# bacpop/Pansim

Hardware: AMD Instinct MI355X
Metric: generations/sec (higher is better)
Workload: dtype u8

## Files before the change

### pansim_amd/csrc/core_kernels.h

```cpp
#pragma once

#include "ps_common.h"

#include <type_traits>

#define PS_SWEEP_MAX_GENS 2
struct core_sweep_args {
    uint8_t *state;
    uint8_t *out;
    const uint32_t *idx;
    const uint32_t *idx_next[PS_SWEEP_MAX_GENS - 1];
    const uint32_t *idxT;
    uint32_t N, pitch, cpr, rows;
    uint32_t site_offset;
    uint32_t gen, k0, k1;
    ps_core_plan plan;
    uint32_t *overflow_flag;
    unsigned long long *stamps;
    uint32_t *work_ctr;
    uint32_t launch_parity;
    uint32_t nt;
    uint32_t qcap;
    uint32_t qcap_limit;
    uint32_t *wide_flags;
    const uint32_t *site_T;
};

typedef uint32_t ps_u32x4 __attribute__((ext_vector_type(4)));
__device__ __forceinline__ uint4 ps_load_row16(const uint8_t *p, bool nt)
{
    if (nt) {
        const ps_u32x4 v = __builtin_nontemporal_load((const ps_u32x4 *)p);
        return make_uint4(v.x, v.y, v.z, v.w);
    }
    return *(const uint4 *)p;
}
__device__ __forceinline__ void ps_store_row16(uint8_t *p, const uint4 &v, bool nt)
{
    if (nt) {
        ps_u32x4 w = { v.x, v.y, v.z, v.w };
        __builtin_nontemporal_store(w, (ps_u32x4 *)p);
    } else {
        *(uint4 *)p = v;
    }
}

__device__ __forceinline__ void ps_set_byte(uint32_t (&w)[4], uint32_t k, uint32_t v)
{
    const uint32_t j = k >> 2, sh = (k & 3u) * 8u;
    const uint32_t m = ~(0xFFu << sh), val = v << sh;
#pragma unroll
    for (uint32_t jj = 0; jj < 4; jj++) w[jj] = (jj == j) ? ((w[jj] & m) | val) : w[jj];
}

#ifndef PS_WAVE_DMA
#define PS_WAVE_DMA 0
#endif
__device__ __forceinline__ void ps_dma16(const uint8_t *gsrc, uint8_t *lds_base, bool nt)
{
    if (nt) __builtin_amdgcn_global_load_lds((const __attribute__((address_space(1))) void *)gsrc,
                                             (__attribute__((address_space(3))) void *)lds_base, 16, 0, 2);
    else __builtin_amdgcn_global_load_lds((const __attribute__((address_space(1))) void *)gsrc,
                                          (__attribute__((address_space(3))) void *)lds_base, 16, 0, 0);
}

__device__ __forceinline__ uint32_t ps_noncand_word(const ps_u4 &A, uint32_t cshift)
{
    return (cshift <= 0u ? A.x : 0u) | (cshift <= 1u ? A.y : 0u) | (cshift <= 2u ? A.z : 0u) | (cshift <= 3u ? A.w : 0u);
}

__device__ __forceinline__ uint32_t ps_site_bits(uint32_t site) { return 0x0F0F0F0Fu << (4u * (site & 1u)); }
__device__ __forceinline__ uint32_t ps_bit_cell(uint32_t p) { return ((p & 3u) << 2) | (p >> 3); }
__device__ __forceinline__ uint32_t ps_valid_word(uint32_t nvalid)
{
    if (nvalid >= 16u) return 0xFFFFFFFFu;
    uint32_t m = 0;
#pragma unroll
    for (uint32_t k = 0; k < 16u; k++)
        if (k < nvalid) m |= 0x11u << (8u * (k & 3u) + (k >> 2));
    return m;
}

__device__ __forceinline__ uint32_t ps_cand_word(const ps_u4 &A, uint32_t site, uint32_t cshift)
{
    return ~ps_noncand_word(A, cshift) & ps_site_bits(site);
}

template <bool WT>
__device__ __forceinline__ ps_cell ps_classify_site(uint32_t u, const ps_core_plan &pl, const core_sweep_args &a, uint32_t site)
{
    if (!WT) return ps_classify(u, pl);
    const uint4 *rec = (const uint4 *)(a.site_T + 8u * (size_t)min(site - a.site_offset, a.rows - 1u));
    const uint4 lo = rec[0], hi = rec[1];
    ps_core_plan sp;
    sp.T[0] = lo.x; sp.T[1] = lo.y; sp.T[2] = lo.z; sp.T[3] = lo.w; sp.T[4] = hi.x; sp.T[5] = hi.y; sp.T[6] = hi.z;
    return ps_classify(u, sp);
}

template <bool WT>
__device__ __forceinline__ ps_cell ps_cell_events(const core_sweep_args &a, const ps_u4 &A, const ps_u4 &B, uint32_t site, uint32_t ind, uint32_t gen,
                                                  uint32_t k0, uint32_t k1, const ps_core_plan &pl, uint32_t &l2y)
{
    ps_cell o = { 0u, 0u };
    const uint32_t n = ps_cell_nibble(A, site, ind);
    if (n >> pl.cshift) return o;
    const uint32_t code = ps_sym_code(4u * n + ps_cell_pair(B, site, ind), pl);
    if (code > 1u) {
        o.mut = code;
    } else if (code == 1u) {
        const ps_u4 l2 = ps_philox(site, ind, gen, PS_STREAM_CORE_L2, k0, k1);
        o = ps_classify_site<WT>(l2.x, pl, a, site);
        l2y = l2.y;
    }
    return o;
}

template <bool DO_GATHER, bool DO_MUT, bool DO_HR, bool WT = false>
__global__ void __launch_bounds__(1024) core_sweep_inline_kernel(core_sweep_args a)
{
    extern __shared__ __attribute__((aligned(16))) uint8_t lds[];
    const uint32_t lane = threadIdx.x, lpr = blockDim.x;
    uint8_t *rowA = lds;
    uint8_t *rowS = rowA + a.pitch;
    uint16_t *hrm = (uint16_t *)(rowS + a.pitch);
    const ps_core_plan pl = a.plan;
    const bool events = pl.has_events && (DO_MUT || DO_HR);

    for (uint32_t row = blockIdx.x; row < a.rows; row += gridDim.x) {
        const uint32_t site = a.site_offset + row;
        uint8_t *grow = a.state + (size_t)row * a.pitch;
        if (DO_GATHER) {
            for (uint32_t c = lane; c < a.cpr; c += lpr)
                *(uint4 *)(rowA + 16u * c) = *(const uint4 *)(grow + 16u * c);
            __syncthreads();
        }
        for (uint32_t c = lane; c < a.cpr; c += lpr) {
            uint32_t d[4];
            if (DO_GATHER) {
#pragma unroll
                for (int j = 0; j < 4; j++) {
                    uint32_t w = 0;
#pragma unroll
                    for (int b = 0; b < 4; b++) {
                        const uint32_t i = c * 16u + 4 * j + b;
                        const uint32_t v = (i < a.N) ? (uint32_t)rowA[a.idx[i]] : 0u;
                        w |= v << (8 * b);
                    }
                    d[j] = w;
                }
            } else {
                const uint4 v = *(const uint4 *)(grow + 16u * c);
                d[0] = v.x; d[1] = v.y; d[2] = v.z; d[3] = v.w;
            }
            uint32_t hm = 0;
            if (events) {
                const ps_u4 A = ps_philox_l1a(site >> 1, c, a.gen, a.k0, a.k1), B = ps_philox_l1b(site >> 2, c, a.gen, a.k0, a.k1);
                uint32_t cm = ps_cand_word(A, site, pl.cshift);
                while (cm) {
                    const uint32_t k = ps_bit_cell(__builtin_ctz(cm));
                    cm &= cm - 1u;
                    const uint32_t i = c * 16u + k;
                    if (i >= a.N) continue;
                    uint32_t l2y;
                    const ps_cell cell = ps_cell_events<WT>(a, A, B, site, i, a.gen, a.k0, a.k1, pl, l2y);
                    if (DO_MUT && cell.mut) ps_set_byte(d, k, cell.mut);
                    if (DO_HR && cell.hr) hm |= 1u << k;
                }
            }
            if (DO_HR) {
                *(uint4 *)(rowS + 16u * c) = make_uint4(d[0], d[1], d[2], d[3]);
                hrm[c] = (uint16_t)hm;
            } else {
                *(uint4 *)(grow + 16u * c) = make_uint4(d[0], d[1], d[2], d[3]);
            }
        }
        if (DO_HR) {
            __syncthreads();
            for (uint32_t c = lane; c < a.cpr; c += lpr) {
                const uint4 v = *(const uint4 *)(rowS + 16u * c);
                uint32_t d[4] = { v.x, v.y, v.z, v.w };
                uint32_t hm = hrm[c];
                while (hm) {
                    const uint32_t k = __builtin_ctz(hm);
                    hm &= hm - 1u;
                    const uint32_t i = c * 16u + k;
                    const ps_u4 l2 = ps_philox(site, i, a.gen, PS_STREAM_CORE_L2, a.k0, a.k1);
                    uint32_t donor = ps_mulhi(l2.y, a.N - 1u);
                    donor += (donor >= i) ? 1u : 0u;
                    ps_set_byte(d, k, (uint32_t)rowS[donor]);
                }
                *(uint4 *)(grow + 16u * c) = make_uint4(d[0], d[1], d[2], d[3]);
            }
            if (!DO_GATHER) __syncthreads();
        }
    }
}

#define PS_BATCH_ROWS 4u

__device__ __forceinline__ void ps_wave_sync()
{
    __builtin_amdgcn_fence(__ATOMIC_RELEASE, "wavefront");
    __builtin_amdgcn_wave_barrier();
    __builtin_amdgcn_fence(__ATOMIC_ACQUIRE, "wavefront");
}

__device__ __forceinline__ uint32_t ps_lane_prefix(uint64_t bal)
{
    return __builtin_amdgcn_mbcnt_hi((uint32_t)(bal >> 32), __builtin_amdgcn_mbcnt_lo((uint32_t)bal, 0u));
}

__device__ __forceinline__ uint32_t ps_wave_scan_incl(uint32_t x)
{
    x += (uint32_t)__builtin_amdgcn_update_dpp(0, (int)x, 0x111, 0xF, 0xF, false);
    x += (uint32_t)__builtin_amdgcn_update_dpp(0, (int)x, 0x112, 0xF, 0xF, false);
    x += (uint32_t)__builtin_amdgcn_update_dpp(0, (int)x, 0x114, 0xF, 0xF, false);
    x += (uint32_t)__builtin_amdgcn_update_dpp(0, (int)x, 0x118, 0xF, 0xF, false);
    x += (uint32_t)__builtin_amdgcn_update_dpp(0, (int)x, 0x142, 0xA, 0xF, false);
    x += (uint32_t)__builtin_amdgcn_update_dpp(0, (int)x, 0x143, 0xC, 0xF, false);
    return x;
}

struct ps_class_words { uint32_t dec, res; };
__device__ __forceinline__ ps_class_words ps_classes(uint32_t p0, uint32_t p1, uint32_t p2, uint32_t p3, uint32_t p4, uint32_t p5,
                                                     uint32_t k, uint32_t nE, uint32_t vm)
{
    const uint32_t c1 = __builtin_amdgcn_bitop3_b32(p1, p2, p3, 0x01) & vm;
    uint32_t lt;
    switch (nE) {
    case 1: lt = __builtin_amdgcn_bitop3_b32(p0, p5, p4, 0x01); break;
    case 2: lt = __builtin_amdgcn_bitop3_b32(p0, p5, p4, 0x03); break;
    case 3: lt = __builtin_amdgcn_bitop3_b32(p0, p5, p4, 0x07); break;
    case 4: lt = __builtin_amdgcn_bitop3_b32(p0, p5, p4, 0x0F); break;
    case 5: lt = __builtin_amdgcn_bitop3_b32(p0, p5, p4, 0x1F); break;
    case 6: lt = __builtin_amdgcn_bitop3_b32(p0, p5, p4, 0x3F); break;
    case 7: lt = __builtin_amdgcn_bitop3_b32(p0, p5, p4, 0x7F); break;
    default: lt = 0xFFFFFFFFu; break;
    }
    ps_class_words o;
    o.dec = k ? c1 & __builtin_amdgcn_bitop3_b32(p0, p5, p4, 0x07) : 0u;
    o.res = c1 & lt & ~o.dec;
    return o;
}

struct ps_apply_words { uint32_t y0, y1, ya, yb, yc; };
PS_HD uint32_t ps_bfi(uint32_t m, uint32_t a, uint32_t b)
{
#if defined(__HIP_DEVICE_COMPILE__) && __has_builtin(__builtin_amdgcn_bitop3_b32)
    return __builtin_amdgcn_bitop3_b32(m, a, b, 0xCA);
#else
    return (a & m) | (b & ~m);
#endif
}
__device__ __forceinline__ ps_apply_words ps_apply_prepare(uint32_t dec, uint32_t p4, uint32_t p5)
{
    const uint32_t r1 = p5 >> 1, r2 = p4 >> 2, l1 = p5 << 1, l2 = dec << 2;
    ps_apply_words o;
    o.y0 = ps_bfi(0x01010101u, p4, ps_bfi(0x02020202u, l1, l2));
    o.y1 = ps_bfi(0x02020202u, p4, ps_bfi(0x04040404u, l1, l2));
    o.ya = ps_bfi(0x09090909u, r2, ps_bfi(0x12121212u, r1, dec));
    o.yb = ps_bfi(0x12121212u, r2, ps_bfi(0x24242424u, r1, dec));
    o.yc = ps_bfi(0x24242424u, r2, ps_bfi(0x48484848u, r1, dec));
    return o;
}
template <uint32_t SLOT>
__device__ __forceinline__ uint32_t ps_apply_dword(const ps_apply_words &y, uint32_t d)
{
    constexpr uint32_t sh = SLOT == 0u ? 0u : SLOT == 1u ? 1u : SLOT == 2u ? 0u : SLOT == 3u ? 1u : SLOT == 4u ? 2u : SLOT == 5u ? 3u : SLOT == 6u ? 4u : 5u;
    const uint32_t src = SLOT == 0u ? y.y0 : SLOT == 1u ? y.y1 : (SLOT == 2u || SLOT == 5u) ? y.ya : (SLOT == 3u || SLOT == 6u) ? y.yb : y.yc;
    const uint32_t f = (src >> sh) & 0x07070707u;
    const uint32_t allele = __builtin_amdgcn_perm(0x00080402u, 0u, f);
    const uint32_t mask = __builtin_amdgcn_perm(0x00FFFFFFu, 0u, f);
    return ps_bfi(mask, allele, d);
}
template <uint32_t H>
__device__ __forceinline__ void ps_apply_row(const ps_apply_words &y, uint4 &d)
{
    d.x = ps_apply_dword<4u * H + 0u>(y, d.x);
    d.y = ps_apply_dword<4u * H + 1u>(y, d.y);
    d.z = ps_apply_dword<4u * H + 2u>(y, d.z);
    d.w = ps_apply_dword<4u * H + 3u>(y, d.w);
}

__device__ __forceinline__ uint32_t ps_push_scan(uint32_t w0, uint32_t w1, uint16_t *q, uint32_t lane, uint32_t qcap)
{
    const uint32_t c0 = (uint32_t)__popc(w0), c = c0 + (uint32_t)__popc(w1);
    const uint32_t incl = ps_wave_scan_incl(c);
    const uint32_t qn = __builtin_amdgcn_readlane(incl, 63);
    if (qn <= qcap) {
        uint16_t *qp = q + (incl - c) - 1, *qp1 = qp + c0;
        const uint32_t tag = lane << 6;
        for (uint32_t m = w0; m; m &= m - 1u) *++qp = (uint16_t)(tag | (uint32_t)__builtin_ctz(m));
        for (uint32_t m = w1; m; m &= m - 1u) *++qp1 = (uint16_t)(tag | 32u | (uint32_t)__builtin_ctz(m));
    }
    return qn;
}
__device__ __forceinline__ uint32_t ps_entry_cell(uint32_t ent)
{
    const uint32_t cell = ((ent & 3u) << 2) | ((ent >> 3) & 3u), row = ((ent >> 2) & 1u) | ((ent >> 4) & 2u);
    return (row << 10) | ((ent >> 2) & 0x3F0u) | cell;
}

PS_HD uint32_t ps_gather_dword(uint32_t lane, uint32_t m) { return lane + 64u * m; }
PS_HD uint32_t ps_gather_child(uint32_t lane, uint32_t m, uint32_t b) { return 4u * ps_gather_dword(lane, m) + b; }
PS_HD uint32_t ps_gather_source(uint32_t child, uint32_t parent, uint32_t N, uint32_t pitch)
{
    return child < N ? parent : (N < pitch - 1u ? N : pitch - 1u);
}

__device__ __forceinline__ uint32_t ps_pack4(uint32_t b0, uint32_t b1, uint32_t b2, uint32_t b3)
{
    return __builtin_amdgcn_perm(b1, b0, 0x0c0c0400u) | __builtin_amdgcn_perm(b3, b2, 0x04000c0cu);
}

#ifdef PS_STAMP
#define PS_T(k) do { unsigned long long t_; asm volatile("s_waitcnt lgkmcnt(0)\n\ts_memtime %0\n\ts_waitcnt lgkmcnt(0)" : "=s"(t_) :: "memory"); st_acc[k] += t_ - st_last; st_last = t_; } while (0)
#else
#define PS_T(k) do { } while (0)
#endif
#ifndef PS_WAVE_LB
#define PS_WAVE_LB 6
#endif
#ifndef PS_WAVE_PREFETCH
#define PS_WAVE_PREFETCH 0
#endif
__host__ __device__ constexpr uint32_t ps_queue_bytes(uint32_t qcap) { return (qcap * 2u + 15u) & ~15u; }
__host__ __device__ constexpr uint32_t ps_wave_lds(uint32_t qcap) { return PS_BATCH_ROWS * 1024u + ps_queue_bytes(qcap); }

template <bool DO_GATHER, bool DO_MUT, bool DO_HR, bool NT = false, bool WT = false, uint32_t T = 1>
__global__ void __launch_bounds__(256, T > 1 ? 4 : PS_WAVE_LB) core_sweep_wave_kernel(core_sweep_args a)
{
    static_assert(T >= 1 && T <= PS_SWEEP_MAX_GENS, "generations per pass");
    static_assert(T == 1 || (DO_GATHER && (DO_MUT || DO_HR)), "several generations per pass: the gather + events form only");
#ifdef PS_STAMP
    unsigned long long st_acc[8] = { 0, 0, 0, 0, 0, 0, 0, 0 };
    unsigned long long st_last;
    asm volatile("s_memtime %0\n\ts_waitcnt lgkmcnt(0)" : "=s"(st_last) :: "memory");
#endif
#ifdef PS_GROUP_TIMES
    const unsigned long long gt_start = __builtin_amdgcn_s_memrealtime();
#endif
    constexpr uint32_t PS_ROWS = PS_BATCH_ROWS;
    extern __shared__ __attribute__((aligned(16))) uint8_t lds[];
    const uint32_t wave = threadIdx.x >> 6, lane = threadIdx.x & 63u;
    uint8_t *rowbuf = lds + wave * ps_wave_lds(a.qcap);
    uint16_t *q = (uint16_t *)(rowbuf + PS_ROWS * 1024u);
    const ps_core_plan pl = a.plan;
    const uint32_t nE = 3u * pl.k + pl.R;
    constexpr bool events = DO_MUT || DO_HR;
    const bool has_chunk = lane < a.cpr;
    const uint32_t i0 = lane * 16u;
    const uint32_t ld_off = has_chunk ? i0 : 0u;
    const uint32_t nvalid = (i0 >= a.N) ? 0u : min(16u, a.N - i0);
    const uint32_t vm = ps_valid_word(nvalid);

    uint32_t pidx[T][16];
    if (DO_GATHER) {
#pragma unroll
        for (uint32_t t = 0; t < T; t++) {
            const uint32_t *ix = t ? a.idx_next[t ? t - 1u : 0u] : a.idx;
            const bool wide = ((uintptr_t)ix & 15u) == 0u;
#pragma unroll
            for (uint32_t m = 0; m < 4; m++) {
                const uint32_t c0 = ps_gather_child(lane, m, 0u);
                if (wide && c0 + 4u <= a.N) {
                    const uint4 p4 = *(const uint4 *)(ix + c0);
                    pidx[t][4u * m] = p4.x, pidx[t][4u * m + 1u] = p4.y, pidx[t][4u * m + 2u] = p4.z, pidx[t][4u * m + 3u] = p4.w;
                } else {
#pragma unroll
                    for (uint32_t b = 0; b < 4; b++) pidx[t][4u * m + b] = ps_gather_source(c0 + b, c0 + b < a.N ? ix[c0 + b] : 0u, a.N, a.pitch);
                }
            }
        }
    }

    constexpr uint32_t PS_CHUNK = 3u;
    const uint32_t grp = blockIdx.x & 7u;
    const uint32_t off = a.site_offset & 3u, g0 = a.site_offset >> 2;
    const uint32_t batches = (a.rows + off + PS_ROWS - 1u) / PS_ROWS;
    const uint32_t b_lo = (uint32_t)((uint64_t)batches * grp / 8u), b_hi = (uint32_t)((uint64_t)batches * (grp + 1u) / 8u);
    uint32_t *ctr = a.work_ctr + (a.launch_parity * 8u + grp) * 32u;
    if (blockIdx.x < 8u && threadIdx.x == 0) a.work_ctr[((a.launch_parity ^ 1u) * 8u + blockIdx.x) * 32u] = 0u;
    uint32_t next_chunk = 0;
    if (lane == 0) next_chunk = __hip_atomic_fetch_add(ctr, 1u, __ATOMIC_RELAXED, __HIP_MEMORY_SCOPE_AGENT);
#if PS_WAVE_PREFETCH
    uint4 vn[PS_ROWS];
    uint32_t pf_batch = 0xFFFFFFFFu;
#pragma unroll
    for (uint32_t rr = 0; rr < PS_ROWS; rr++) vn[rr] = make_uint4(0, 0, 0, 0);
#endif
    for (;;) {
        const uint32_t chunk = __builtin_amdgcn_readfirstlane(next_chunk);
        if (b_lo + chunk * PS_CHUNK >= b_hi) break;
        if (lane == 0) next_chunk = __hip_atomic_fetch_add(ctr, 1u, __ATOMIC_RELAXED, __HIP_MEMORY_SCOPE_AGENT);
    for (uint32_t cb = 0; cb < PS_CHUNK; cb++) {
        const uint32_t batch = b_lo + chunk * PS_CHUNK + cb;
        if (batch >= b_hi) break;
        const int lr0 = (int)(batch * PS_ROWS) - (int)off;
        const uint32_t sg = g0 + batch;
        auto lrow = [&](uint32_t rr) -> uint32_t { return (uint32_t)min(max(lr0 + (int)rr, 0), (int)a.rows - 1); };
        uint4 v[PS_ROWS];
#if PS_WAVE_PREFETCH
        if (pf_batch == batch) {
#pragma unroll
            for (uint32_t rr = 0; rr < PS_ROWS; rr++) v[rr] = vn[rr];
        } else
#endif
#pragma unroll
        for (uint32_t rr = 0; rr < PS_ROWS; rr++)
            v[rr] = ps_load_row16(a.state + (size_t)lrow(rr) * a.pitch + ld_off, NT);
        if (DO_GATHER) {
#pragma unroll
            for (uint32_t rr = 0; rr < PS_ROWS; rr++) *(uint4 *)(rowbuf + rr * 1024u + i0) = v[rr];
            ps_wave_sync();
        }
        PS_T(0);

#pragma unroll
        for (uint32_t t = 0; t < T; t++) {
        const uint32_t gen = a.gen + t;
        uint32_t wl[2] = { 0u, 0u };
        ps_apply_words y[2] = {};
        if (events) {
            const ps_u4 A0 = ps_philox_l1a(2u * sg, lane, gen, a.k0, a.k1);
            const ps_u4 A1 = ps_philox_l1a(2u * sg + 1u, lane, gen, a.k0, a.k1);
            const ps_u4 B = ps_philox_l1b(sg, lane, gen, a.k0, a.k1);
            const ps_class_words c0 = ps_classes(A0.x, A0.y, A0.z, A0.w, B.x, B.z, pl.k, nE, vm);
            const ps_class_words c1 = ps_classes(A1.x, A1.y, A1.z, A1.w, B.y, B.w, pl.k, nE, vm);
            wl[0] = c0.res;
            wl[1] = c1.res;
            if (DO_MUT) {
                y[0] = ps_apply_prepare(c0.dec, B.x & c0.dec, B.z & c0.dec);
                y[1] = ps_apply_prepare(c1.dec, B.y & c1.dec, B.w & c1.dec);
            }
        }
        PS_T(2);
        constexpr bool ahead = T > 1 && DO_GATHER;
        uint32_t g[16] = {};
        auto gather = [&](uint32_t rr) {
#pragma unroll
            for (int k = 0; k < 16; k++) g[k] = rowbuf[rr * 1024u + pidx[t][k]];
        };
        if (ahead) gather(0u);
#pragma unroll
        for (uint32_t rr = 0; rr < PS_ROWS; rr++) {
            uint8_t *row = rowbuf + rr * 1024u;
            uint4 d = v[rr];
            if (DO_GATHER) {
                if (!ahead) gather(rr);
                uint32_t w[4];
#pragma unroll
                for (int m = 0; m < 4; m++) w[m] = ps_pack4(g[4 * m], g[4 * m + 1], g[4 * m + 2], g[4 * m + 3]);
                ps_wave_sync();
#pragma unroll
                for (uint32_t m = 0; m < 4; m++) *(uint32_t *)(row + 4u * ps_gather_dword(lane, m)) = w[m];
                if (events && DO_MUT) {
                    ps_wave_sync();
                    d = *(const uint4 *)(row + i0);
                }
                if (ahead && rr + 1u < PS_ROWS) {
                    __builtin_amdgcn_sched_barrier(0);
                    gather(rr + 1u);
                    __builtin_amdgcn_sched_barrier(0);
                }
            }
            if (events && DO_MUT) {
                if (rr & 1u) ps_apply_row<1u>(y[rr >> 1], d);
                else ps_apply_row<0u>(y[rr >> 1], d);
            }
            if (events && (DO_MUT || !DO_GATHER)) *(uint4 *)(row + i0) = d;
            __builtin_amdgcn_sched_barrier(0);
        }
        PS_T(1);
        const uint32_t qcap = a.qcap_limit ? min(a.qcap, a.qcap_limit) : a.qcap;
        uint32_t qn = 0;
        if (events) qn = ps_push_scan(wl[0], wl[1], q, lane, qcap);
        PS_T(3);
        ps_wave_sync();
#if PS_WAVE_PREFETCH
        if (t + 1u == T) {
            uint32_t nb = batch + 1u;
            if (cb + 1u >= PS_CHUNK || nb >= b_hi) nb = b_lo + (uint32_t)__builtin_amdgcn_readfirstlane(next_chunk) * PS_CHUNK;
            pf_batch = nb < b_hi ? nb : 0xFFFFFFFFu;
            if (nb < b_hi) {
                const int nlr0 = (int)(nb * PS_ROWS) - (int)off;
#pragma unroll
                for (uint32_t rr = 0; rr < PS_ROWS; rr++)
                    vn[rr] = ps_load_row16(a.state + (size_t)(uint32_t)min(max(nlr0 + (int)rr, 0), (int)a.rows - 1) * a.pitch + ld_off, NT);
            }
        }
#endif
        const bool redo = events && (qn > qcap || (DO_HR && 2u * qn > qcap));
        if (redo) {
#pragma unroll 1
            for (uint32_t rr = 0; rr < PS_ROWS; rr++) {
                uint8_t *row = rowbuf + rr * 1024u;
                const uint32_t site = 4u * sg + rr;
                const ps_u4 Ar = ps_philox_l1a(site >> 1, lane, gen, a.k0, a.k1);
                const ps_u4 Br = ps_philox_l1b(sg, lane, gen, a.k0, a.k1);
                uint32_t cmr = ps_cand_word(Ar, site, pl.cshift) & vm;
                uint32_t hm = 0;
                while (cmr) {
                    const uint32_t k = ps_bit_cell(__builtin_ctz(cmr)), cellidx = i0 + k;
                    cmr &= cmr - 1u;
                    uint32_t l2y = 0;
                    const ps_cell cell = ps_cell_events<WT>(a, Ar, Br, site, cellidx, gen, a.k0, a.k1, pl, l2y);
                    if (DO_MUT && cell.mut) row[cellidx] = (uint8_t)cell.mut;
                    if (DO_HR && cell.hr) hm |= 1u << k;
                }
                if (DO_HR) {
                    ps_wave_sync();
                    uint32_t dv[4] = { 0u, 0u, 0u, 0u };
                    for (uint32_t tmp = hm; tmp;) {
                        const uint32_t k = __builtin_ctz(tmp), cellidx = i0 + k;
                        tmp &= tmp - 1u;
                        const ps_u4 l2 = ps_philox(site, cellidx, gen, PS_STREAM_CORE_L2, a.k0, a.k1);
                        uint32_t donor = ps_mulhi(l2.y, a.N - 1u);
                        donor += (donor >= cellidx) ? 1u : 0u;
                        ps_set_byte(dv, k, (uint32_t)row[donor]);
                    }
                    ps_wave_sync();
                    for (uint32_t tmp = hm; tmp;) {
                        const uint32_t k = __builtin_ctz(tmp);
                        tmp &= tmp - 1u;
                        row[i0 + k] = (uint8_t)((dv[k >> 2] >> (8u * (k & 3u))) & 0xFFu);
                    }
                }
            }
            ps_wave_sync();
        } else if (events) {
            uint16_t *qh = q + qcap - 1u;
            for (uint32_t base = 0; base < qn; base += 64u) {
                const uint32_t e = base + lane;
                if (e < qn) {
                    const uint32_t ent = ps_entry_cell(q[e]);
                    const uint32_t cellidx = ent & 1023u, rr = ent >> 10;
                    const ps_u4 l2 = ps_philox(4u * sg + rr, cellidx, gen, PS_STREAM_CORE_L2, a.k0, a.k1);
                    const ps_cell cell = ps_classify_site<WT>(l2.x, pl, a, 4u * sg + rr);
                    if (DO_MUT && cell.mut) rowbuf[ent] = (uint8_t)cell.mut;
                    if (DO_HR) {
                        uint32_t out = 0;
                        if (cell.hr) {
                            uint32_t donor = ps_mulhi(l2.y, a.N - 1u);
                            donor += (donor >= cellidx) ? 1u : 0u;
                            out = donor | 0x8000u;
                        }
                        *(qh - e) = (uint16_t)out;
                    }
                }
            }
            if (DO_HR) {
                ps_wave_sync();
                for (uint32_t base = 0; base < qn; base += 64u) {
                    const uint32_t e = base + lane;
                    if (e < qn) {
                        const uint32_t h = *(qh - e);
                        if (h >> 15) *(qh - e) = (uint16_t)((uint32_t)rowbuf[(ps_entry_cell(q[e]) & 3072u) | (h & 1023u)] | 0x8000u);
                    }
                }
                ps_wave_sync();
                for (uint32_t base = 0; base < qn; base += 64u) {
                    const uint32_t e = base + lane;
                    if (e < qn) {
                        const uint32_t h = *(qh - e);
                        if (h >> 15) rowbuf[ps_entry_cell(q[e])] = (uint8_t)(h & 0xFFu);
                    }
                }
            }
            ps_wave_sync();
        }
        }
        PS_T(5);

        if (has_chunk) {
#pragma unroll
            for (uint32_t rr = 0; rr < PS_ROWS; rr++) {
                const int lr = lr0 + (int)rr;
                if (lr >= 0 && lr < (int)a.rows) {
                    const uint4 o = (DO_GATHER || events) ? *(const uint4 *)(rowbuf + rr * 1024u + i0) : v[rr];
                    ps_store_row16(a.out + (size_t)lr * a.pitch + i0, o, NT);
                }
            }
        }
        ps_wave_sync();
        PS_T(6);
    }
    }
#ifdef PS_STAMP
    if (lane == 0)
        for (int k = 0; k < 8; k++) atomicAdd((unsigned long long *)a.stamps + k, st_acc[k]);
#endif
#ifdef PS_GROUP_TIMES
    if (lane == 0) {
        atomicMax((unsigned long long *)a.stamps + 8 + grp, (unsigned long long)__builtin_amdgcn_s_memrealtime());
        atomicMax((unsigned long long *)a.stamps + 16 + grp, gt_start);
        if (blockIdx.x < 8 && wave == 0) ((unsigned long long *)a.stamps)[24 + grp] = gt_start;
    }
#endif
}

#ifndef PS_WCAP
#define PS_WCAP 1216u
#endif
#ifndef PS_WBPC
#define PS_WBPC 6
#endif
#ifndef PS_WLB
#define PS_WLB 6
#endif
#ifndef PS_WINDOW_NT_LOADS
#define PS_WINDOW_NT_LOADS 0
#endif
#define PS_WSTRIDE (PS_WCAP + 16u)
#define PS_WHR 64u
__host__ __device__ constexpr uint32_t ps_window_lds(uint32_t qcap) { return PS_BATCH_ROWS * PS_WSTRIDE + ps_queue_bytes(qcap) + PS_WHR * 6u; }

template <bool WT>
__device__ __forceinline__ uint32_t ps_donor_value(const core_sweep_args &a, const ps_core_plan &pl, const uint8_t *old_row,
                                                   uint32_t site, uint32_t donor, bool do_mut)
{
    uint32_t val = old_row[a.idx[donor]];
    if (do_mut) {
        const ps_u4 A = ps_philox_l1a(site >> 1, donor >> 4, a.gen, a.k0, a.k1);
        const uint32_t n = ps_cell_nibble(A, site, donor);
        if ((n >> pl.cshift) == 0u) {
            const ps_u4 B = ps_philox_l1b(site >> 2, donor >> 4, a.gen, a.k0, a.k1);
            const uint32_t code = ps_sym_code(4u * n + ps_cell_pair(B, site, donor), pl);
            if (code > 1u) {
                val = code;
            } else if (code == 1u) {
                const ps_u4 l2 = ps_philox(site, donor, a.gen, PS_STREAM_CORE_L2, a.k0, a.k1);
                const ps_cell cell = ps_classify_site<WT>(l2.x, pl, a, site);
                if (cell.mut) val = cell.mut;
            }
        }
    }
    return val;
}


template <bool DO_MUT, bool DO_HR, bool NT, bool WIDE, bool WT = false>
__global__ void __launch_bounds__(256, PS_WLB) core_sweep_window_kernel(core_sweep_args a)
{
    constexpr uint32_t PS_ROWS = PS_BATCH_ROWS;
    extern __shared__ __attribute__((aligned(16))) uint8_t lds[];
    const uint32_t wave = threadIdx.x >> 6, lane = threadIdx.x & 63u;
    uint8_t *rowbuf = lds + wave * ps_window_lds(a.qcap);
    uint16_t *q = (uint16_t *)(rowbuf + PS_ROWS * PS_WSTRIDE);
    uint32_t *hr_d = (uint32_t *)(rowbuf + PS_ROWS * PS_WSTRIDE + ps_queue_bytes(a.qcap));
    uint16_t *hr_e = (uint16_t *)(hr_d + PS_WHR);
    if (lane < PS_ROWS) *(uint4 *)(rowbuf + lane * PS_WSTRIDE + PS_WCAP) = make_uint4(0, 0, 0, 0);
    const ps_core_plan pl = a.plan;
    const uint32_t segs = (a.N + 1023u) >> 10;
    const uint32_t grp = blockIdx.x & 7u;
    const uint32_t wg = __builtin_amdgcn_readfirstlane((blockIdx.x >> 3) * 4u + wave);
    const uint32_t sgm = wg % segs;
    if (wg < segs && lane == 0) a.work_ctr[(((a.launch_parity ^ 1u) * 8u + grp) * segs + wg) * 32u] = 0u;
    if (WIDE) {
        if (__builtin_amdgcn_readfirstlane(a.wide_flags[(a.gen & 1u) * 32u]) == 0u) return;
    } else if (blockIdx.x == 0 && threadIdx.x == 0) {
        a.wide_flags[((a.gen + 1u) & 1u) * 32u] = 0u;
    }
    const uint32_t c_first = sgm * 1024u, c_last = min(c_first + 1023u, a.N - 1u);
    const uint32_t chunk = sgm * 64u + lane;
    const bool has_chunk = chunk < a.cpr;
    const uint32_t i0 = lane * 16u, c0 = c_first + i0;
    const uint32_t nvalid = (c0 >= a.N) ? 0u : min(16u, a.N - c0);
    const uint32_t vm = ps_valid_word(nvalid);
    const uint32_t nE = 3u * pl.k + pl.R;
    const uint32_t w_lo = __builtin_amdgcn_readfirstlane(a.idx[c_first]) & ~15u;
    const uint32_t w_hi = __builtin_amdgcn_readfirstlane(a.idx[c_last]);
    const uint32_t wbytes = w_hi - w_lo + 1u;
    const bool wide = wbytes > PS_WCAP;
    uint32_t pidx[16];
#pragma unroll
    for (uint32_t k = 0; k < 16; k++) pidx[k] = (k < nvalid) ? a.idx[c0 + k] - w_lo : PS_WCAP;
    const bool ld0 = !WIDE && i0 < wbytes, ld1 = !WIDE && 1024u + i0 < wbytes;
    auto cell_addr = [](uint32_t ent) -> uint32_t { return (ent & 1023u) + ((ent >> 10) & 3u) * PS_WSTRIDE; };

    constexpr uint32_t PS_CHUNK = 3u;
    const uint32_t off = a.site_offset & 3u, g0 = a.site_offset >> 2;
    const uint32_t batches = (a.rows + off + PS_ROWS - 1u) / PS_ROWS;
    const uint32_t b_lo = (uint32_t)((uint64_t)batches * grp / 8u), b_hi = (uint32_t)((uint64_t)batches * (grp + 1u) / 8u);
    uint32_t *ctr = a.work_ctr + ((a.launch_parity * 8u + grp) * segs + sgm) * 32u;
    if (wide != WIDE) {
        if (!WIDE && lane == 0) a.wide_flags[(a.gen & 1u) * 32u] = 1u;
        return;
    }
    uint32_t next_chunk = 0;
    if (lane == 0) next_chunk = __hip_atomic_fetch_add(ctr, 1u, __ATOMIC_RELAXED, __HIP_MEMORY_SCOPE_AGENT);
    for (;;) {
        const uint32_t chk = __builtin_amdgcn_readfirstlane(next_chunk);
        if (b_lo + chk * PS_CHUNK >= b_hi) break;
        if (lane == 0) next_chunk = __hip_atomic_fetch_add(ctr, 1u, __ATOMIC_RELAXED, __HIP_MEMORY_SCOPE_AGENT);
    for (uint32_t cb = 0; cb < PS_CHUNK; cb++) {
        const uint32_t batch = b_lo + chk * PS_CHUNK + cb;
        if (batch >= b_hi) break;
        const int lr0 = (int)(batch * PS_ROWS) - (int)off;
        const uint32_t sg = g0 + batch;
        auto lrow = [&](uint32_t rr) -> uint32_t { return (uint32_t)min(max(lr0 + (int)rr, 0), (int)a.rows - 1); };
#pragma unroll
        for (uint32_t rr = 0; rr < PS_ROWS; rr++) {
            const uint8_t *src = a.state + (size_t)lrow(rr) * a.pitch + w_lo;
            if (ld0) ps_dma16(src + i0, rowbuf + rr * PS_WSTRIDE, NT && PS_WINDOW_NT_LOADS);
            if (ld1) ps_dma16(src + 1024u + i0, rowbuf + rr * PS_WSTRIDE + 1024u, NT && PS_WINDOW_NT_LOADS);
        }
        uint32_t wl0, wl1;
        ps_apply_words y[2] = {};
        {
            const ps_u4 A0 = ps_philox_l1a(2u * sg, chunk, a.gen, a.k0, a.k1);
            const ps_u4 A1 = ps_philox_l1a(2u * sg + 1u, chunk, a.gen, a.k0, a.k1);
            const ps_u4 B = ps_philox_l1b(sg, chunk, a.gen, a.k0, a.k1);
            const ps_class_words c0 = ps_classes(A0.x, A0.y, A0.z, A0.w, B.x, B.z, pl.k, nE, vm);
            const ps_class_words c1 = ps_classes(A1.x, A1.y, A1.z, A1.w, B.y, B.w, pl.k, nE, vm);
            wl0 = c0.res;
            wl1 = c1.res;
            if (DO_MUT) {
                y[0] = ps_apply_prepare(c0.dec, B.x & c0.dec, B.z & c0.dec);
                y[1] = ps_apply_prepare(c1.dec, B.y & c1.dec, B.w & c1.dec);
            }
        }
        asm volatile("s_waitcnt vmcnt(0)" ::: "memory");
        ps_wave_sync();
#pragma unroll
        for (uint32_t rr = 0; rr < PS_ROWS; rr++) {
            uint8_t *win = rowbuf + rr * PS_WSTRIDE;
            uint32_t w[4] = { 0u, 0u, 0u, 0u };
            if (!WIDE) {
#pragma unroll
                for (int j = 0; j < 4; j++)
                    w[j] = ps_pack4(win[pidx[4 * j]], win[pidx[4 * j + 1]], win[pidx[4 * j + 2]], win[pidx[4 * j + 3]]);
// ... 1523 lines not shown
```

### pansim_amd/csrc/pansim_capi.hip

```cpp
#include "../../include/pansim_hip.h"

#include <hip/hip_runtime.h>

#include <algorithm>
#include <charconv>
#include <chrono>
#include <condition_variable>
#include <mutex>
#include <cmath>
#include <cstdarg>
#include <cstdio>
#include <cstdlib>
#include <cstring>
#include <string>
#include <thread>
#include <type_traits>
#include <vector>

#include "acc_kernels.h"
#include "core_kernels.h"
#include "ps_common.h"

static thread_local std::string g_err;

// ... 80 lines not shown
    hs_poisson_table(lambda, &kmin, &t);
    if (t.empty() || t.size() > cap || !kmin_out || !thr) return 0;
    *kmin_out = kmin;
    memcpy(thr, t.data(), t.size() * sizeof(uint32_t));
    return (uint32_t)t.size();
}


static uint32_t prob_to_u32(double p)
{
    const double x = std::floor(p * 4294967296.0);
    if (!(x > 0.0)) return 0u;
    if (x >= 4294967295.0) return 0xFFFFFFFFu;
    return (uint32_t)x;
}

static void make_core_plan(double lam_mut, double lam_hr, uint64_t L, ps_core_plan *plan)
{
    const double p = (lam_mut > 0.0) ? -std::expm1(-lam_mut / (double)L) : 0.0;
    const double q = (lam_hr > 0.0) ? -std::expm1(-lam_hr / (double)L) : 0.0;
    const double a = p * (1.0 - q) / 3.0;
    const double b = p * q / 3.0;
    const double c = (1.0 - p) * q;
    const uint32_t k = (uint32_t)std::floor(a * 64.0);
    const double a_left = a - (double)k / 64.0;
    const double m_res = a_left + a_left + a_left + b + b + b + c;
    uint32_t R = (uint32_t)std::ceil(m_res * 64.0);
    if (3u * k + R > 64u) R = 64u - 3u * k;
    const double scale = R ? 64.0 / (double)R : 0.0;
    double cum[7];
    cum[0] = a_left * scale;
    cum[1] = (a_left + a_left) * scale;
    cum[2] = (a_left + a_left + a_left) * scale;
    cum[3] = (a_left + a_left + a_left + b) * scale;
    cum[4] = (a_left + a_left + a_left + b + b) * scale;
    cum[5] = (a_left + a_left + a_left + b + b + b) * scale;
    cum[6] = m_res * scale;
    uint32_t prev = 0;
    for (int j = 0; j < 7; j++) {
        uint32_t t = prob_to_u32(cum[j]);
        if (t < prev) t = prev;
        plan->T[j] = t;
        prev = t;
    }
    if (plan->T[6] == 0u) R = 0u;
    plan->k = k;
    plan->R = R;
    plan->has_events = (k > 0u || R > 0u) ? 1u : 0u;
    uint32_t cs = 0;
    while (cs < 4u && 3u * k + R > (4u << cs)) cs++;
    plan->cshift = cs;
}

static uint32_t acc_flip_threshold(double lam, uint64_t n_genes)
{
    if (!(lam > 0.0) || n_genes == 0) return 0u;
    const double pf = -std::expm1(-2.0 * lam / (double)n_genes) / 2.0;
    return prob_to_u32(pf);
}

enum { PS_RO_HIST, PS_RO_CLUSTERS, PS_RO_TREE, PS_RO_KNN, PS_RO_GEN, PS_RO_LD_SEL, PS_RO_LD, PS_RO_UPGMA, PS_RO_DIFF, PS_RO_PARS, PS_RO_TCMP, PS_RO_GS, PS_RO_MLST, PS_RO_NJ, PS_RO_BOOT, PS_RO_NNI, PS_RO_LIK, PS_RO_MODEL, PS_RO_MODEL_NNI, PS_RO_ANC, PS_RO_GENE, PS_RO_COUNT };
struct readout_slot {
    void *d = nullptr;
    uint64_t cap = 0;
    double ms[5] = {};
    bool timed = false;
};

struct ps_population {
    ps_config cfg{};
    int device = 0;
    hipStream_t stream = nullptr;
    bool rates_set = false;
    uint8_t *state = nullptr;
    uint8_t *state2 = nullptr;
    int sweep_oop = -1;
    uint32_t pitch = 0, cpr = 0;
    ps_core_plan cplan{};
    bool site_weighted = false;
    uint32_t *d_site_T = nullptr;
    uint8_t *d_gene_tab = nullptr;
    bool nibble_safe = true;
    bool onehot_safe = true;
    uint32_t *d_pack2 = nullptr;
    uint32_t *d_pair_part = nullptr;
    uint64_t pair_part_cap = 0;
    uint64_t pack2_cap = 0;
    acc_dims d{};
    uint64_t *G[2] = { nullptr, nullptr };
    bool g_valid = false;
    int32_t *fuse_counts_out = nullptr;
    double *fuse_logw_out = nullptr;
    bool counts_fresh = false;
    hipStream_t stream_of_call = nullptr;
    uint64_t edit_epoch = 0;
    uint64_t *I[2] = { nullptr, nullptr };
    uint32_t *d_ptab[PS_MAX_COMP] = {};
    uint32_t ptab_kmin[PS_MAX_COMP] = {}, ptab_len[PS_MAX_COMP] = {};
    void *hgt_ovf_img = nullptr;
    uint32_t hgt_bin_cap = 0;
    void *hgt_scratch = nullptr;
    uint64_t hgt_scratch_cap = 0;
    uint64_t *I_snap = nullptr;
    bool snap_valid = false;
    uint32_t hgt_slices = 0;
    uint32_t hgt_events_per_thread = 0;
    bool hgt_list_in_global = false;
    bool hgt_bin_list_in_global = false;
    uint32_t hgt_bin_prio = 0;
    uint32_t *cnt = nullptr;
    int cur = 0;
    ps_acc_plan aplan{};
    uint32_t donor_lo = 0, donor_cnt = 0;
    uint64_t *d_delta = nullptr;
    uint64_t delta_words = 0;
    ps_exchange_fn exchange = nullptr;
    void *exchange_ctx = nullptr;
    uint32_t *d_idx = nullptr;
    uint32_t *d_idxT = nullptr;
    uint32_t *d_work = nullptr;
    uint32_t work_flags_ofs = 0;
    uint64_t sweep_launches = 0;
    uint64_t window_launches = 0;
    double *d_log1p = nullptr;
    int32_t *d_num_genes = nullptr;
    double *d_logw = nullptr;
    uint32_t *d_H = nullptr;
    double *d_Dt = nullptr;
    void *d_davg = nullptr;
    uint64_t davg_cap = 0;
    int davg_form = 0;
    void *d_davg_in = nullptr;
    uint64_t davg_in_cap = 0;
    uint32_t davg_nb = 0;
    uint32_t davg_ib = 0;
    bool davg_plain_division = false;
    uint64_t H_cap = 0;
    int core_davg_form = 0;
    uint32_t core_davg_band = 0;
    uint32_t *d_cdavg = nullptr;
    uint64_t cdavg_cap = 0;
    int pair_mode = 0;
    int last_pair_form = 0;
    uint32_t pair_ranges = 0;
    int hgt_mode = 0;
    void *d_pairs = nullptr;
    uint32_t pair_threads = 0;
    uint64_t pairs_cap = 0, pairs_cached = 0;
    const uint32_t *pairs_src1 = nullptr, *pairs_src2 = nullptr;
    bool pairs_tiled = false;
    std::vector<uint32_t> h_r1, h_r2;
    uint32_t lds_limit = 160 * 1024;
    uint32_t sweep_blocks_per_cu = 8;
    uint32_t sweep_rows = 4;
    bool force_block_sweep = false;
    bool force_inline_sweep = false;
    uint32_t block_waves = 0;
    bool no_block_preload = false;
    uint32_t block_batch = 0;
    uint32_t sweep_generations = 0;
    uint32_t sweep_queue_cap = 0;
    uint32_t hgt_apply_threads = 1024;
    uint32_t window_blocks_per_cu = 0;
    uint32_t free_cus_per_xcd = 0;
    bool exchange_beside_sweep = false;
    int last_sweep_form = 0;
    int window_sweep = -1;
    int (*rows_refresh)(void *ctx) = nullptr;
    void *rows_ctx = nullptr;
    std::vector<uint32_t> row_slot;
    uint32_t *d_row_slot = nullptr;
    bool rows_overridden = false;
    uint32_t *d_site_counts = nullptr;
    unsigned long long *d_div = nullptr;
    hipEvent_t div_ev[2] = {};
    bool div_timed = false;
    readout_slot ro[PS_RO_COUNT];
    uint32_t gene_team = 0;
    uint32_t ld_band = 0;
    uint32_t mlst_band = 0;
    int gather_form = 0;
    double sample_ms = 0.0;
    bool sample_timed = false;
    uint32_t *h_flag = nullptr, *d_flag = nullptr;
    unsigned long long *h_stamps = nullptr, *d_stamps = nullptr;
};

static int use_device(const ps_population *p)
{
    HIPCHK(hipSetDevice(p->device));
    return PS_OK;
}

template <class T>
static hipError_t dev_grow_err(T *&ptr, uint64_t &cap, uint64_t need)
{
    if (cap >= need) return hipSuccess;
    if (ptr) {
        const hipError_t e = hipFree(ptr);
        if (e != hipSuccess) return e;
    }
    ptr = nullptr;
    cap = 0;
    const hipError_t e = hipMalloc(&ptr, need * sizeof(std::conditional_t<std::is_void<T>::value, char, T>));
    if (e == hipSuccess) cap = need;
    return e;
}

template <class T>
static int dev_grow(T *&ptr, uint64_t &cap, uint64_t need)
{
    HIPCHK(dev_grow_err(ptr, cap, need));
    return PS_OK;
}

#include "readout_common.h"

template <class T>
struct dev_tmp {
    T *p = nullptr;
    int device = 0;
    dev_tmp() = default;
    dev_tmp(const dev_tmp &) = delete;
    dev_tmp &operator=(const dev_tmp &) = delete;
    ~dev_tmp()
    {
        if (!p) return;
        (void)hipSetDevice(device);
        (void)hipFree(p);
    }
    int alloc(uint64_t n)
    {
        HIPCHK(hipGetDevice(&device));
        HIPCHK(hipMalloc(&p, n * sizeof(T)));
        return PS_OK;
    }
};

static int rows_current(ps_population *p, const uint32_t **slot_out)
{
    if (p->rows_overridden) p->row_slot.clear();
    else if (p->rows_refresh) PSCHK(p->rows_refresh(p->rows_ctx));
    *slot_out = p->row_slot.empty() ? nullptr : p->row_slot.data();
    return PS_OK;
}

template <typename T>
static void rows_permute(T *v, const uint32_t *slot, uint64_t n)
{
    if (!slot) return;
    std::vector<T> tmp(v, v + n);
    for (uint64_t k = 0; k < n; k++) v[k] = tmp[slot[k]];
}

extern "C" void ps_population_destroy(ps_population *p)
{
    if (!p) return;
    (void)hipSetDevice(p->device);
    if (p->stream) (void)hipStreamSynchronize(p->stream);
    void *ptrs[] = { p->d_row_slot, p->state, p->state2, p->d_delta, p->hgt_ovf_img, p->G[0], p->G[1], p->I[0], p->I[1], p->I_snap, p->d_ptab[0], p->d_ptab[1], p->hgt_scratch, p->cnt, p->d_idx, p->d_idxT, p->d_work,
                     p->d_log1p, p->d_num_genes, p->d_logw, p->d_pairs, p->d_H, p->d_Dt, p->d_davg, p->d_davg_in, p->d_pack2, p->d_pair_part, p->d_cdavg };
    for (void *q : ptrs)
        if (q) (void)hipFree(q);
    for (int c = 2; c < PS_MAX_COMP; c++)
        if (p->d_ptab[c]) (void)hipFree(p->d_ptab[c]);
    if (p->d_site_T) (void)hipFree(p->d_site_T);
    if (p->d_gene_tab) (void)hipFree(p->d_gene_tab);
    if (p->d_site_counts) (void)hipFree(p->d_site_counts);
    if (p->d_div) (void)hipFree(p->d_div);
    for (readout_slot &r : p->ro)
        if (r.d) (void)hipFree(r.d);
    for (hipEvent_t e : p->div_ev)
        if (e) (void)hipEventDestroy(e);
    if (p->h_flag) (void)hipHostFree(p->h_flag);
    if (p->h_stamps) {
        if (p->d_stamps) {
            (void)hipMemcpy(p->h_stamps, p->d_stamps, 32 * sizeof(unsigned long long), hipMemcpyDeviceToHost);
            (void)hipFree(p->d_stamps);
        }
        if (getenv("PANSIM_PRINT_STAMPS"))
            for (int k = 0; k < 32; k++) fprintf(stderr, "stamp[%d] = %llu\n", k, p->h_stamps[k]);
        (void)hipHostFree(p->h_stamps);
    }
    if (p->stream) (void)hipStreamDestroy(p->stream);
    delete p;
}

static int pop_create_impl(const ps_config *cfg, const uint8_t *init_vec, ps_population *p)
{
    int ndev = 0;
    PSCHK(ps_needs_device(&ndev));
    if (cfg->device >= 0) {
        if (cfg->device >= ndev) return ps_fail(PS_ERR_INVALID, "device %d out of range", cfg->device);
        p->device = cfg->device;
    } else {
        HIPCHK(hipGetDevice(&p->device));
    }
    PSCHK(use_device(p));
    if (cfg->core)
        if (const char *e = getenv("PANSIM_SWEEP_FREE_CUS")) p->free_cus_per_xcd = (uint32_t)std::max(0, std::min(8, atoi(e)));
    if (p->free_cus_per_xcd) {
        hipDeviceProp_t prop;
        HIPCHK(hipGetDeviceProperties(&prop, p->device));
        std::vector<uint32_t> mask((size_t)(prop.multiProcessorCount + 31) / 32, 0xFFFFFFFFu);
        for (uint32_t b = 0; b < 8u * p->free_cus_per_xcd && b < (uint32_t)prop.multiProcessorCount; b++) mask[b / 32u] &= ~(1u << (b % 32u));
        if (hipExtStreamCreateWithCUMask(&p->stream, (uint32_t)mask.size(), mask.data()) != hipSuccess) {
            (void)hipGetLastError();
            p->free_cus_per_xcd = 0;
            HIPCHK(hipStreamCreateWithFlags(&p->stream, hipStreamNonBlocking));
        }
    } else
    HIPCHK(hipStreamCreateWithFlags(&p->stream, hipStreamNonBlocking));
    if (const char *e = getenv("PANSIM_SWEEP_BLOCKS_PER_CU")) {
        const int v = atoi(e);
        if (v >= 1 && v <= 8) p->sweep_blocks_per_cu = (uint32_t)v;
    }
    if (const char *e = getenv("PANSIM_SWEEP_GENERATIONS")) {
        const int v = atoi(e);
        if (v >= 0 && v <= (int)PS_SWEEP_MAX_GENS) p->sweep_generations = (uint32_t)v;
    }
    if (const char *e = getenv("PANSIM_HGT_MODE")) p->hgt_mode = atoi(e);
    if (const char *e = getenv("PANSIM_SWEEP_OOP")) p->sweep_oop = std::max(-1, std::min(2, atoi(e)));
    if (const char *e = getenv("PANSIM_WINDOW_SWEEP")) p->window_sweep = std::max(-1, std::min(1, atoi(e)));
    if (const char *e = getenv("PANSIM_ACC_LDS_LIMIT")) { const int v = atoi(e); if (v >= 1024 && v <= 160 * 1024 && !cfg->core) p->lds_limit = (uint32_t)v; }
    if (const char *e = getenv("PANSIM_HGT_APPLY_THREADS")) { const int v = atoi(e); if (v == 256 || v == 512 || v == 1024) p->hgt_apply_threads = (uint32_t)v; }
    if (const char *e = getenv("PANSIM_WINDOW_BPC")) p->window_blocks_per_cu = (uint32_t)std::max(0, std::min(8, atoi(e)));
    if (const char *e = getenv("PANSIM_BLOCK_BATCH")) p->block_batch = (uint32_t)atoi(e);
    if (const char *e = getenv("PANSIM_BLOCK_WAVES")) p->block_waves = (uint32_t)atoi(e);
    if (const char *e = getenv("PANSIM_HGT_SLICES")) p->hgt_slices = (uint32_t)atoi(e);
    if (const char *e = getenv("PANSIM_HGT_BIN_LIST_GLOBAL")) p->hgt_bin_list_in_global = atoi(e) != 0;
    if (const char *e = getenv("PANSIM_HGT_BIN_PRIO")) p->hgt_bin_prio = (uint32_t)std::max(0, std::min(3, atoi(e)));
    if (const char *e = getenv("PANSIM_SWEEP_ROWS")) {
        const int v = atoi(e);
        if (v >= 2 && v <= 4) p->sweep_rows = (uint32_t)v;
    }
    const uint64_t N = cfg->pop_size, C = cfg->ncols;
    HIPCHK(hipMalloc(&p->d_idx, std::max<uint64_t>(N, 1) * sizeof(uint32_t)));
    HIPCHK(hipHostMalloc(&p->h_flag, sizeof(uint32_t), hipHostMallocMapped));
    *p->h_flag = 0;
    HIPCHK(hipHostMalloc(&p->h_stamps, 32 * sizeof(unsigned long long), hipHostMallocMapped));
    memset(p->h_stamps, 0, 32 * sizeof(unsigned long long));
    HIPCHK(hipMalloc(&p->d_stamps, 32 * sizeof(unsigned long long)));
    HIPCHK(hipMemset(p->d_stamps, 0, 32 * sizeof(unsigned long long)));
    HIPCHK(hipHostGetDevicePointer((void **)&p->d_flag, p->h_flag, 0));
    uint8_t *d_vec = nullptr;
    HIPCHK(hipMalloc(&d_vec, std::max<uint64_t>(C, 1)));
    if (C && init_vec) HIPCHK(hipMemcpyAsync(d_vec, init_vec, C, hipMemcpyHostToDevice, p->stream));
    if (cfg->core) {
        p->pitch = (uint32_t)((N + 127) / 128 * 128);
        p->cpr = p->pitch / 16;
        HIPCHK(hipMalloc(&p->state, std::max<uint64_t>(C, 1) * p->pitch));
        HIPCHK(hipMalloc(&p->d_idxT, 16ull * p->cpr * sizeof(uint32_t)));
        {
            const uint64_t nctr = 8 * std::max<uint64_t>(1, std::min<uint64_t>((N + 1023) / 1024, 4096));
            HIPCHK(hipMalloc(&p->d_work, 2 * nctr * 128 + 256));
            HIPCHK(hipMemsetAsync(p->d_work, 0, 2 * nctr * 128 + 256, p->stream));
            p->work_flags_ofs = (uint32_t)(2 * nctr * 32);
        }
        if (C && init_vec) {
            const uint64_t total = C * p->cpr;
            const uint32_t blocks = (uint32_t)std::min<uint64_t>((total + 255) / 256, 65536);
            core_init_kernel<<<blocks, 256, 0, p->stream>>>(p->state, d_vec, (uint32_t)N, p->pitch,
                                                            (uint32_t)C);
        }
    } else {
        p->d.N = (uint32_t)N;
        p->d.G = (uint32_t)C;
        p->d.W = (uint32_t)((N + 63) / 64);
        p->d.GW = (uint32_t)((C + 63) / 64);
        const uint64_t nG = std::max<uint64_t>((uint64_t)p->d.G * p->d.W, 1) * 8;
        const uint64_t nI = std::max<uint64_t>((uint64_t)p->d.N * p->d.GW, 1) * 8;
        HIPCHK(hipMalloc(&p->G[0], nG));
        for (int k = 0; k < 2; k++) HIPCHK(hipMalloc(&p->I[k], nI));
        if (C > 65536) return ps_fail(PS_ERR_INVALID, "at most 65536 accessory genes are supported");
        HIPCHK(hipMalloc(&p->cnt, (std::max<uint64_t>(N, 1) * PS_MAX_COMP + 64) * sizeof(uint32_t)));
        HIPCHK(hipMalloc(&p->d_log1p, std::max<uint64_t>(C, 1) * sizeof(double)));
        HIPCHK(hipMalloc(&p->d_num_genes, std::max<uint64_t>(N, 1) * sizeof(int32_t)));
        HIPCHK(hipMalloc(&p->d_logw, std::max<uint64_t>(N, 1) * sizeof(double)));
        const uint64_t total = (uint64_t)p->d.G * p->d.W + (uint64_t)p->d.N * p->d.GW;
        if (total && init_vec)
            acc_init_kernel<<<(uint32_t)((total + 255) / 256), 256, 0, p->stream>>>(p->G[0], p->I[0],
                                                                                d_vec, p->d);
        p->g_valid = true;
    }
    HIPCHK(hipGetLastError());
    HIPCHK(hipStreamSynchronize(p->stream));
    HIPCHK(hipFree(d_vec));
    return PS_OK;
}

extern "C" int ps_population_create(const ps_config *cfg, const uint8_t *init_vec, ps_population **out)
{
    if (!cfg || !out) return ps_fail(PS_ERR_INVALID, "null argument");
    *out = nullptr;
    if (cfg->pop_size < 1) return ps_fail(PS_ERR_INVALID, "pop_size must be >= 1");
    if (cfg->pop_size > 0xFFFFFFFFull - 128 || cfg->global_cols > 0xFFFFFFFFull
        || cfg->ncols > 0xFFFFFFFFull)
        return ps_fail(PS_ERR_INVALID, "pop_size and column counts must fit 32 bits");
    if (cfg->col_offset + cfg->ncols > cfg->global_cols)
        return ps_fail(PS_ERR_INVALID, "column shard [%llu,%llu) exceeds global_cols %llu",
                       (unsigned long long)cfg->col_offset,
                       (unsigned long long)(cfg->col_offset + cfg->ncols),
                       (unsigned long long)cfg->global_cols);
    if (!cfg->core && (cfg->col_offset != 0 || cfg->ncols != cfg->global_cols))
        return ps_fail(PS_ERR_INVALID, "the accessory matrix is replicated, not sharded");
    if (cfg->ncols && !init_vec) return ps_fail(PS_ERR_INVALID, "init_vec is null");
    ps_population *p = new ps_population();
    p->cfg = *cfg;
    const int rc = pop_create_impl(cfg, init_vec, p);
    if (rc != PS_OK) {
        const std::string keep = g_err;
        ps_population_destroy(p);
        g_err = keep;
        return rc;
    }
    *out = p;
    return PS_OK;
}

extern "C" int ps_init_vector(uint64_t seed, int core, uint64_t col_offset, uint64_t ncols,
                              double avg_gene_freq, uint8_t *out)
{
    if (!out && ncols) return ps_fail(PS_ERR_INVALID, "null output");
    for (uint64_t c = 0; c < ncols; c++) {
        const uint64_t g = col_offset + c;
        if (core)
            out[c] = (uint8_t)(1u << (hs_u32(seed, PS_STREAM_INIT_CORE, 0, g) >> 30));
        else
            out[c] = hs_f64(seed, PS_STREAM_INIT_ACC, 0, g) < avg_gene_freq ? 1 : 0;
    }
    return PS_OK;
}

static int check_device_flag(ps_population *p)
{
    if (p->h_flag && *p->h_flag != 0)
        return ps_fail(PS_ERR_STATE, "a device error flag is set (%u)", *p->h_flag);
    return PS_OK;
}

static int sync_checked(ps_population *p)
{
    HIPCHK(hipStreamSynchronize(p->stream));
    return check_device_flag(p);
}

extern "C" int ps_sync(ps_population *p)
{
    if (!p) return ps_fail(PS_ERR_INVALID, "null handle");
    PSCHK(use_device(p));
    return sync_checked(p);
}

extern "C" int ps_set_tuning(ps_population *p, const char *key, int64_t value)
{
    if (!p || !key) return ps_fail(PS_ERR_INVALID, "null argument");
    const std::string k(key);
    if (k == "sweep_blocks_per_cu") {
        if (value < 1 || value > 8) return ps_fail(PS_ERR_INVALID, "sweep_blocks_per_cu must be 1..8");
        p->sweep_blocks_per_cu = (uint32_t)value;
    } else if (k == "sweep_rows") {
        if (value < 2 || value > 4) return ps_fail(PS_ERR_INVALID, "sweep_rows must be 2..4");
        p->sweep_rows = (uint32_t)value;
    } else if (k == "sweep_out_of_place") {
        if (value < -1 || value > 2) return ps_fail(PS_ERR_INVALID, "sweep_out_of_place must be -1 (choose), 0 (in place), 1 (out of place) or 2 (out of place, nontemporal loads and stores)");
        p->sweep_oop = (int)value;
    } else if (k == "hgt_apply_threads") {
        if (value != 256 && value != 512 && value != 1024) return ps_fail(PS_ERR_INVALID, "hgt_apply_threads must be 256, 512 or 1024");
        p->hgt_apply_threads = (uint32_t)value;
    } else if (k == "window_blocks_per_cu") {
        if (value < 0 || value > 8) return ps_fail(PS_ERR_INVALID, "window_blocks_per_cu must be 0 (choose) or 1..8");
        p->window_blocks_per_cu = (uint32_t)value;
    } else if (k == "davg_form") {
        if (value < 0 || value > 3)
            return ps_fail(PS_ERR_INVALID, "davg_form must be 0 (choose), 1 (LDS-tile popcount kernels), 2 (matrix cores, one kernel) or 3 (matrix cores, two phases)");
        p->davg_form = (int)value;
    } else if (k == "core_davg_form") {
        if (value < 0 || value > 3)
            return ps_fail(PS_ERR_INVALID, "core_davg_form must be 0 (choose), 1 (whole matrix), 2 (banded) or 3 (generic)");
        p->core_davg_form = (int)value;
    } else if (k == "ld_band") {
        if (value < 0 || value > 65536) return ps_fail(PS_ERR_INVALID, "ld_band must be 0 (choose)..65536 rows of loci");
        p->ld_band = (uint32_t)value;
    } else if (k == "mlst_band") {
        if (value < 0 || value > 65535) return ps_fail(PS_ERR_INVALID, "mlst_band must be 0 (choose)..65535 loci");
        p->mlst_band = (uint32_t)value;
    } else if (k == "gene_team") {
        if (value != 0 && value != 64 && value != 256) return ps_fail(PS_ERR_INVALID, "gene_team must be 0 (choose), 64 or 256 threads");
        p->gene_team = (uint32_t)value;
    } else if (k == "gather_form") {
        if (value < 0 || value > 2) return ps_fail(PS_ERR_INVALID, "gather_form must be 0 (choose), 1 (source rows staged in LDS) or 2 (bytes loaded from global memory)");
        p->gather_form = (int)value;
    } else if (k == "core_davg_band") {
        if (value < 0 || value > (1ll << 31)) return ps_fail(PS_ERR_INVALID, "core_davg_band must be 0 (choose)..2^31 rows");
        p->core_davg_band = (uint32_t)value;
    } else if (k == "davg_plain_division") {
        p->davg_plain_division = value != 0;
    } else if (k == "davg_ib") {
        if (value != 0 && value != 16 && value != 32) return ps_fail(PS_ERR_INVALID, "davg_ib must be 0 (choose), 16 or 32");
        p->davg_ib = (uint32_t)value;
    } else if (k == "davg_nb") {
        if (value < 0 || value > 4 || value == 3) return ps_fail(PS_ERR_INVALID, "davg_nb must be 0 (choose), 1, 2 or (two-phase form only) 4");
        p->davg_nb = (uint32_t)value;
    } else if (k == "hgt_mode") {
        if (value < 0 || value > 2) return ps_fail(PS_ERR_INVALID, "hgt_mode must be 0 (auto), 1 (one atomic per event) or 2 (binned by recipient partition, two passes)");
        p->hgt_mode = (int)value;
    } else if (k == "pair_mode") {
        if (value < 0 || value > 7) return ps_fail(PS_ERR_INVALID, "pair_mode must be 0 (auto), 1 (sampled), 2 (all pairs), 3 (sampled, nibble form even for one-hot matrices), 4 (transposed bit strings, streamed per pair), 5 (all pairs, xor + popcount tiles even for one-hot matrices), 6 (all pairs, i8 matrix cores when the matrix is one-hot; mode 2 takes the FP4 form) or 7 (the FP4 form on three +-1 features per site)");
        p->pair_mode = (int)value;
    } else if (k == "pair_ranges") {
        if (value < 0 || value > 65535) return ps_fail(PS_ERR_INVALID, "pair_ranges must be 0 (choose)..65535");
        p->pair_ranges = (uint32_t)value;
    } else if (k == "force_block_sweep") {
        p->force_block_sweep = value != 0;
    } else if (k == "force_inline_sweep") {
        p->force_inline_sweep = value != 0;
    } else if (k == "hgt_slices") {
        if (value < 0 || value > 4096) return ps_fail(PS_ERR_INVALID, "hgt_slices must be 0..4096");
        p->hgt_slices = (uint32_t)value;
    } else if (k == "block_batch") {
        if (value != 0 && value != 2 && value != 4) return ps_fail(PS_ERR_INVALID, "block_batch must be 0 (choose), 2 or 4");
        p->block_batch = (uint32_t)value;
    } else if (k == "hgt_bin_cap") {
        if (value < 0 || value > (1 << 30)) return ps_fail(PS_ERR_INVALID, "hgt_bin_cap must be 0 (sized by the rates)..2^30");
        p->hgt_bin_cap = (uint32_t)value;
    } else if (k == "hgt_events_per_thread") {
        if (value < 0 || value > 100000) return ps_fail(PS_ERR_INVALID, "hgt_events_per_thread must be 0 (whole chip)..100000");
        p->hgt_events_per_thread = (uint32_t)value;
    } else if (k == "window_sweep") {
        if (value < -1 || value > 1) return ps_fail(PS_ERR_INVALID, "window_sweep must be -1 (choose), 0 (block sweep) or 1 (window sweep where the parents are sorted)");
        p->window_sweep = (int)value;
    } else if (k == "sweep_generations") {
        if (value < 0 || value > (int64_t)PS_SWEEP_MAX_GENS) return ps_fail(PS_ERR_INVALID, "sweep_generations must be 0 (choose), 1 or 2");
        p->sweep_generations = (uint32_t)value;
    } else if (k == "sweep_queue_cap") {
        if (value < 0 || value > 65536) return ps_fail(PS_ERR_INVALID, "sweep_queue_cap must be 0 (real size)..65536");
        p->sweep_queue_cap = (uint32_t)value;
    } else if (k == "hgt_list_in_global") {
        p->hgt_list_in_global = value != 0;
    } else if (k == "hgt_bin_list_in_global") {
        p->hgt_bin_list_in_global = value != 0;
    } else if (k == "no_block_preload") {
        p->no_block_preload = value != 0;
    } else if (k == "block_waves") {
        if (value != 0 && value != 4 && value != 8 && value != 16) return ps_fail(PS_ERR_INVALID, "block_waves must be 0 (auto), 4, 8 or 16");
        p->block_waves = (uint32_t)value;
    } else if (k == "lds_limit") {
        if (value < 1024 || value > 160 * 1024) return ps_fail(PS_ERR_INVALID, "lds_limit must be 1 KiB..160 KiB");
        p->lds_limit = (uint32_t)value;
        p->pairs_cached = 0;
    } else {
        return ps_fail(PS_ERR_INVALID, "unknown tuning key %s", key);
    }
    return PS_OK;
}

extern "C" int ps_load_matrix(ps_population *p, const uint8_t *rows)
{
    if (!p || !rows) return ps_fail(PS_ERR_INVALID, "null argument");
    PSCHK(use_device(p));
    const uint64_t N = p->cfg.pop_size, C = p->cfg.ncols;
    if (N * C == 0) return PS_OK;
    uint8_t *d_rows = nullptr;
    HIPCHK(hipMalloc(&d_rows, N * C));
    HIPCHK(hipMemcpyAsync(d_rows, rows, N * C, hipMemcpyHostToDevice, p->stream));
    if (p->cfg.core) {
        bool safe = true;
        bool onehot = true;
        for (uint64_t k = 0; k < N * C; k++) {
            const uint8_t b = rows[k];
            if (b > 15) { safe = false; onehot = false; break; }
            if (b != 1 && b != 2 && b != 4 && b != 8) onehot = false;
        }
        p->nibble_safe = safe;
        p->onehot_safe = onehot;
        dim3 grid((uint32_t)((C + 63) / 64), (uint32_t)((p->pitch + 63) / 64));
        core_transpose_kernel<true><<<grid, 256, 0, p->stream>>>(p->state, d_rows, (uint32_t)N,
                                                                 p->pitch, C);
    } else {
        const uint64_t nI = (uint64_t)p->d.N * p->d.GW;
        p->snap_valid = false;
        acc_pack_rows_kernel<<<(uint32_t)((nI + 255) / 256), 256, 0, p->stream>>>(d_rows, p->I[p->cur],
                                                                              p->d);
        p->g_valid = false;
        p->counts_fresh = false;
        p->edit_epoch++;
    }
    HIPCHK(hipGetLastError());
    HIPCHK(hipStreamSynchronize(p->stream));
    HIPCHK(hipFree(d_rows));
    p->rows_overridden = true;
    return PS_OK;
}

extern "C" int ps_read_matrix(ps_population *p, uint8_t *rows)
{
    if (!p || !rows) return ps_fail(PS_ERR_INVALID, "null argument");
    PSCHK(use_device(p));
    const uint64_t N = p->cfg.pop_size, C = p->cfg.ncols;
    if (N * C == 0) return PS_OK;
    uint8_t *d_rows = nullptr;
    HIPCHK(hipMalloc(&d_rows, N * C));
    if (p->cfg.core) {
        dim3 grid((uint32_t)((C + 63) / 64), (uint32_t)((N + 63) / 64));
        core_transpose_kernel<false><<<grid, 256, 0, p->stream>>>(p->state, d_rows, (uint32_t)N,
                                                                  p->pitch, C);
    } else {
        acc_unpack_rows_kernel<<<(uint32_t)((N * C + 255) / 256), 256, 0, p->stream>>>(
            p->I[p->cur], d_rows, p->d);
    }
    HIPCHK(hipGetLastError());
    const uint32_t *slot = nullptr;
    PSCHK(rows_current(p, &slot));
    HIPCHK(hipMemcpyAsync(rows, d_rows, N * C, hipMemcpyDeviceToHost, p->stream));
    HIPCHK(hipStreamSynchronize(p->stream));
    HIPCHK(hipFree(d_rows));
    if (slot) {
        std::vector<uint8_t> tmp(rows, rows + N * C);
        for (uint64_t k = 0; k < N; k++) memcpy(rows + k * C, tmp.data() + (uint64_t)slot[k] * C, C);
    }
    return PS_OK;
}

static int set_hgt_count_tables(ps_population *p, int n_comp, const double *lam_rec)
{
    PSCHK(use_device(p));
    for (int c = 0; c < PS_MAX_COMP; c++) {
        if (p->d_ptab[c]) { HIPCHK(hipStreamSynchronize(p->stream)); HIPCHK(hipFree(p->d_ptab[c])); }
        p->d_ptab[c] = nullptr;
        p->ptab_len[c] = 0;
        if (c >= n_comp || !(lam_rec[c] > 0.0)) continue;
        std::vector<uint32_t> thr;
        hs_poisson_table(lam_rec[c], &p->ptab_kmin[c], &thr);
        HIPCHK(hipMalloc(&p->d_ptab[c], thr.size() * sizeof(uint32_t)));
        HIPCHK(hipMemcpy(p->d_ptab[c], thr.data(), thr.size() * sizeof(uint32_t), hipMemcpyHostToDevice));
        p->ptab_len[c] = (uint32_t)thr.size();
    }
    return PS_OK;
}

extern "C" int ps_set_rates(ps_population *p, int n_comp, const double *lam_mut, const double *lam_rec,
                            const uint64_t *comp_begin, const uint64_t *comp_end)
{
    if (!p) return ps_fail(PS_ERR_INVALID, "null handle");
    if (n_comp < 0 || n_comp > 2) return ps_fail(PS_ERR_INVALID, "n_comp must be 0..2");
    for (int c = 0; c < n_comp; c++) {
        if (!(lam_mut[c] >= 0.0) || !(lam_rec[c] >= 0.0) || std::isinf(lam_mut[c]) || std::isinf(lam_rec[c]))
            return ps_fail(PS_ERR_INVALID, "rates must be finite and >= 0");
        if (comp_begin[c] > comp_end[c] || comp_end[c] > p->cfg.global_cols)
            return ps_fail(PS_ERR_INVALID, "compartment range out of bounds");
    }
    if (p->cfg.core) {
        if (n_comp != 1) return ps_fail(PS_ERR_INVALID, "the core matrix has one compartment (main.rs:276, :279)");
        if (p->cfg.pop_size < 2 && lam_rec[0] > 0.0)
            return ps_fail(PS_ERR_INVALID, "recombination needs pop_size >= 2 (population.rs:584 panics)");
        make_core_plan(lam_mut[0], lam_rec[0], p->cfg.global_cols, &p->cplan);
    } else {
        p->aplan = ps_acc_plan{};
        p->aplan.n_comp = n_comp;
        for (int c = 0; c < n_comp; c++) {
            if (p->cfg.pop_size < 2 && lam_rec[c] > 0.0)
                return ps_fail(PS_ERR_INVALID, "recombination needs pop_size >= 2 (population.rs:584 panics)");
            p->aplan.comp_begin[c] = (uint32_t)comp_begin[c];
            p->aplan.comp_end[c] = (uint32_t)comp_end[c];
            p->aplan.flip_thr[c] = acc_flip_threshold(lam_mut[c], comp_end[c] - comp_begin[c]);
            p->aplan.lam_rec[c] = lam_rec[c];
        }
        PSCHK(set_hgt_count_tables(p, n_comp, lam_rec));
    }
    p->site_weighted = false;
    p->rates_set = true;
    return PS_OK;
}

static_assert(PS_MAX_COMP == PS_MAX_SITE_COMP, "the header documents the compartment cap");
struct site_tables {
    bool ranges = false;
    uint64_t rb[PS_MAX_COMP] = {}, re[PS_MAX_COMP] = {};
    ps_core_plan cplan{};
    std::vector<uint32_t> T;
    std::vector<uint32_t> flip;
    std::vector<uint16_t> wq;
};

static bool mask_range(const float *w, uint64_t n, uint64_t *b, uint64_t *e)
{
    uint64_t i = 0;
// ... 57 lines not shown
        }
    }
    t->ranges = core ? n_comp == 1 : n_comp <= 2;
    for (int c = 0; c < n_comp && t->ranges; c++) {
        uint64_t b2 = 0, e2 = 0;
        t->ranges = mask_range(w_mut + (uint64_t)c * cols, cols, &t->rb[c], &t->re[c]);
        if (t->ranges && core) t->ranges = t->rb[c] == 0 && t->re[c] == cols;
        if (t->ranges && !core)
            t->ranges = mask_range(w_rec + (uint64_t)c * cols, cols, &b2, &e2) && b2 == t->rb[c] && e2 == t->re[c];
        if (t->ranges && c == 1) t->ranges = t->re[0] <= t->rb[1] || t->re[1] <= t->rb[0];
    }
    if (core) {
        t->T.assign(7 * cols, 0u);
        if (t->ranges) {
            make_core_plan(lam_mut[0], lam_rec[0], cols, &t->cplan);
            for (uint64_t s = 0; s < cols; s++) memcpy(&t->T[7 * s], t->cplan.T, 7 * sizeof(uint32_t));
            return PS_OK;
        }
        double lam_hr = 0.0;
        for (int c = 0; c < n_comp; c++) lam_hr += lam_rec[c];
        const double q = (lam_hr > 0.0) ? -std::expm1(-lam_hr / (double)cols) : 0.0;
        std::vector<double> ps(cols);
        double m_max = 0.0;
        for (uint64_t s = 0; s < cols; s++) {
            double r = 0.0;
            for (int c = 0; c < n_comp; c++)
                if (lam_mut[c] > 0.0) r += lam_mut[c] * (double)w_mut[(uint64_t)c * cols + s] / Wm[c];
            ps[s] = (r > 0.0) ? -std::expm1(-r) : 0.0;
            m_max = std::max(m_max, site_event_mass(ps[s], q));
        }
        uint32_t R = (uint32_t)std::ceil(m_max * 64.0);
        if (R > 64u) R = 64u;
        const double scale = R ? 64.0 / (double)R : 0.0;
        uint32_t t6 = 0;
        for (uint64_t s = 0; s < cols; s++) {
            site_thresholds(ps[s], q, scale, &t->T[7 * s]);
            t6 = std::max(t6, t->T[7 * s + 6]);
        }
        if (t6 == 0u) R = 0u;
        ps_core_plan &pl = t->cplan;
        pl = ps_core_plan{};
        pl.T[6] = t6;
        pl.k = 0u;
        pl.R = R;
        pl.has_events = R > 0u ? 1u : 0u;
        uint32_t cs = 0;
        while (cs < 4u && R > (4u << cs)) cs++;
        pl.cshift = cs;
        return PS_OK;
    }
    t->flip.assign(cols, 0u);
    t->wq.assign((uint64_t)n_comp * cols, 0);
    if (t->ranges) {
        for (int c = 0; c < n_comp; c++)
            for (uint64_t g = t->rb[c]; g < t->re[c]; g++) {
                t->flip[g] = acc_flip_threshold(lam_mut[c], t->re[c] - t->rb[c]);
                t->wq[(uint64_t)c * cols + g] = 1;
            }
        return PS_OK;
    }
    for (uint64_t g = 0; g < cols; g++) {
        double r = 0.0;
        for (int c = 0; c < n_comp; c++)
            if (lam_mut[c] > 0.0) r += lam_mut[c] * (double)w_mut[(uint64_t)c * cols + g] / Wm[c];
        t->flip[g] = (r > 0.0) ? prob_to_u32(-std::expm1(-2.0 * r) / 2.0) : 0u;
    }
    for (int c = 0; c < n_comp; c++) {
        const float *w = w_rec + (uint64_t)c * cols;
        double wmax = 0.0;
        for (uint64_t g = 0; g < cols; g++) wmax = std::max(wmax, (double)w[g]);
        if (!(wmax > 0.0)) continue;
        for (uint64_t g = 0; g < cols; g++) {
            if (!(w[g] > 0.0f)) continue;
            const double x = std::floor((double)w[g] / wmax * 65535.0 + 0.5);
            t->wq[(uint64_t)c * cols + g] = (uint16_t)(x < 1.0 ? 1.0 : x);
        }
    }
    return PS_OK;
}

extern "C" int ps_site_tables(int core, uint64_t global_cols, int n_comp, const double *lam_mut, const double *lam_rec, const float *w_mut,
                              const float *w_rec, uint32_t *plan_out, uint32_t *thr_out, uint16_t *wq_out)
{
    site_tables t;
    PSCHK(make_site_tables(core, global_cols, n_comp, lam_mut, lam_rec, w_mut, w_rec, &t));
    if (plan_out) {
        plan_out[0] = core ? t.cplan.k : 0u;
        plan_out[1] = core ? t.cplan.R : 0u;
        plan_out[2] = core ? t.cplan.cshift : 0u;
        plan_out[3] = core ? t.cplan.has_events : 0u;
        plan_out[4] = t.ranges ? 1u : 0u;
    }
    if (thr_out) {
        const std::vector<uint32_t> &v = core ? t.T : t.flip;
        memcpy(thr_out, v.data(), v.size() * sizeof(uint32_t));
    }
    if (wq_out && !core) memcpy(wq_out, t.wq.data(), t.wq.size() * sizeof(uint16_t));
    return PS_OK;
}

extern "C" int ps_set_site_rates(ps_population *p, int n_comp, const double *lam_mut, const double *lam_rec, const float *w_mut,
                                 const float *w_rec)
{
    if (!p) return ps_fail(PS_ERR_INVALID, "null handle");
    const int core = p->cfg.core ? 1 : 0;
    const uint64_t cols = p->cfg.global_cols;
    site_tables t;
    PSCHK(make_site_tables(core, cols, n_comp, lam_mut, lam_rec, w_mut, w_rec, &t));
    if (t.ranges) return ps_set_rates(p, n_comp, lam_mut, lam_rec, t.rb, t.re);
    for (int c = 0; c < n_comp; c++)
        if (p->cfg.pop_size < 2 && lam_rec[c] > 0.0)
            return ps_fail(PS_ERR_INVALID, "recombination needs pop_size >= 2 (population.rs:584 panics)");
    PSCHK(use_device(p));
    HIPCHK(hipStreamSynchronize(p->stream));
    if (core) {
        const uint64_t rows = p->cfg.ncols, off = p->cfg.col_offset;
        std::vector<uint32_t> rec(8 * std::max<uint64_t>(rows, 1), 0u);
        for (uint64_t r = 0; r < rows; r++) memcpy(&rec[8 * r], &t.T[7 * (off + r)], 7 * sizeof(uint32_t));
        if (!p->d_site_T) HIPCHK(hipMalloc(&p->d_site_T, rec.size() * sizeof(uint32_t)));
        HIPCHK(hipMemcpy(p->d_site_T, rec.data(), rec.size() * sizeof(uint32_t), hipMemcpyHostToDevice));
        p->cplan = t.cplan;
    } else {
        const uint64_t GW = p->d.GW, G64 = GW * 64;
        const uint64_t thr_bytes = G64 * 4, nz_bytes = (uint64_t)PS_MAX_COMP * GW * 8, wq_bytes = (uint64_t)PS_MAX_COMP * G64 * 2;
        std::vector<uint8_t> tab(thr_bytes + nz_bytes + wq_bytes, 0);
        uint32_t *thr = (uint32_t *)tab.data();
        uint64_t *nz = (uint64_t *)(tab.data() + thr_bytes);
        uint16_t *wq = (uint16_t *)(tab.data() + thr_bytes + nz_bytes);
        memcpy(thr, t.flip.data(), cols * 4);
        for (int c = 0; c < n_comp; c++)
            for (uint64_t g = 0; g < cols; g++) {
                const uint16_t v = t.wq[(uint64_t)c * cols + g];
                wq[(uint64_t)c * G64 + g] = v;
                if (v) nz[(uint64_t)c * GW + (g >> 6)] |= 1ull << (g & 63u);
            }
        if (!p->d_gene_tab) HIPCHK(hipMalloc(&p->d_gene_tab, tab.size()));
        HIPCHK(hipMemcpy(p->d_gene_tab, tab.data(), tab.size(), hipMemcpyHostToDevice));
        p->aplan = ps_acc_plan{};
        p->aplan.n_comp = n_comp;
        for (int c = 0; c < n_comp; c++) {
            p->aplan.comp_begin[c] = 0;
            p->aplan.comp_end[c] = (uint32_t)cols;
            p->aplan.lam_rec[c] = lam_rec[c];
        }
        PSCHK(set_hgt_count_tables(p, n_comp, lam_rec));
    }
    p->site_weighted = true;
    p->rates_set = true;
    return PS_OK;
}

static uint32_t sweep_queue_entries(const ps_core_plan &pl, uint32_t cells, bool twice)
{
    if (!pl.has_events) return 16u;
    if (pl.cshift > 1u || pl.k > 1u) return 0u;
    const double m = (double)PS_BATCH_ROWS * (double)cells * (double)pl.R / 64.0;
    const uint32_t n = ((uint32_t)std::ceil(m + 10.0 * std::sqrt(m) + 16.0) + 15u) & ~15u;
    return twice ? 2u * n : n;
}

template <bool GA, bool MU, bool HR>
static int launch_core_sweep_wave(ps_population *p, core_sweep_args a, hipStream_t st, uint32_t gens = 1)
{
    const uint32_t block = 256u, wpb = block / 64u;
    a.qcap = sweep_queue_entries(a.plan, std::min(1024u, (uint32_t)p->cfg.pop_size), HR);
    a.launch_parity = (uint32_t)(p->sweep_launches++ & 1u);
    const uint32_t lds = wpb * ps_wave_lds(a.qcap);
    const uint32_t batches = (a.rows + (a.site_offset & 3u) + PS_BATCH_ROWS - 1u) / PS_BATCH_ROWS;
    const uint32_t want = (batches + wpb - 1u) / wpb;
    const uint32_t fit = std::max(1u, std::min(8u, p->lds_limit / lds));
    const uint32_t bpc = std::min(p->sweep_blocks_per_cu, fit);
    const uint32_t grid = std::max(8u, std::min((want + 7u) & ~7u, 256u * bpc));
    constexpr bool EV = MU || HR;
    if (gens > 1) {
        if constexpr (GA && MU) {
            if (gens != 2u) return ps_fail(PS_ERR_INVALID, "the wave sweep applies 1 or 2 generations per launch, not %u", gens);
            if (a.site_T) {
                if (a.nt) hipLaunchKernelGGL((core_sweep_wave_kernel<true, true, HR, true, true, 2u>), dim3(grid), dim3(block), lds, st, a);
                else hipLaunchKernelGGL((core_sweep_wave_kernel<true, true, HR, false, true, 2u>), dim3(grid), dim3(block), lds, st, a);
            } else if (a.nt) hipLaunchKernelGGL((core_sweep_wave_kernel<true, true, HR, true, false, 2u>), dim3(grid), dim3(block), lds, st, a);
            else hipLaunchKernelGGL((core_sweep_wave_kernel<true, true, HR, false, false, 2u>), dim3(grid), dim3(block), lds, st, a);
        } else
            return ps_fail(PS_ERR_INVALID, "the wave sweep has no several-generation form of this step");
    } else
    if (EV && a.site_T) {
        if (a.nt) hipLaunchKernelGGL((core_sweep_wave_kernel<GA, MU, HR, true, EV>), dim3(grid), dim3(block), lds, st, a);
        else hipLaunchKernelGGL((core_sweep_wave_kernel<GA, MU, HR, false, EV>), dim3(grid), dim3(block), lds, st, a);
    } else if (a.nt) hipLaunchKernelGGL((core_sweep_wave_kernel<GA, MU, HR, true>), dim3(grid), dim3(block), lds, st, a);
    else hipLaunchKernelGGL((core_sweep_wave_kernel<GA, MU, HR, false>), dim3(grid), dim3(block), lds, st, a);
    HIPCHK(hipGetLastError());
    return PS_OK;
}

static bool wave_sweep_eligible(ps_population *p, bool mu, bool hr)
{
    if (p->pitch > 1024 || p->force_block_sweep) return false;
    const ps_core_plan &pl = p->cplan;
    if (!pl.has_events || (!mu && !hr)) return true;
    const uint32_t qe = sweep_queue_entries(pl, std::min(1024u, (uint32_t)p->cfg.pop_size), hr);
    return qe != 0u && 4u * ps_wave_lds(qe) <= p->lds_limit;
}

static bool block_sweep_geometry(const ps_population *p, bool ga, bool mu, bool hr, core_block_geom *g,
                                 uint32_t *lds, uint32_t *waves)
{
    const ps_core_plan &pl = p->cplan;
    const bool events = pl.has_events && (mu || hr);
    if (events && (pl.cshift > 1u || pl.k > 1u)) return false;
    g->segs = (p->cpr + 63u) / 64u;
    auto up16 = [](double x) { return (uint32_t)(((uint64_t)std::ceil(x) + 15u) & ~15ull); };
    const double hr_frac = (events && hr) ? (double)(pl.T[6] - pl.T[2]) / 4294967296.0 * (double)pl.R / 64.0 : 0.0;
    for (uint32_t SB = (p->block_batch == 2 ? 2u : 4u); SB >= 2; SB >>= 1) {
        uint32_t nw = 4;
        while (nw < 16u && nw * SB < g->segs) nw *= 2u;
        if (p->block_waves) nw = p->block_waves;
        *waves = nw;
        g->SB = SB;
        const double mq = events ? SB * 1024.0 * (double)pl.R / 64.0 : 0.0;
        g->QW = std::max(64u, up16(mq + 10.0 * std::sqrt(mq)));
        for (uint32_t R = std::max(1u, nw * SB / std::max(1u, g->segs)); R >= 1; R >>= 1) {
            const uint32_t batches_per_wave = (R * g->segs + nw * SB - 1u) / (nw * SB);
            const double mh = (double)batches_per_wave * SB * 1024.0 * hr_frac;
            g->R = R;
            g->HW = std::max(16u, up16(mh + 10.0 * std::sqrt(mh) + 16.0));
            const uint32_t rows_bytes = (ga ? 2u : 1u) * R * p->pitch;
            const uint32_t scratch = (std::max(nw * (g->QW + 2u * g->HW) * 4u, R * p->cpr * 2u + 16u) + 15u) & ~15u;
            g->ovf_off = rows_bytes + scratch - 4u;
            *lds = rows_bytes + scratch;
            if (*lds <= p->lds_limit) return true;
            if (R == 1) break;
        }
    }
    return false;
}

static bool block_sweep_preload(const ps_population *p, const core_block_geom &g, uint32_t nw)
{
    return p->pitch <= 65536u && g.R * g.segs <= nw * g.SB && !p->no_block_preload;
}

template <uint32_t SB, bool PRE, bool GA, bool MU, bool HR, bool WT = false>
static int launch_block_kernel(const core_sweep_args &a, const core_block_geom &g, uint32_t lds, uint32_t nw, hipStream_t st)
{
    if ((MU || HR) && !WT && a.site_T) return launch_block_kernel<SB, PRE, GA, MU, HR, MU || HR>(a, g, lds, nw, st);
    auto kern = core_sweep_block_kernel<SB, PRE, GA, MU, HR, WT>;
    if (lds > 64 * 1024)
        HIPCHK(hipFuncSetAttribute((const void *)kern, hipFuncAttributeMaxDynamicSharedMemorySize, (int)lds));
    const uint32_t groups = (a.rows + g.R - 1) / g.R;
    int bpc = 0;
    HIPCHK(hipOccupancyMaxActiveBlocksPerMultiprocessor(&bpc, (const void *)kern, (int)(64u * nw), lds));
    bpc = std::max(1, bpc);
    const uint32_t grid = std::max(1u, std::min(groups, 256u * (uint32_t)bpc));
    hipLaunchKernelGGL(kern, dim3(grid), dim3(64u * nw), lds, st, a, g);
    HIPCHK(hipGetLastError());
    return PS_OK;
}

template <bool GA, bool MU, bool HR>
static int launch_core_sweep_block(ps_population *p, const core_sweep_args &a, const uint32_t *d_idx, hipStream_t st)
{
    core_block_geom g{};
    uint32_t lds = 0, nw = 0;
    if (!p->force_inline_sweep && block_sweep_geometry(p, GA, MU, HR, &g, &lds, &nw)) {
        const bool pre = GA && block_sweep_preload(p, g, nw);
        if (GA) {
            const uint32_t n = (pre ? 8u : 16u) * p->cpr;
            if (pre) idx_pack16_kernel<<<(n + 255) / 256, 256, 0, st>>>(d_idx, p->d_idxT, a.N, p->cpr);
            else idx_transpose_kernel<<<(n + 255) / 256, 256, 0, st>>>(d_idx, p->d_idxT, a.N, p->cpr);
        }
        if (GA && pre)
            return g.SB == 4u ? launch_block_kernel<4, GA, GA, MU, HR>(a, g, lds, nw, st)
                              : launch_block_kernel<2, GA, GA, MU, HR>(a, g, lds, nw, st);
        return g.SB == 4u ? launch_block_kernel<4, false, GA, MU, HR>(a, g, lds, nw, st)
                          : launch_block_kernel<2, false, GA, MU, HR>(a, g, lds, nw, st);
    }
    const uint32_t block = 1024u;
    const uint32_t hrm_bytes = (a.cpr * 2u + 15u) & ~15u;
    lds = 2u * a.pitch + hrm_bytes;
    if (lds > p->lds_limit)
        return ps_fail(PS_ERR_INVALID, "pop_size %u needs %u bytes of LDS per row (limit %u)", a.N, lds,
                       p->lds_limit);
    constexpr bool EV = MU || HR;
    auto kern = (EV && a.site_T) ? core_sweep_inline_kernel<GA, MU, HR, EV> : core_sweep_inline_kernel<GA, MU, HR>;
    if (lds > 64 * 1024)
        HIPCHK(hipFuncSetAttribute((const void *)kern, hipFuncAttributeMaxDynamicSharedMemorySize, (int)lds));
    const uint32_t cap = 256u * (lds > 80 * 1024 ? 1u : 2u);
    const uint32_t grid = std::max(1u, std::min(a.rows, cap));
    hipLaunchKernelGGL(kern, dim3(grid), dim3(block), lds, st, a);
    HIPCHK(hipGetLastError());
    return PS_OK;
}

static uint32_t window_sweep_lds(const ps_core_plan &pl)
{
    const uint32_t qe = sweep_queue_entries(pl, 1024u, false);
    return qe ? 4u * ps_window_lds(qe) : 0u;
}

template <bool HR>
static int launch_core_sweep_window(ps_population *p, const core_sweep_args &a, hipStream_t st)
{
    const uint32_t lds = window_sweep_lds(a.plan);
    const uint32_t bpc = std::max(1u, std::min(p->window_blocks_per_cu ? p->window_blocks_per_cu : (uint32_t)PS_WBPC, p->lds_limit / lds));
    const uint32_t segs = (a.N + 1023u) / 1024u;
    const uint32_t grid = (std::max(8u * ((segs + 3u) / 4u), (256u - 8u * p->free_cus_per_xcd) * bpc) + 7u) & ~7u;
    core_sweep_args a0 = a, b = a;
    a0.qcap = b.qcap = sweep_queue_entries(a.plan, 1024u, false);
    a0.launch_parity = (uint32_t)(p->window_launches++ & 1u);
    b.launch_parity = (uint32_t)(p->window_launches++ & 1u);
#define PS_WLAUNCH(NT_)                                                                                                    \
    {                                                                                                                     \
        hipLaunchKernelGGL((core_sweep_window_kernel<true, HR, NT_, false>), dim3(grid), dim3(256), lds, st, a0);          \
        hipLaunchKernelGGL((core_sweep_window_kernel<true, HR, NT_, true>), dim3(grid), dim3(256), lds, st, b);            \
    }
#define PS_WLAUNCH_W(NT_)                                                                                                  \
    {                                                                                                                     \
        hipLaunchKernelGGL((core_sweep_window_kernel<true, HR, NT_, false, true>), dim3(grid), dim3(256), lds, st, a0);    \
        hipLaunchKernelGGL((core_sweep_window_kernel<true, HR, NT_, true, true>), dim3(grid), dim3(256), lds, st, b);      \
    }
    if (a.site_T) { if (a.nt) PS_WLAUNCH_W(true) else PS_WLAUNCH_W(false) }
    else if (a.nt) PS_WLAUNCH(true) else PS_WLAUNCH(false)
#undef PS_WLAUNCH_W
#undef PS_WLAUNCH
    HIPCHK(hipGetLastError());
    return PS_OK;
}

static int launch_core_sweep(ps_population *p, const uint32_t *d_idx, uint32_t gen, bool ga, bool mu,
                             bool hr, hipStream_t st, bool parents_sorted = false, uint32_t gens = 1,
                             const uint32_t *const *d_idx_next = nullptr)
{
    if (p->cfg.ncols == 0) return PS_OK;
    core_sweep_args a;
    a.state = p->state;
// ... 1017 lines not shown
                hipLaunchKernelGGL(core_allpairs_mfma_fp4_kernel<false>, dim3(tile_pairs, ranges), dim3(512), lds, st, p->d_pack2, WT, N, p->d_H, cpr, n_chunks, ntile);
                p->last_pair_form = PS_PAIR_FORM_ALLPAIRS_MFMA_FP4;
            } else {
            HIPCHK(hipFuncSetAttribute((const void *)core_allpairs_mfma_kernel, hipFuncAttributeMaxDynamicSharedMemorySize, (int)lds));
            hipLaunchKernelGGL(core_allpairs_mfma_kernel, dim3(tile_pairs, ranges), dim3(512), lds, st, p->d_pack2, WT, N, p->d_H, cpr, n_chunks, ntile);
            }
            if (ranges > 1u) core_allpairs_sum_slices_kernel<<<N, 256, 0, st>>>(p->d_H, N, ranges);
            core_pair_lookup256_kernel<<<(uint32_t)((P + 255) / 256), 256, 0, st>>>(p->d_H, N, d_r1, d_r2, d_perm, P, d_a);
        } else
        if (use_all) {
            p->last_pair_form = PS_PAIR_FORM_ALLPAIRS;
            const uint32_t WA = 32u, ntile = (N + 127u) / 128u;
            const uint32_t lds = 2u * 128u * ((WA >> 2) + 1u) * 16u;
            PSCHK(dev_grow(p->d_H, p->H_cap, (uint64_t)N * N));
            HIPCHK(hipMemsetAsync(p->d_H, 0, (uint64_t)N * N * sizeof(uint32_t), st));
            const uint32_t tile_pairs = ntile * (ntile + 1u) / 2u;
            const uint32_t n_chunks = (rows + WA * 8u - 1u) / (WA * 8u);
            uint32_t ranges = std::max(1u, std::min(n_chunks, (256u * 16u + tile_pairs - 1u) / tile_pairs));
            const uint32_t cpr = (n_chunks + ranges - 1u) / ranges;
            ranges = (n_chunks + cpr - 1u) / cpr;
            core_allpairs_kernel<<<dim3(tile_pairs, ranges), 256, lds, st>>>(p->state, N, p->pitch, rows, p->d_H, WA,
                                                                          cpr, ntile);
            core_pair_lookup_kernel<<<(uint32_t)((P + 255) / 256), 256, 0, st>>>(p->d_H, N, d_r1, d_r2, d_perm, P, d_a);
        } else if (p->onehot_safe && W && p->pair_mode != 3) {
            p->last_pair_form = PS_PAIR_FORM_TILED2;
            constexpr int A = 32;
            constexpr uint32_t PT = 1024;
            const uint32_t n_tiles = (rows + W * 16 - 1) / (W * 16);
            const uint64_t need = (uint64_t)n_tiles * N * W;
            PSCHK(dev_grow(p->d_pack2, p->pack2_cap, need));
            const uint32_t pack_lds = N * W * 4u;
            if (pack_lds > 64 * 1024)
                HIPCHK(hipFuncSetAttribute((const void *)core_pack2_kernel, hipFuncAttributeMaxDynamicSharedMemorySize, (int)pack_lds));
            hipLaunchKernelGGL(core_pack2_kernel, dim3(n_tiles), dim3(PT), pack_lds, st, p->state, N, p->pitch, rows, p->d_pack2, W);
            const uint32_t lds = N * ((W >> 2) + 1u) * 16u;
            auto kern = core_pair_counts_packed2<A>;
            if (lds > 64 * 1024)
                HIPCHK(hipFuncSetAttribute((const void *)kern, hipFuncAttributeMaxDynamicSharedMemorySize, (int)lds));
            const uint32_t pair_blocks = std::max(1u, (p->pair_threads + PT - 1) / PT);
            uint32_t ranges = std::max(1u, std::min(n_tiles, p->pair_ranges ? p->pair_ranges : (256u * 4u + pair_blocks - 1) / pair_blocks));
            const uint32_t max_tpr = std::max(1u, 65535u / (W * 16u));
            ranges = std::max(ranges, (n_tiles + max_tpr - 1) / max_tpr);
            const uint32_t tpr = (n_tiles + ranges - 1) / ranges;
            ranges = (n_tiles + tpr - 1) / tpr;
            uint32_t *part = nullptr;
            PSCHK(pair_partials(p, (uint64_t)ranges * P, &part));
            hipLaunchKernelGGL(kern, dim3(pair_blocks, ranges), dim3(PT), lds, st, p->d_pack2, N, n_tiles, d_r1, d_r2,
                               (uint32_t)P, d_r1 + 5 * P, d_r1 + 6 * P, p->pair_threads, part, W, tpr);
            core_pair_reduce_kernel<<<(uint32_t)((P + 255) / 256), 256, 0, st>>>(part, ranges, (uint32_t)P, d_perm, d_a);
        } else if (p->nibble_safe && W) {
            p->last_pair_form = PS_PAIR_FORM_TILED4;
            constexpr int A = 32;
            constexpr uint32_t PT = 1024;
            const uint32_t lds = N * ((W >> 2) + 1u) * 16u;
            auto kern = core_pair_counts_tiled<A>;
            if (lds > 64 * 1024)
                HIPCHK(hipFuncSetAttribute((const void *)kern, hipFuncAttributeMaxDynamicSharedMemorySize, (int)lds));
            const uint32_t n_tiles = (rows + W * 8 - 1) / (W * 8);
            const uint32_t pair_blocks = std::max(1u, (p->pair_threads + PT - 1) / PT);
            uint32_t ranges = std::max(1u, std::min(n_tiles, p->pair_ranges ? p->pair_ranges : (256u * 4u + pair_blocks - 1) / pair_blocks));
            const uint32_t max_tpr = std::max(1u, 16383u / (W * 8u));
            ranges = std::max(ranges, (n_tiles + max_tpr - 1) / max_tpr);
            const uint32_t tpr = (n_tiles + ranges - 1) / ranges;
            ranges = (n_tiles + tpr - 1) / tpr;
            uint32_t *part = nullptr;
            PSCHK(pair_partials(p, (uint64_t)ranges * P, &part));
            hipLaunchKernelGGL(kern, dim3(pair_blocks, ranges), dim3(PT), lds, st, p->state, N, p->pitch,
                               rows, d_r1, d_r2, (uint32_t)P, d_r1 + 5 * P, d_r1 + 6 * P, p->pair_threads, part, W, tpr);
            core_pair_reduce_kernel<<<(uint32_t)((P + 255) / 256), 256, 0, st>>>(part, ranges, (uint32_t)P, d_perm, d_a);
        } else {
            p->last_pair_form = PS_PAIR_FORM_SIMPLE;
            const uint32_t slices = std::max(1u, std::min(rows, 64u));
            const uint32_t rps = (rows + slices - 1) / slices;
            dim3 grid((uint32_t)((P + 255) / 256), (rows + rps - 1) / rps);
            core_pair_counts_simple<<<grid, 256, 0, st>>>(p->state, p->pitch, rows, d_r1, d_r2, d_perm, P, d_a, rps);
        }
    } else {
        const bool all = p->pair_mode != 1 && (uint64_t)N * N * 4 <= (2ull << 30)
                         && (p->pair_mode == 2 || (double)P * 4.0 > (double)N * (double)N);
        if (all) {
            PSCHK(dev_grow(p->d_H, p->H_cap, (uint64_t)N * N + N));
            uint32_t *rowcnt = p->d_H + (uint64_t)N * N;
            const uint32_t nt = (N + 63u) / 64u;
            acc_pair_inter_tiled_kernel<<<dim3(nt, nt), 256, 0, st>>>(p->I[p->cur], p->d_H, rowcnt, p->d);
            acc_pair_lookup_kernel<<<(uint32_t)((P + 255) / 256), 256, 0, st>>>(p->d_H, rowcnt, N, d_r1, d_r2, d_perm, P, d_a, d_b);
        } else {
            acc_pair_counts_kernel<<<(uint32_t)((P * 8 + 255) / 256), 256, 0, st>>>(p->I[p->cur], d_r1, d_r2, d_perm, P,
                                                                             d_a, d_b, p->d);
        }
    }
    HIPCHK(hipGetLastError());
    return PS_OK;
}

__global__ void __launch_bounds__(256) pairs_map_kernel(const uint32_t *r1, const uint32_t *r2, const uint32_t *slot, uint32_t *m1,
                                                        uint32_t *m2, uint64_t P)
{
    const uint64_t k = (uint64_t)blockIdx.x * blockDim.x + threadIdx.x;
    if (k >= P) return;
    m1[k] = slot[r1[k]];
    m2[k] = slot[r2[k]];
}

static int pairs_for_launch(ps_population *p, uint64_t P, const uint32_t *r1, const uint32_t *r2, bool trusted, const uint32_t *slot,
                            uint32_t **d_r1, uint32_t **d_r2, hipStream_t st)
{
    const bool dev_map = slot && !core_pairs_take_a_tiled_kernel(p, P);
    if (slot && !dev_map) {
        std::vector<uint32_t> m1(P), m2(P);
        for (uint64_t k = 0; k < P; k++) { m1[k] = slot[r1[k]]; m2[k] = slot[r2[k]]; }
        PSCHK(upload_pairs(p, P, m1.data(), m2.data()));
    } else {
        PSCHK(upload_pairs(p, P, r1, r2, trusted));
    }
    uint32_t *d = (uint32_t *)p->d_pairs;
    *d_r1 = d;
    *d_r2 = d + P;
    if (dev_map) {
        *d_r1 = d + 7 * P;
        *d_r2 = d + 8 * P;
        pairs_map_kernel<<<(uint32_t)((P + 255) / 256), 256, 0, st>>>(d, d + P, p->d_row_slot, *d_r1, *d_r2, P);
        HIPCHK(hipGetLastError());
    }
    return PS_OK;
}

extern "C" int ps_pairwise_counts(ps_population *p, uint64_t P, const uint32_t *range1, const uint32_t *range2,
                                  uint32_t *out_a, uint32_t *out_b, int out_is_device)
{
    if (!p || !range1 || !range2 || !out_a) return ps_fail(PS_ERR_INVALID, "null argument");
    if (!p->cfg.core && !out_b) return ps_fail(PS_ERR_INVALID, "out_b is required for the accessory matrix");
    if (P == 0) return PS_OK;
    const uint64_t N = p->cfg.pop_size;
    for (uint64_t k = 0; k < P; k++)
        if (range1[k] >= N || range2[k] >= N)
            return ps_fail(PS_ERR_INVALID, "pair %llu out of range", (unsigned long long)k);
    PSCHK(use_device(p));
    const uint32_t *slot = nullptr;
    PSCHK(rows_current(p, &slot));
    uint32_t *d_r1 = nullptr, *d_r2 = nullptr;
    PSCHK(pairs_for_launch(p, P, range1, range2, false, slot, &d_r1, &d_r2, p->stream));
    uint32_t *d_perm = (uint32_t *)p->d_pairs + 2 * P, *d_a = d_perm + P, *d_b = d_a + P;
    uint32_t *ka = out_is_device ? out_a : d_a;
    uint32_t *kb = out_is_device ? out_b : d_b;
    PSCHK(pair_counts_device(p, P, d_r1, d_r2, d_perm, ka, kb, p->stream));
    if (!out_is_device) {
        HIPCHK(hipMemcpyAsync(out_a, d_a, P * 4, hipMemcpyDeviceToHost, p->stream));
        if (!p->cfg.core) HIPCHK(hipMemcpyAsync(out_b, d_b, P * 4, hipMemcpyDeviceToHost, p->stream));
    }
    HIPCHK(hipStreamSynchronize(p->stream));
    return PS_OK;
}

extern "C" int ps_last_sweep_form(ps_population *p)
{
    if (!p) return ps_fail(PS_ERR_INVALID, "null handle");
    return p->last_sweep_form;
}

extern "C" int ps_last_pair_form(ps_population *p) { return p ? p->last_pair_form : 0; }

extern "C" int ps_pairwise_distances(ps_population *p, uint64_t P, const uint32_t *range1,
                                     const uint32_t *range2, double *out)
{
    if (!p || !out) return ps_fail(PS_ERR_INVALID, "null argument");
    std::vector<uint32_t> a(P), b(P);
    PSCHK(ps_pairwise_counts(p, P, range1, range2, a.data(), b.data(), 0));
    const double ncols = (double)p->cfg.ncols, cg = (double)p->cfg.core_genes;
    for (uint64_t k = 0; k < P; k++) {
        if (p->cfg.core) {
            const uint32_t distance = a[k] / 2;
            out[k] = (double)distance / ncols;
        } else {
            out[k] = 1.0 - (((double)a[k] + cg) / ((double)b[k] + cg));
        }
    }
    return PS_OK;
}

static const uint64_t PS_CDAVG_SCRATCH = 1ull << 30;

struct core_davg_bands { uint32_t c0, c_end, band; uint64_t ld; };

static core_davg_bands core_davg_plan_bands(const ps_population *p, uint64_t first, uint64_t count)
{
    const uint64_t N = p->cfg.pop_size;
    core_davg_bands b;
    b.c0 = (uint32_t)(first & ~255ull);
    b.c_end = (uint32_t)(first + count);
    b.ld = (N + 63) & ~63ull;
    const uint64_t span = ((uint64_t)(b.c_end - b.c0) + 255) & ~255ull;
    const uint64_t band = p->core_davg_band ? ((uint64_t)p->core_davg_band + 255) & ~255ull
                                            : std::max<uint64_t>(256, (PS_CDAVG_SCRATCH / b.ld) & ~255ull);
    b.band = (uint32_t)std::min<uint64_t>(std::min<uint64_t>(band, span), 65280);
    return b;
}

struct core_site_list { const uint32_t *d = nullptr; uint32_t n = 0; };

static int core_davg_pack(ps_population *p, const uint32_t *d_slot, hipStream_t st, uint32_t *WT_out, core_site_list list = {})
{
    const uint32_t N = (uint32_t)p->cfg.pop_size, rows = list.d ? list.n : (uint32_t)p->cfg.ncols;
    if (list.d && (d_slot || !rows)) return ps_fail(PS_ERR_STATE, "the strings of a site list are packed in internal order from at least one site");
    const uint32_t WT = ((rows + 15u) / 16u + PS_PT_WB - 1u) / PS_PT_WB * PS_PT_WB;
    const uint64_t need = (uint64_t)((N + 31u) / 32u * 32u) * WT;
    PSCHK(dev_grow(p->d_pack2, p->pack2_cap, need));
    const uint64_t ptiles = (uint64_t)((N + PS_PT_IB - 1u) / PS_PT_IB) * (WT / PS_PT_WB);
    if (ptiles > 0x7FFFFFFFull) return ps_fail(PS_ERR_INVALID, "matrix too large for the transposed distance form");
    if (list.d) core_packT_kernel<false, true, false, false, true><<<dim3((uint32_t)ptiles), 256, 0, st>>>(p->state, N, p->pitch, rows, p->d_pack2, WT, list.d);
    else if (d_slot) core_packT_kernel<false, true, false, true><<<dim3((uint32_t)ptiles), 256, 0, st>>>(p->state, N, p->pitch, rows, p->d_pack2, WT, d_slot);
    else core_packT_kernel<false, true><<<dim3((uint32_t)ptiles), 256, 0, st>>>(p->state, N, p->pitch, rows, p->d_pack2, WT);
    HIPCHK(hipGetLastError());
    *WT_out = WT;
    return PS_OK;
}

static int core_davg_whole(ps_population *p, bool onehot, const uint32_t *d_slot, uint64_t first, uint64_t count, double *d_out,
                           hipStream_t st)
{
    const uint32_t N = (uint32_t)p->cfg.pop_size, rows = (uint32_t)p->cfg.ncols;
    const double L = (double)p->cfg.global_cols;
    const uint32_t grid = (uint32_t)(((first & 15u) + count + 15u) / 16u);
    if (onehot) {
        uint32_t WT = 0;
        PSCHK(core_davg_pack(p, d_slot, st, &WT));
        const uint32_t ntile = (N + PS_MF_TILE - 1u) / PS_MF_TILE, tile_pairs = ntile * (ntile + 1u) / 2u, n_chunks = WT / PS_MF_CHUNK_DW;
        uint32_t ranges = mfma_allpairs_ranges(N, n_chunks, tile_pairs);
        const uint32_t cpr = (n_chunks + ranges - 1u) / ranges;
        ranges = (n_chunks + cpr - 1u) / cpr;
        PSCHK(dev_grow(p->d_H, p->H_cap, (uint64_t)N * N * ranges));
        const uint32_t lds = 256u * 16u * 16u;
        if ((uint64_t)cpr * PS_MF_CHUNK_DW * 16u < (1u << 24)) {
            HIPCHK(hipFuncSetAttribute((const void *)core_allpairs_mfma_fp4_kernel<false>, hipFuncAttributeMaxDynamicSharedMemorySize, (int)lds));
            hipLaunchKernelGGL(core_allpairs_mfma_fp4_kernel<false>, dim3(tile_pairs, ranges), dim3(512), lds, st, p->d_pack2, WT, N, p->d_H, cpr, n_chunks, ntile);
        } else {
            HIPCHK(hipFuncSetAttribute((const void *)core_allpairs_mfma_kernel, hipFuncAttributeMaxDynamicSharedMemorySize, (int)lds));
            hipLaunchKernelGGL(core_allpairs_mfma_kernel, dim3(tile_pairs, ranges), dim3(512), lds, st, p->d_pack2, WT, N, p->d_H, cpr, n_chunks, ntile);
        }
        if (ranges > 1u) core_allpairs_sum_slices_kernel<<<N, 256, 0, st>>>(p->d_H, N, ranges);
        core_average_from_h_kernel<8u><<<grid, 320, 0, st>>>(p->d_H, N, (uint32_t)first, (uint32_t)count, L, d_out);
    } else {
        const uint32_t WA = 32u, ntile = (N + 127u) / 128u;
        const uint32_t lds = 2u * 128u * ((WA >> 2) + 1u) * 16u;
        PSCHK(dev_grow(p->d_H, p->H_cap, (uint64_t)N * N));
        HIPCHK(hipMemsetAsync(p->d_H, 0, (uint64_t)N * N * sizeof(uint32_t), st));
        const uint32_t tile_pairs = ntile * (ntile + 1u) / 2u;
        const uint32_t n_chunks = (rows + WA * 8u - 1u) / (WA * 8u);
        uint32_t ranges = std::max(1u, std::min(n_chunks, (256u * 16u + tile_pairs - 1u) / tile_pairs));
        const uint32_t cpr = (n_chunks + ranges - 1u) / ranges;
        ranges = (n_chunks + cpr - 1u) / cpr;
        core_allpairs_kernel<<<dim3(tile_pairs, ranges), 256, lds, st>>>(p->state, N, p->pitch, rows, p->d_H, WA, cpr, ntile);
        core_average_from_h_kernel<7u><<<grid, 320, 0, st>>>(p->d_H, N, (uint32_t)first, (uint32_t)count, L, d_out);
    }
    HIPCHK(hipGetLastError());
    return PS_OK;
}

struct core_davg_src { bool fp4; uint32_t WT, n_chunks, ranges, cpr; const uint32_t *slot; uint32_t sites; };

static int core_davg_prepare(ps_population *p, const core_davg_bands &b, bool fp4, const uint32_t *d_slot, hipStream_t st,
                             core_davg_src *o, core_site_list list = {})
{
    const uint32_t N = (uint32_t)p->cfg.pop_size, rows = list.d ? list.n : (uint32_t)p->cfg.ncols;
    if (list.d && !fp4) return ps_fail(PS_ERR_INVALID, "the resampled form of the core strings exists for one-hot matrices only");
    *o = core_davg_src{ fp4 && rows > 0, 0, 0, 1, 0, d_slot, rows };
    const uint64_t slice = (uint64_t)b.band * b.ld;
    if (o->fp4) {
        PSCHK(core_davg_pack(p, d_slot, st, &o->WT, list));
        o->n_chunks = o->WT / PS_MF_CHUNK_DW;
        const uint32_t ntile = (N + PS_MF_TILE - 1u) / PS_MF_TILE, blocks = b.band / PS_MF_TILE * ntile;
        const uint32_t rmin = (o->n_chunks + 131070u) / 131071u;
        uint32_t r = std::min(o->n_chunks, std::max(rmin, (1024u + blocks - 1u) / blocks));
        r = std::max(rmin, std::min(r, (uint32_t)std::max<uint64_t>(1, PS_CDAVG_SCRATCH / slice)));
        o->cpr = (o->n_chunks + r - 1u) / r;
        o->ranges = (o->n_chunks + o->cpr - 1u) / o->cpr;
    }
    const uint64_t need = slice * o->ranges;
    PSCHK(dev_grow(p->d_cdavg, p->cdavg_cap, need));
    return PS_OK;
}

static int core_davg_band_counts(ps_population *p, const core_davg_src &src, const core_davg_bands &b, uint32_t lo, uint32_t nrows,
                                 hipStream_t st)
{
    const uint32_t N = (uint32_t)p->cfg.pop_size, rows = src.sites;
    uint32_t *C = p->d_cdavg;
    const uint64_t n = (uint64_t)nrows * b.ld, slice = (uint64_t)b.band * b.ld;
    if (rows == 0) {
        HIPCHK(hipMemsetAsync(C, 0, n * sizeof(uint32_t), st));
    } else if (src.fp4) {
        const uint32_t ntile = (N + PS_MF_TILE - 1u) / PS_MF_TILE, rtiles = (nrows + PS_MF_TILE - 1u) / PS_MF_TILE;
        const uint32_t lds = 256u * 16u * 16u;
        HIPCHK(hipFuncSetAttribute((const void *)core_allpairs_mfma_fp4_kernel<true>, hipFuncAttributeMaxDynamicSharedMemorySize, (int)lds));
        hipLaunchKernelGGL(core_allpairs_mfma_fp4_kernel<true>, dim3(rtiles * ntile, src.ranges), dim3(512), lds, st, p->d_pack2, src.WT, N,
                           C, src.cpr, src.n_chunks, ntile, lo / PS_MF_TILE, lo + nrows, b.ld, slice);
        for (uint32_t r = 1; r < src.ranges; r++)
            u32_add_kernel<<<(uint32_t)((n + 255) / 256), 256, 0, st>>>(C, C + r * slice, n);
    } else {
        core_band_counts_simple<<<dim3((N + 255u) / 256u, nrows), 256, 0, st>>>(p->state, p->pitch, rows, N, src.slot, lo, C, b.ld);
    }
    HIPCHK(hipGetLastError());
    return PS_OK;
}

static int core_davg_band_fold(const uint32_t *C, const core_davg_bands &b, uint32_t N, uint32_t lo, uint32_t nrows, uint64_t first,
                               double L, double *d_out, hipStream_t st)
// ... 502 lines not shown
static double zig_exp_1(ref_std_rng &rng, const double *xt, const double *ft)
{
    for (;;) {
        const uint64_t bits = rng.next_u64();
        const unsigned i = (unsigned)(bits & 0xff);
        const double u = (double)(bits >> 11) / 9007199254740992.0;
        const double x = u * xt[i];
        if (x < xt[i + 1]) return x;
        if (i == 0) return 7.69711747013104972 - std::log(rng.gen_f64());
        if (ft[i + 1] + (ft[i] - ft[i + 1]) * rng.gen_f64() < std::exp(-x)) return x;
    }
}

extern "C" int ps_reference_selection_coefficients(uint64_t seed, uint64_t G, double prop_positive, double pos_lambda,
                                                   double neg_lambda, double *out)
{
    if (!out && G) return ps_fail(PS_ERR_INVALID, "null output");
    for (uint64_t g = 0; g < G; g++) out[g] = 0.0;
    if (!(prop_positive >= 0.0)) return PS_OK;
    if (!(pos_lambda > 0.0) || !(neg_lambda > 0.0)) return ps_fail(PS_ERR_INVALID, "Exp::new(lambda).unwrap() panics for lambda <= 0");
    static double xt[257], ft[257];
    static std::once_flag once;
    std::call_once(once, [] { zig_exp_tables(xt, ft); });
    ref_std_rng rng(seed);
    for (uint64_t g = 0; g < G; g++) {
        const double weight = rng.uniform01();
        double s;
        if (weight <= prop_positive) {
            s = zig_exp_1(rng, xt, ft) / pos_lambda;
        } else {
            s = zig_exp_1(rng, xt, ft) / neg_lambda;
            while (s > 1.0) s = zig_exp_1(rng, xt, ft) / neg_lambda;
            s = -1.0 * s;
        }
        out[g] = s;
    }
    return PS_OK;
}

extern "C" int ps_sample_pairs(uint64_t seed, uint64_t N, uint64_t P, uint32_t *range1, uint32_t *range2)
{
    if (!range1 || !range2) return ps_fail(PS_ERR_INVALID, "null output");
    if (N < 2) return ps_fail(PS_ERR_INVALID, "pair sampling needs pop_size >= 2 (main.rs:421 panics)");
    for (uint64_t k = 0; k < P; k++)
        range1[k] = ps_mulhi(hs_u32(seed, PS_STREAM_PAIRS, 0, k), (uint32_t)N);
    for (uint64_t k = 0; k < P; k++) {
        uint32_t e = ps_mulhi(hs_u32(seed, PS_STREAM_PAIRS, 1, k), (uint32_t)(N - 1));
        if (e >= range1[k]) e += 1;
        range2[k] = e;
    }
    return PS_OK;
}

#define PS_RING 8
struct ps_sim {
    ps_sim_params prm{};
    ps_derived der{};
    ps_population *core = nullptr, *acc = nullptr;
    std::vector<double> sel;
    std::vector<uint32_t> r1, r2;
    uint32_t *d_idx[PS_RING] = {};
    uint32_t *h_idx[PS_RING] = {};
    uint32_t *m_idx[PS_RING] = {};
    hipEvent_t ev_idx[PS_RING] = {}, ev_core[PS_RING] = {};
    hipEvent_t ev_hgt = nullptr;
    hipEvent_t ev_gap[PS_RING][2] = {};
    std::vector<uint32_t> h_kids;
    uint32_t *h_draw[PS_RING] = {};
    uint32_t *m_draw[PS_RING] = {};
    int prev_slot = -1;
    std::vector<uint32_t> sigma, sigma_prev_inv;
    uint64_t sigma_step = ~0ull;
    bool heavy_hgt = false;
    bool slot_used[PS_RING] = {};
    int last_sweep_slot = -1;
    int32_t *h_num_genes = nullptr, *m_num_genes = nullptr;
    double *h_logw = nullptr, *m_logw = nullptr, *h_avg = nullptr;
    double *d_avg = nullptr;
    bool avg_prefetched = false;
    uint64_t avg_epoch = 0;
    hipEvent_t ev_avg = nullptr;
    std::vector<double> h_w;
    hipEvent_t ev_bin = nullptr;
    double *d_log1p = nullptr;
    uint64_t step_count = 0;
    uint64_t gens_done = 0;
    bool need_logw = false;
    bool device_draw = false;
    double *h_cum = nullptr, *d_cum = nullptr;
    uint32_t *d_idx_tsum = nullptr;
    uint32_t *d_idx_cnt = nullptr;
    int last_slot = 0;
    uint32_t *d_anc = nullptr;
    uint32_t anc_capacity = 0;
    uint64_t anc_written = 0;
    uint32_t *h_cnt = nullptr;
    uint64_t h_cnt_cap = 0;
    hipEvent_t ev_dist[4] = {};
    double dist_core_ms = 0.0, dist_acc_ms = 0.0;
    uint64_t host_calls = 0;
    double host_wait_ms = 0.0, host_weights_ms = 0.0, host_draw_ms = 0.0;
    int (*weights_hook)(void *ctx, ps_sim *s, uint32_t gen, double *w) = nullptr;
    void *weights_ctx = nullptr;
    int emu_shards = 0;
    void *emu_buf = nullptr;
    uint64_t emu_cap = 0;
    uint32_t emu_clock_khz = 0;
    double emu_link_gbps = 153.0, emu_latency_us = 20.0, emu_modelled_us = 0.0;
    uint64_t exchange_calls = 0, exchange_bytes = 0;
    bool timing = false;
    std::vector<std::pair<hipEvent_t, hipEvent_t>> tev;
    std::vector<hipEvent_t> ev_pool;
};

extern "C" void ps_sim_destroy(ps_sim *s)
{
    if (!s) return;
    if (s->core) (void)hipSetDevice(s->core->device);
    if (s->core) (void)hipStreamSynchronize(s->core->stream);
    if (s->acc) (void)hipStreamSynchronize(s->acc->stream);
    for (int k = 0; k < PS_RING; k++) {
        if (s->d_idx[k]) (void)hipFree(s->d_idx[k]);
        if (s->h_idx[k]) (void)hipHostFree(s->h_idx[k]);
        if (s->h_draw[k]) (void)hipHostFree(s->h_draw[k]);
        if (s->ev_idx[k]) (void)hipEventDestroy(s->ev_idx[k]);
        if (s->ev_core[k]) (void)hipEventDestroy(s->ev_core[k]);
        if (k == 0 && s->ev_hgt) (void)hipEventDestroy(s->ev_hgt);
        if (k == 0 && s->ev_avg) (void)hipEventDestroy(s->ev_avg);
        if (k == 0 && s->ev_bin) (void)hipEventDestroy(s->ev_bin);
        for (int j = 0; j < 2; j++) if (s->ev_gap[k][j]) (void)hipEventDestroy(s->ev_gap[k][j]);
    }
    if (s->h_num_genes) (void)hipHostFree(s->h_num_genes);
    if (s->h_logw) (void)hipHostFree(s->h_logw);
    if (s->h_avg) (void)hipHostFree(s->h_avg);
    if (s->h_cum) (void)hipHostFree(s->h_cum);
    if (s->d_cum) (void)hipFree(s->d_cum);
    if (s->d_idx_cnt) (void)hipFree(s->d_idx_cnt);
    if (s->d_idx_tsum) (void)hipFree(s->d_idx_tsum);
    if (s->d_anc) (void)hipFree(s->d_anc);
    if (s->h_cnt) (void)hipHostFree(s->h_cnt);
    for (auto e : s->ev_dist) if (e) (void)hipEventDestroy(e);
    if (s->d_avg) (void)hipFree(s->d_avg);
    if (s->emu_buf) (void)hipFree(s->emu_buf);
    if (s->d_log1p) (void)hipFree(s->d_log1p);
    for (auto &pr : s->tev) { (void)hipEventDestroy(pr.first); (void)hipEventDestroy(pr.second); }
    for (auto e : s->ev_pool) (void)hipEventDestroy(e);
    ps_population_destroy(s->core);
    ps_population_destroy(s->acc);
    delete s;
}

static int sim_refresh_rows(void *ctx);
static uint32_t sim_sweep_generations(ps_sim *s);

static int sim_create_impl(const ps_sim_params *p, ps_sim *s)
{
    char msg[1024];
    if (ps_sim_validate(p, msg, sizeof msg) != PS_OK) return ps_fail(PS_ERR_INVALID, "%s", msg);
    if (p->shard_count < 1 || p->shard_rank < 0 || p->shard_rank >= p->shard_count)
        return ps_fail(PS_ERR_INVALID, "bad shard %d of %d", p->shard_rank, p->shard_count);
    if (p->pop_size < 2) return ps_fail(PS_ERR_INVALID, "pop_size must be >= 2 (main.rs:421 / population.rs:584 panic)");
    s->prm = *p;
    PSCHK(ps_sim_derive(p, &s->der));
    const ps_derived &d = s->der;
    const uint64_t N = p->pop_size, L = p->core_size, G = d.pan_size;
    s->sel.assign(std::max<uint64_t>(G, 1), 0.0);
    if (p->reference_seed_stream)
        PSCHK(ps_reference_selection_coefficients(p->seed, G, p->prop_positive, p->pos_lambda, p->neg_lambda, s->sel.data()));
    else
        PSCHK(ps_selection_coefficients(p->seed, G, p->prop_positive, p->pos_lambda, p->neg_lambda, s->sel.data()));
    for (uint64_t g = 0; g < G; g++)
        if (std::log(1.0 + s->sel[g]) != 0.0) s->need_logw = true;
    const uint64_t sb = L * (uint64_t)p->shard_rank / (uint64_t)p->shard_count;
    const uint64_t se = L * ((uint64_t)p->shard_rank + 1) / (uint64_t)p->shard_count;
    ps_config cc{};
    cc.pop_size = N; cc.ncols = se - sb; cc.global_cols = L; cc.col_offset = sb;
    cc.core_genes = p->core_genes; cc.seed = p->seed; cc.core = 1; cc.device = p->device;
    {
        std::vector<uint8_t> v(std::max<uint64_t>(cc.ncols, 1));
        PSCHK(ps_init_vector(p->seed, 1, sb, cc.ncols, 0.0, v.data()));
        PSCHK(ps_population_create(&cc, v.data(), &s->core));
    }
    ps_config ca{};
    ca.pop_size = N; ca.ncols = G; ca.global_cols = G; ca.col_offset = 0;
    ca.core_genes = p->core_genes; ca.seed = p->seed; ca.core = 0; ca.device = s->core->device;
    {
        std::vector<uint8_t> v(std::max<uint64_t>(G, 1));
        PSCHK(ps_init_vector(p->seed, 0, 0, G, d.avg_gene_freq_adj, v.data()));
        PSCHK(ps_population_create(&ca, v.data(), &s->acc));
    }
    s->core->rows_refresh = s->acc->rows_refresh = sim_refresh_rows;
    s->core->rows_ctx = s->acc->rows_ctx = s;
    {
        const uint64_t b0 = 0, e0 = L;
        const double lm = d.n_core_mutations;
        const double lr = (p->HR_rate > 0.0) ? d.n_recombinations_core : 0.0;
        PSCHK(ps_set_rates(s->core, 1, &lm, &lr, &b0, &e0));
        double lrec[2] = { 0, 0 };
        for (int c = 0; c < d.n_comp; c++) lrec[c] = (p->HGT_rate > 0.0) ? d.n_recombinations_pan[c] : 0.0;
        PSCHK(ps_set_rates(s->acc, d.n_comp, d.n_pan_mutations, lrec, d.comp_begin, d.comp_end));
    }
    s->r1.resize(p->max_distances);
    s->r2.resize(p->max_distances);
    PSCHK(ps_sample_pairs(p->seed, N, p->max_distances, s->r1.data(), s->r2.data()));
    PSCHK(use_device(s->core));
    for (int k = 0; k < PS_RING; k++) {
        HIPCHK(hipMalloc(&s->d_idx[k], N * sizeof(uint32_t)));
        HIPCHK(hipHostMalloc(&s->h_idx[k], N * sizeof(uint32_t), hipHostMallocMapped));
        HIPCHK(hipHostGetDevicePointer((void **)&s->m_idx[k], s->h_idx[k], 0));
        HIPCHK(hipHostMalloc(&s->h_draw[k], N * sizeof(uint32_t), hipHostMallocMapped));
        HIPCHK(hipHostGetDevicePointer((void **)&s->m_draw[k], s->h_draw[k], 0));
        HIPCHK(hipEventCreateWithFlags(&s->ev_idx[k], hipEventDisableTiming));
        HIPCHK(hipEventCreateWithFlags(&s->ev_core[k], hipEventDisableTiming));
    }
    if (p->max_distances > 0) {
        PSCHK(upload_pairs(s->core, p->max_distances, s->r1.data(), s->r2.data(), true));
        PSCHK(upload_pairs(s->acc, p->max_distances, s->r1.data(), s->r2.data(), true));
    }
    if (!wave_sweep_eligible(s->core, true, p->HR_rate > 0.0)) {
        core_block_geom g{};
        uint32_t lds = 0, nw = 0;
        if (block_sweep_geometry(s->core, true, true, p->HR_rate > 0.0, &g, &lds, &nw))
            s->acc->hgt_list_in_global = lds + 16384u > s->core->lds_limit;
    }
    {
        const double bytes = 2.0 * (double)N * (double)s->core->cfg.ncols;
        double ept;
        if (sim_sweep_generations(s) >= 2u) {
            const double per_gen_ms = bytes / 4.0e12 * 1e3 / 2.0;
            ept = std::min((per_gen_ms - 0.222) / 0.445e-3, 192.0);
        } else {
            const double sweep_ms = bytes / 4.2e12 * 1e3;
            ept = std::min((sweep_ms - 0.3) / 1.0e-3 * 0.5, 112.0);
        }
        s->acc->hgt_events_per_thread = ept >= 16.0 ? (uint32_t)ept : 0u;
        if (const char *e = getenv("PANSIM_HGT_EVENTS_PER_THREAD")) s->acc->hgt_events_per_thread = (uint32_t)atoi(e);
    }
    HIPCHK(hipEventCreateWithFlags(&s->ev_hgt, hipEventDisableTiming));
    {
        const uint32_t parts = hgt_partitions(s->acc);
        s->heavy_hgt = (double)N * s->der.n_recombinations_pan_total >= 7.5e6 && parts >= 1 && parts <= 1024;
    }
    if (const char *e = getenv("PANSIM_HEAVY_HGT")) s->heavy_hgt = atoi(e) != 0;
    if (!getenv("PANSIM_SWEEP_BLOCKS_PER_CU")) {
        uint64_t max_comp = 0;
        for (int c = 0; c < d.n_comp; c++) max_comp = std::max<uint64_t>(max_comp, d.comp_end[c] - d.comp_begin[c]);
        const uint64_t list_lds = 2 * max_comp;
        if (list_lds > 36 * 1024) s->acc->hgt_list_in_global = true;
        const uint32_t light = 4u;
        s->core->sweep_blocks_per_cu = list_lds <= 16 * 1024 ? light : std::min(light, 6u);
    }
    HIPCHK(hipHostMalloc(&s->h_num_genes, N * sizeof(int32_t), hipHostMallocMapped));
    HIPCHK(hipHostMalloc(&s->h_logw, N * sizeof(double), hipHostMallocMapped));
    HIPCHK(hipHostGetDevicePointer((void **)&s->m_num_genes, s->h_num_genes, 0));
    HIPCHK(hipHostGetDevicePointer((void **)&s->m_logw, s->h_logw, 0));
    HIPCHK(hipHostMalloc(&s->h_avg, N * sizeof(double)));
    s->device_draw = N >= 4096;
    if (const char *e = getenv("PANSIM_DEVICE_DRAW")) s->device_draw = atoi(e) != 0;
    HIPCHK(hipHostMalloc(&s->h_cum, N * sizeof(double)));
    HIPCHK(hipMalloc(&s->d_cum, N * sizeof(double)));
    HIPCHK(hipMalloc(&s->d_idx_tsum, ((N + 1023) / 1024 + 1) * sizeof(uint32_t)));
    HIPCHK(hipMalloc(&s->d_idx_cnt, N * sizeof(uint32_t)));
    HIPCHK(hipMemset(s->d_idx_cnt, 0, N * sizeof(uint32_t)));
    HIPCHK(hipMalloc(&s->d_avg, N * sizeof(double)));
    if (G) {
        std::vector<double> l1p(G);
        for (uint64_t g = 0; g < G; g++) l1p[g] = std::log(1.0 + s->sel[g] * 1.0);
        HIPCHK(hipMalloc(&s->d_log1p, G * sizeof(double)));
        HIPCHK(hipMemcpy(s->d_log1p, l1p.data(), G * sizeof(double), hipMemcpyHostToDevice));
    }
    if (G && !s->need_logw && !(getenv("PANSIM_FUSE_COUNTS") && atoi(getenv("PANSIM_FUSE_COUNTS")) == 0)) {
        s->acc->fuse_counts_out = s->m_num_genes;
        s->acc->fuse_logw_out = s->m_logw;
    }
    return PS_OK;
}

extern "C" int ps_sim_create(const ps_sim_params *p, ps_sim **out)
{
    if (!p || !out) return ps_fail(PS_ERR_INVALID, "null argument");
    *out = nullptr;
    ps_sim *s = new ps_sim();
    const int rc = sim_create_impl(p, s);
    if (rc != PS_OK) {
        const std::string keep = g_err;
        ps_sim_destroy(s);
        g_err = keep;
        return rc;
    }
    *out = s;
    return PS_OK;
}

static int sim_average_distance(ps_sim *s)
{
    ps_population *acc = s->acc;
    const uint64_t N = s->prm.pop_size;
    hipStream_t sa = acc->stream;
    const bool sharded = acc->exchange && acc->donor_cnt != 0 && acc->d.G > 0 && N >= 2;
    if (!sharded) return average_distance_device(acc, s->d_avg, sa);
    HIPCHK(hipMemsetAsync(s->d_avg, 0, N * sizeof(double), sa));
    PSCHK(average_distance_device(acc, s->d_avg, sa, acc->donor_lo, acc->donor_cnt));
    const std::string prev = g_err;
    g_err.clear();
    const int rc = acc->exchange(acc->exchange_ctx, s->d_avg, N, (void *)sa);
    if (rc != 0) {
        const std::string inner = g_err;
        return ps_fail(PS_ERR_STATE, "the all-gather of the average distances failed (%d)%s%s", rc, inner.empty() ? "" : ": ", inner.c_str());
    }
    g_err = prev;
    return PS_OK;
}

static int sim_host_weights(ps_sim *s, uint32_t gen, double *w, bool avg_ready = false)
{
    (void)gen;
    ps_population *acc = s->acc;
    const ps_sim_params &p = s->prm;
    const uint64_t N = p.pop_size;
    hipStream_t sa = acc->stream;
    using clk = std::chrono::steady_clock;
    auto ms_since = [](clk::time_point t0) { return std::chrono::duration<double, std::milli>(clk::now() - t0).count(); };
    for (uint64_t i = 0; i < N; i++) s->h_avg[i] = 1.0;
    if (p.competition_strength > 0.0) {
        const bool ahead = s->avg_prefetched && s->avg_epoch == acc->edit_epoch;
        if (!avg_ready && !ahead) PSCHK(sim_average_distance(s));
        s->avg_prefetched = false;
        HIPCHK(hipMemcpyAsync(s->h_avg, s->d_avg, N * sizeof(double), hipMemcpyDeviceToHost, sa));
    }
    if (s->need_logw)
        acc_fitness_kernel<<<(uint32_t)((N + 255) / 256), 256, 0, sa>>>(acc->I[acc->cur], s->d_log1p, 1,
                                                                     s->m_num_genes, s->m_logw, acc->d);
    else if (!acc->counts_fresh)
        acc_gene_count_rows_kernel<<<(uint32_t)((N + 3) / 4), 256, 0, sa>>>(acc->I[acc->cur], s->m_num_genes,
                                                                         s->m_logw, acc->d);
    HIPCHK(hipGetLastError());
    auto th0 = clk::now();
    HIPCHK(hipStreamSynchronize(sa));
    s->host_wait_ms += ms_since(th0);
    th0 = clk::now();
    PSCHK(ps_sample_weights(s->h_num_genes, s->h_logw, N, acc->cfg.ncols, s->der.avg_gene_num, s->h_avg,
                            p.no_control_genome_size, p.genome_size_penalty, p.competition_strength, w));
    s->host_weights_ms += ms_since(th0);
    return PS_OK;
}

static int sim_light_hgt(ps_sim *s, uint32_t gen)
{
    const bool heavy_hgt = s->prm.HGT_rate > 0.0 && s->heavy_hgt;
    if (s->prm.HGT_rate > 0.0 && !heavy_hgt) PSCHK(launch_acc_hgt(s->acc, gen, s->acc->stream));
    return PS_OK;
}

static int sim_accessory_half(ps_sim *s, uint32_t gen, uint32_t gens, bool light_hgt)
{
    ps_population *core = s->core, *acc = s->acc;
    const ps_sim_params &p = s->prm;
    const uint64_t N = p.pop_size, G = acc->cfg.ncols;
    hipStream_t sa = acc->stream, sc = core->stream;
    const int slot = (int)(s->step_count % PS_RING);
    using clk = std::chrono::steady_clock;
    auto ms_since = [](clk::time_point t0) { return std::chrono::duration<double, std::milli>(clk::now() - t0).count(); };
    auto th0 = clk::now();
    {
        const int back = (int)std::min<uint32_t>(4u * gens, PS_RING);
        const int wslot = (slot + PS_RING - back) % PS_RING;
        if (s->slot_used[wslot]) HIPCHK(hipEventSynchronize(s->ev_core[wslot]));
    }
    s->host_wait_ms += ms_since(th0);
    std::vector<double> &w = s->h_w;
    w.resize(N);
    if (s->weights_hook) PSCHK(s->weights_hook(s->weights_ctx, s, gen, w.data()));
    else PSCHK(sim_host_weights(s, gen, w.data()));
    th0 = clk::now();
    s->prev_slot = s->step_count ? s->last_slot : -1;
    s->last_slot = slot;
    if (core->rows_overridden || acc->rows_overridden) s->anc_written = 0;
    core->rows_overridden = acc->rows_overridden = false;
    const bool want_snap = p.HGT_rate > 0.0 && !hgt_takes_binned_form(acc);
    if (s->device_draw) {
        double total = w[0];
        for (uint64_t i = 1; i < N; i++) { s->h_cum[i - 1] = total; total += w[i]; }
        HIPCHK(hipMemcpyAsync(s->d_cum, s->h_cum, (N - 1) * sizeof(double), hipMemcpyHostToDevice, sa));
        acc_draw_parents_kernel<<<(uint32_t)((N + 255) / 256), 256, 0, sa>>>(s->d_cum, total, (uint32_t)N, (uint32_t)p.seed,
                                                                         (uint32_t)(p.seed >> 32), gen, s->d_idx_cnt, s->m_draw[slot]);
        {
            const uint32_t tiles = (uint32_t)((N + 1023) / 1024);
            idx_tile_sums_kernel<<<tiles, 256, 0, sa>>>(s->d_idx_cnt, (uint32_t)N, s->d_idx_tsum);
            idx_tile_prefix_kernel<<<1, 256, 0, sa>>>(s->d_idx_tsum, tiles);
            idx_scan_kernel<<<tiles, 256, 0, sa>>>(s->d_idx_cnt, (uint32_t)N, s->d_idx_tsum);
        }
        idx_fill_kernel<<<(uint32_t)((N + 255) / 256), 256, 0, sa>>>(s->d_idx_cnt, (uint32_t)N, s->d_idx[slot], s->m_idx[slot]);
        idx_zero_kernel<<<(uint32_t)((N + 255) / 256), 256, 0, sa>>>(s->d_idx_cnt, (uint32_t)N);
        HIPCHK(hipGetLastError());
        s->host_draw_ms += ms_since(th0);
        s->host_calls++;
        PSCHK(launch_acc_step(acc, s->d_idx[slot], gen, true, true, sa, nullptr, want_snap));
    } else {
    PSCHK(ps_draw_parents(w.data(), N, p.seed, gen, s->h_idx[slot]));
    memcpy(s->h_draw[slot], s->h_idx[slot], N * sizeof(uint32_t));
    {
        s->h_kids.assign(N, 0u);
        uint32_t *ix = s->h_idx[slot];
        for (uint64_t k = 0; k < N; k++) s->h_kids[ix[k]]++;
        uint64_t j = 0;
        for (uint64_t par = 0; par < N; par++)
            for (uint32_t c = s->h_kids[par]; c; c--) ix[j++] = (uint32_t)par;
    }
    s->host_draw_ms += ms_since(th0);
    s->host_calls++;
    if (G == 0) HIPCHK(hipMemcpyAsync(s->d_idx[slot], s->h_idx[slot], N * sizeof(uint32_t), hipMemcpyHostToDevice, sa));
    PSCHK(launch_acc_step(acc, s->m_idx[slot], gen, true, true, sa, s->d_idx[slot], want_snap));
    }
    HIPCHK(hipEventRecord(s->ev_idx[slot], sa));
    if (s->anc_capacity) {
        HIPCHK(hipMemcpyAsync(s->d_anc + (s->anc_written % s->anc_capacity) * N, s->d_idx[slot], N * sizeof(uint32_t), hipMemcpyDeviceToDevice, sa));
        s->anc_written++;
    }
    const bool heavy_hgt = p.HGT_rate > 0.0 && s->heavy_hgt;
    if (heavy_hgt) {
        const int prev = s->last_sweep_slot;
        HIPCHK(hipEventRecord(s->ev_hgt, sa));
        static const bool gap_on_core = getenv("PANSIM_GAP_ON_CORE_STREAM") && atoi(getenv("PANSIM_GAP_ON_CORE_STREAM")) != 0;
        if (gap_on_core && !s->ev_bin) HIPCHK(hipEventCreateWithFlags(&s->ev_bin, hipEventDisableTiming));
        PSCHK(launch_acc_hgt(acc, gen, sa, prev >= 0 ? s->ev_core[prev] : nullptr, s->ev_hgt, gap_on_core ? sc : nullptr, s->ev_bin));
        HIPCHK(hipStreamWaitEvent(sc, s->ev_hgt, 0));
    }

    {
        const bool sharded_rows = acc->exchange && acc->donor_cnt != 0;
        const bool big_davg = acc->d.G > 0 && N >= 2 && (sharded_rows || N > 8192 || acc->davg_form >= 2) && acc->davg_form != 1;
        static const bool off = getenv("PANSIM_DAVG_AHEAD") && atoi(getenv("PANSIM_DAVG_AHEAD")) == 0;
        if (!off && p.competition_strength > 0.0 && big_davg && (heavy_hgt || p.HGT_rate <= 0.0) && (int64_t)gen + 1 != (int64_t)p.n_gen) {
            PSCHK(sim_average_distance(s));
            s->avg_prefetched = true;
            s->avg_epoch = acc->edit_epoch;
            if (!s->ev_avg) HIPCHK(hipEventCreateWithFlags(&s->ev_avg, hipEventDisableTiming));
            HIPCHK(hipEventRecord(s->ev_avg, sa));
            HIPCHK(hipStreamWaitEvent(sc, s->ev_avg, 0));
        }
    }

    if (light_hgt) PSCHK(sim_light_hgt(s, gen));
    s->step_count++;
    return PS_OK;
}

static int sim_core_half(ps_sim *s, uint32_t first, uint32_t gens)
{
    ps_population *core = s->core;
    const ps_sim_params &p = s->prm;
    hipStream_t sc = core->stream;
    int slots[PS_SWEEP_MAX_GENS];
    for (uint32_t t = 0; t < gens; t++) slots[t] = (int)((s->step_count + PS_RING - gens + t) % PS_RING);
    const int slot = slots[gens - 1u];
    HIPCHK(hipStreamWaitEvent(sc, s->ev_idx[slot], 0));
    hipEvent_t t0 = nullptr, t1 = nullptr;
    if (s->timing) {
        auto take = [&](hipEvent_t *e) -> int {
            if (!s->ev_pool.empty()) { *e = s->ev_pool.back(); s->ev_pool.pop_back(); return PS_OK; }
            HIPCHK(hipEventCreate(e));
            return PS_OK;
        };
        PSCHK(take(&t0));
        PSCHK(take(&t1));
        HIPCHK(hipEventRecord(t0, sc));
    } else {
        if (!s->ev_gap[slot][0]) {
            HIPCHK(hipEventCreate(&s->ev_gap[slot][0]));
            HIPCHK(hipEventCreate(&s->ev_gap[slot][1]));
        }
        HIPCHK(hipEventRecord(s->ev_gap[slot][0], sc));
    }
    const uint32_t *next[PS_SWEEP_MAX_GENS] = {};
    for (uint32_t t = 1; t < gens; t++) next[t - 1u] = s->d_idx[slots[t]];
    PSCHK(launch_core_sweep(core, s->d_idx[slots[0]], first, true, true, p.HR_rate > 0.0, sc, true, gens, next));
    if (s->timing) {
        HIPCHK(hipEventRecord(t1, sc));
        s->tev.emplace_back(t0, t1);
    } else {
        HIPCHK(hipEventRecord(s->ev_gap[slot][1], sc));
    }
    for (uint32_t t = 0; t < gens; t++) {
        HIPCHK(hipEventRecord(s->ev_core[slots[t]], sc));
        s->slot_used[slots[t]] = true;
    }
    s->last_sweep_slot = slot;
    return PS_OK;
}

static uint32_t sim_sweep_generations(ps_sim *s)
{
    ps_population *core = s->core;
    if (core->cfg.ncols == 0 || !core->cplan.has_events) return 1u;
    if (!wave_sweep_eligible(core, true, s->prm.HR_rate > 0.0)) return 1u;
    if (core->sweep_generations) return std::min<uint32_t>(core->sweep_generations, PS_SWEEP_MAX_GENS);
    return 2u;
}

static int sim_generations(ps_sim *s, uint32_t first, uint32_t gens, uint32_t depth)
{
    for (uint32_t t = 0; t < gens; t++) PSCHK(sim_accessory_half(s, first + t, depth, t + 1u < gens));
    PSCHK(sim_core_half(s, first, gens));
    return sim_light_hgt(s, first + gens - 1u);
}

static void sim_exchange_schedule(ps_sim *s)
{
    const char *e = getenv("PANSIM_EXCHANGE_BESIDE_SWEEP");
    const bool on = e && atoi(e) != 0 && s->acc->exchange != nullptr;
    s->acc->exchange_beside_sweep = on;
    if (s->acc->exchange != nullptr && s->core->window_blocks_per_cu == 0 && !getenv("PANSIM_WINDOW_BPC")) s->core->window_blocks_per_cu = 5;
}

extern "C" int ps_sim_set_exchange(ps_sim *s, ps_exchange_fn fn, void *ctx)
{
    if (!s) return ps_fail(PS_ERR_INVALID, "null handle");
    if (s->prm.shard_count < 2) return ps_fail(PS_ERR_INVALID, "the HGT donors are sharded over the site shards of a run: shard_count must be >= 2");
    PSCHK(ps_set_donor_shard(s->acc, (uint32_t)s->prm.shard_rank, (uint32_t)s->prm.shard_count, fn, ctx));
    sim_exchange_schedule(s);
    return PS_OK;
}

extern "C" int ps_sim_set_site_weights(ps_sim *s, const float *w_core, const float *w_acc_mut, const float *w_acc_rec)
{
    if (!s) return ps_fail(PS_ERR_INVALID, "null handle");
    if ((w_acc_mut == nullptr) != (w_acc_rec == nullptr))
        return ps_fail(PS_ERR_INVALID, "the accessory weights come as a pair (mutation and recombination)");
    PSCHK(ps_sim_sync(s));
    const ps_sim_params &p = s->prm;
    const ps_derived &d = s->der;
    if (w_core) {
        const double lm = d.n_core_mutations;
        const double lr = (p.HR_rate > 0.0) ? d.n_recombinations_core : 0.0;
        PSCHK(ps_set_site_rates(s->core, 1, &lm, &lr, w_core, nullptr));
    }
    if (w_acc_mut) {
        double lrec[2] = { 0, 0 };
        for (int c = 0; c < d.n_comp; c++) lrec[c] = (p.HGT_rate > 0.0) ? d.n_recombinations_pan[c] : 0.0;
        PSCHK(ps_set_site_rates(s->acc, d.n_comp, d.n_pan_mutations, lrec, w_acc_mut, w_acc_rec));
        if (s->acc->site_weighted && (uint64_t)hgt_list_u16(s->acc, (uint32_t)s->acc->d.G) * 2u > 36u * 1024u) s->acc->hgt_list_in_global = true;
    }
    return PS_OK;
}

extern "C" int ps_multi_set_site_weights(ps_multi *m, const float *w_core, const float *w_acc_mut, const float *w_acc_rec)
{
    (void)m; (void)w_core; (void)w_acc_mut; (void)w_acc_rec;
    return ps_fail(PS_ERR_INVALID, "ps_multi runs have no per-site weights yet: drive one ps_sim per shard and call ps_sim_set_site_weights");
}

__global__ void __launch_bounds__(256) emu_hold_kernel(unsigned long long ticks)
{
    __shared__ uint32_t pad[19744 / 4];
    pad[threadIdx.x] = threadIdx.x;
    asm volatile("v_mov_b32 v255, 0\n\tv_accvgpr_write_b32 a7, 0" ::: "v255", "a7");
    const unsigned long long t0 = wall_clock64();
    while (wall_clock64() - t0 < ticks) __builtin_amdgcn_s_sleep(64);
    if (pad[(threadIdx.x + 1u) & 255u] == 0xFFFFFFFFu) __builtin_trap();
}

static int emulated_exchange(void *ctx, void *d_words, uint64_t n_words, void *hip_stream)
{
    ps_sim *s = (ps_sim *)ctx;
    const uint64_t bytes = n_words * 8;
    PSCHK(dev_grow(s->emu_buf, s->emu_cap, bytes));
    if (s->emu_clock_khz == 0) {
        int khz = 0, dev = 0;
        HIPCHK(hipGetDevice(&dev));
        if (hipDeviceGetAttribute(&khz, hipDeviceAttributeWallClockRate, dev) != hipSuccess || khz <= 0) khz = 100000;
        s->emu_clock_khz = (uint32_t)khz;
        const char *e = getenv("PANSIM_EMU_XGMI_GBPS");
        if (e && atof(e) > 0.0) s->emu_link_gbps = atof(e);
        e = getenv("PANSIM_EMU_COLL_LATENCY_US");
        if (e && atof(e) >= 0.0) s->emu_latency_us = atof(e);
    }
    const uint64_t part = bytes / (uint64_t)s->emu_shards * (uint64_t)(s->emu_shards - 1);
    static const bool ring = getenv("PANSIM_EMU_RING") && atoi(getenv("PANSIM_EMU_RING")) != 0;
    const double slice = (double)bytes / (double)s->emu_shards;
    const double a2a_us = s->emu_latency_us + slice / (s->emu_link_gbps * 1e3);
    const double gather_us = ring ? s->emu_latency_us + (double)part / (s->emu_link_gbps * 1e3) : a2a_us;
    const unsigned long long ticks = (unsigned long long)(a2a_us * 1e-6 * (double)s->emu_clock_khz * 1e3);
    const unsigned long long ticks2 = (unsigned long long)(gather_us * 1e-6 * (double)s->emu_clock_khz * 1e3);
    hipStream_t st = (hipStream_t)hip_stream;
    HIPCHK(hipMemcpyAsync(s->emu_buf, d_words, part, hipMemcpyDeviceToDevice, st));
    emu_hold_kernel<<<8, 256, 0, st>>>(ticks);
    HIPCHK(hipMemcpyAsync((uint8_t *)s->emu_buf + (bytes - part), (uint8_t *)d_words + (bytes - part), part,
                          hipMemcpyDeviceToDevice, st));
    emu_hold_kernel<<<8, 256, 0, st>>>(ticks2);
    HIPCHK(hipGetLastError());
    if (d_words == (void *)s->d_avg) {
        const uint64_t own = n_words / (uint64_t)s->emu_shards;
        for (uint64_t k = 1; own && k * own < n_words; k++)
            HIPCHK(hipMemcpyAsync((uint64_t *)d_words + k * own, d_words, std::min(own, n_words - k * own) * 8, hipMemcpyDeviceToDevice, st));
    }
    s->exchange_calls++;
    s->exchange_bytes += 2 * part;
    s->emu_modelled_us += a2a_us + gather_us;
    return PS_OK;
}

extern "C" int ps_sim_emulate_exchange(ps_sim *s, int n_shards)
{
    if (!s) return ps_fail(PS_ERR_INVALID, "null handle");
    if (n_shards < 2) return ps_fail(PS_ERR_INVALID, "n_shards must be >= 2");
    s->emu_shards = n_shards;
    PSCHK(ps_set_donor_shard(s->acc, 0u, (uint32_t)n_shards, emulated_exchange, s));
    sim_exchange_schedule(s);
    return PS_OK;
}

extern "C" int ps_sim_exchange_stats(ps_sim *s, int reset, uint64_t *calls, uint64_t *bytes)
{
    if (!s) return ps_fail(PS_ERR_INVALID, "null handle");
    if (calls) *calls = s->exchange_calls;
    if (bytes) *bytes = s->exchange_bytes;
    if (reset) s->exchange_calls = s->exchange_bytes = 0;
    return PS_OK;
}

extern "C" int ps_sim_emulated_link_time(ps_sim *s, int reset, double *modelled_us, double *link_gbps, double *latency_us)
{
    if (!s) return ps_fail(PS_ERR_INVALID, "null handle");
    if (modelled_us) *modelled_us = s->emu_modelled_us;
    if (link_gbps) *link_gbps = s->emu_link_gbps;
    if (latency_us) *latency_us = s->emu_latency_us;
    if (reset) s->emu_modelled_us = 0.0;
    return PS_OK;
}

extern "C" int ps_sim_run(ps_sim *s, uint32_t first_generation, uint32_t count)
{
    if (!s) return ps_fail(PS_ERR_INVALID, "null handle");
    PSCHK(use_device(s->core));
    if ((uint64_t)first_generation != s->gens_done) s->anc_written = 0;
    const uint32_t T = sim_sweep_generations(s);
    uint32_t g = 0;
    for (; g + T <= count; g += T) PSCHK(sim_generations(s, first_generation + g, T, T));
    for (; g < count; g++) PSCHK(sim_generations(s, first_generation + g, 1u, T));
    s->gens_done = (uint64_t)first_generation + count;
    return PS_OK;
}

extern "C" int ps_sim_sync(ps_sim *s)
{
    if (!s) return ps_fail(PS_ERR_INVALID, "null handle");
    PSCHK(use_device(s->core));
    HIPCHK(hipStreamSynchronize(s->acc->stream));
    HIPCHK(hipStreamSynchronize(s->core->stream));
    PSCHK(check_device_flag(s->acc));
    return check_device_flag(s->core);
}

extern "C" ps_population *ps_sim_core(ps_sim *s) { return s ? s->core : nullptr; }
extern "C" ps_population *ps_sim_acc(ps_sim *s) { return s ? s->acc : nullptr; }
extern "C" const double *ps_sim_selection(ps_sim *s) { return s ? s->sel.data() : nullptr; }
extern "C" const uint32_t *ps_sim_range1(ps_sim *s) { return s ? s->r1.data() : nullptr; }
extern "C" const uint32_t *ps_sim_range2(ps_sim *s) { return s ? s->r2.data() : nullptr; }

static void stable_rank(const uint32_t *draw, uint64_t N, std::vector<uint32_t> &start, uint32_t *rank)
{
    start.assign(N + 1, 0u);
    for (uint64_t k = 0; k < N; k++) start[draw[k] + 1]++;
    for (uint64_t i = 0; i < N; i++) start[i + 1] += start[i];
    for (uint64_t k = 0; k < N; k++) rank[k] = start[draw[k]]++;
}

static int sim_refresh_rows(void *ctx)
{
    ps_sim *s = (ps_sim *)ctx;
    if (s->sigma_step == s->step_count) return PS_OK;
    const uint64_t N = s->prm.pop_size;
    PSCHK(use_device(s->core));
    HIPCHK(hipStreamSynchronize(s->acc->stream));
    std::vector<uint32_t> start;
    s->sigma.clear();
    s->sigma_prev_inv.clear();
    if (s->step_count) {
        s->sigma.resize(N);
        stable_rank(s->h_draw[s->last_slot], N, start, s->sigma.data());
        if (s->prev_slot >= 0) {
            std::vector<uint32_t> sp(N);
            stable_rank(s->h_draw[s->prev_slot], N, start, sp.data());
            s->sigma_prev_inv.resize(N);
            for (uint64_t k = 0; k < N; k++) s->sigma_prev_inv[sp[k]] = (uint32_t)k;
        }
    }
    for (ps_population *p : { s->core, s->acc }) {
        p->row_slot = s->sigma;
        if (!s->sigma.empty()) {
            if (!p->d_row_slot) HIPCHK(hipMalloc(&p->d_row_slot, N * sizeof(uint32_t)));
            HIPCHK(hipMemcpyAsync(p->d_row_slot, s->sigma.data(), N * sizeof(uint32_t), hipMemcpyHostToDevice, p->stream));
            HIPCHK(hipStreamSynchronize(p->stream));
        }
// ... 740 lines not shown
```

### pansim_amd/population.py

```python
import ctypes as C

import numpy as np

from . import _lib
from ._lib import PS_GROUPS_MAX, ClusterParams, Clusters, Config, CoreDiversity, Diff, DiffParams, Knn, KnnParams, Lineages, PairHist, PairHistParams, Tree, TreeParams, Upgma, check


def _u32(a):
    return np.ascontiguousarray(a, dtype=np.uint32)


def _f64(a):
    return np.ascontiguousarray(a, dtype=np.float64)


def hamming_bitwise_fast(x, y):
    x = np.ascontiguousarray(x, np.uint8)
    y = np.ascontiguousarray(y, np.uint8)
    if x.size != y.size:
        raise ValueError("slices must have the same length (distances.rs:24 assert_eq)")
    out = C.c_uint32()
    check(_lib.load().ps_hamming_bitwise_fast(x, y, x.size, C.byref(out)))
    return out.value

# ... 556 lines not shown
                                site_within=within[:L], site_total=total[:L], counts=c, gene_counts=None, acc_between=None,
                                gene_fixed=None, gene_private=None)


def draw_parents(weights, seed, generation):
    w = _f64(weights)
    idx = np.zeros(w.size, np.uint32)
    check(_lib.load().ps_draw_parents(w, w.size, int(seed), int(generation), idx))
    return idx


class Population:

    def __init__(self, size, allele_count, max_variants, core, avg_gene_freq, seed, core_genes,
                 acc_sampling_vec=None, *, col_offset=0, global_cols=None, device=-1, init_vec=None,
                 _handle=None, _owned=True):
        self._lib = _lib.load()
        self.core = bool(core)
        self.size = int(size)
        self.ncols = int(allele_count)
        self.core_genes = int(core_genes)
        self.seed = int(seed)
        self.global_cols = self.ncols if global_cols is None else int(global_cols)
        self._owned = _owned
        if _handle is not None:
            self._h = C.c_void_p(_handle)
            return
        if self.core and max_variants != 4:
            raise ValueError("core populations use 4 variants (main.rs:375)")
        cfg = Config(self.size, self.ncols, self.global_cols, int(col_offset), self.core_genes,
                     self.seed, int(self.core), int(device))
        if init_vec is None:
            init_vec = init_vector(seed, core, self.ncols, avg_gene_freq, col_offset)
        init_vec = np.ascontiguousarray(init_vec, np.uint8)
        if init_vec.size != self.ncols:
            raise ValueError("init_vec must have allele_count entries")
        self._h = C.c_void_p()
        check(self._lib.ps_population_create(C.byref(cfg), init_vec.ctypes.data_as(C.c_void_p),
                                             C.byref(self._h)))

    def close(self):
        if getattr(self, "_h", None) and self._h.value and self._owned:
            self._lib.ps_population_destroy(self._h)
        self._h = C.c_void_p()

    def __del__(self):
        try:
            self.close()
        except Exception:
            pass

    def load_matrix(self, rows):
        rows = np.ascontiguousarray(rows, np.uint8)
        if rows.shape != (self.size, self.ncols):
            raise ValueError("matrix must be (size, allele_count)")
        check(self._lib.ps_load_matrix(self._h, rows))

    def read_matrix(self):
        out = np.zeros((self.size, self.ncols), np.uint8)
        check(self._lib.ps_read_matrix(self._h, out))
        return out

    def set_rates(self, mutations_vec, recombinations_vec, comp_begin=None, comp_end=None):
        lm, lr = _f64(mutations_vec), _f64(recombinations_vec)
        if comp_begin is None:
            comp_begin, comp_end = [0], [self.global_cols]
        b = np.ascontiguousarray(comp_begin, np.uint64)
        e = np.ascontiguousarray(comp_end, np.uint64)
        check(self._lib.ps_set_rates(self._h, lm.size, lm, lr, b, e))

    def set_site_rates(self, mutations_vec, recombinations_vec, mutation_weights, recombination_weights=None):
        lm, lr = _f64(mutations_vec), _f64(recombinations_vec)
        if lr.size != lm.size:
            raise ValueError("one recombination rate per mutation rate")
        wm = _weights(mutation_weights, lm.size, self.global_cols, "mutation")
        wr = _weights(recombination_weights, lm.size, self.global_cols, "recombination")
        if wm is None:
            raise ValueError("mutation weights are required")
        check(self._lib.ps_set_site_rates(self._h, lm.size, lm, lr, _ptr(wm), _ptr(wr)))

    def next_generation(self, sample):
        s = _u32(sample)
        if s.size != self.size:
            raise ValueError("sample must have one parent per individual")
        check(self._lib.ps_next_generation(self._h, s))

    def mutate_alleles(self, generation):
        check(self._lib.ps_mutate_alleles(self._h, int(generation)))

    def recombine(self, generation):
        check(self._lib.ps_recombine(self._h, int(generation)))

    def step(self, generation, sample, do_recombine=True):
        s = _u32(sample)
        check(self._lib.ps_step(self._h, int(generation), s, int(bool(do_recombine))))

    def sample_indices(self, generation, avg_gene_num, avg_pairwise_dists, selection_coefficients,
                       verbose=False, no_control_genome_size=False, genome_size_penalty=0.99,
                       competition_strength=0.0):
        idx = np.zeros(self.size, np.uint32)
        check(self._lib.ps_sample_indices(self._h, int(generation), int(avg_gene_num),
                                          _f64(avg_pairwise_dists), _f64(selection_coefficients),
                                          int(verbose), int(no_control_genome_size),
                                          float(genome_size_penalty), float(competition_strength), idx))
        return idx

    def fitness_terms(self, selection_coefficients):
        ng = np.zeros(self.size, np.int32)
        lw = np.zeros(self.size, np.float64)
        check(self._lib.ps_fitness_terms(self._h, _f64(selection_coefficients), ng, lw))
        return ng, lw

    def average_distance(self):
        out = np.zeros(self.size, np.float64)
        check(self._lib.ps_average_distance(self._h, out))
        return out

    def average_distance_rows(self, first, count):
        out = np.zeros(int(count), np.float64)
        check(self._lib.ps_average_distance_rows(self._h, int(first), int(count), out))
        return out

    def pairwise_distances(self, max_distances, range1, range2):
        r1, r2 = _u32(range1)[:max_distances], _u32(range2)[:max_distances]
        out = np.zeros(int(max_distances), np.float64)
        check(self._lib.ps_pairwise_distances(self._h, int(max_distances), np.ascontiguousarray(r1),
                                              np.ascontiguousarray(r2), out))
        return out

    def pairwise_counts(self, range1, range2):
        r1, r2 = _u32(range1), _u32(range2)
        a = np.zeros(r1.size, np.uint32)
        b = np.zeros(r1.size, np.uint32)
        check(self._lib.ps_pairwise_counts(self._h, r1.size, r1, r2, a.ctypes.data_as(C.c_void_p),
                                           b.ctypes.data_as(C.c_void_p), 0))
        return (a,) if self.core else (a, b)

    def pairwise_counts_device(self, range1, range2, out_a_ptr, out_b_ptr=0):
        r1, r2 = _u32(range1), _u32(range2)
        check(self._lib.ps_pairwise_counts(self._h, r1.size, r1, r2, C.c_void_p(out_a_ptr),
                                           C.c_void_p(out_b_ptr), 1))

    def set_donor_shard(self, shard_rank, shard_count, fn=None):
        ptr = C.cast(fn, C.c_void_p) if fn is not None else None
        self._exchange_fn = fn
        check(self._lib.ps_set_donor_shard(self._h, int(shard_rank), int(shard_count), ptr, None))

    def last_pair_form(self):
        return int(self._lib.ps_last_pair_form(self._h))

    def last_sweep_form(self):
        return int(self._lib.ps_last_sweep_form(self._h))

    def gene_frequencies(self):
        out = np.zeros(self.ncols + self.core_genes, np.float64)
        check(self._lib.ps_gene_frequencies(self._h, out))
        return out

    def site_allele_counts(self):
        out = np.zeros((self.ncols, 4), np.uint32)
        check(self._lib.ps_site_allele_counts(self._h, _ptr(out)))
        return out

    def core_diversity(self, spectrum=False):
        return _diversity_call(self._lib.ps_core_diversity, self.size, spectrum, self._h)

    def distance_histogram(self, acc, core_bins=64, acc_bins=64, core_max=None, core_span=None):
        prm = _hist_params(core_bins, acc_bins, core_max, self.global_cols, core_span)
        return _hist_call(self._lib.ps_distance_histogram, prm, self._h, acc._h)

    def distance_histogram_timing(self):
        return _timing(self._lib.ps_distance_histogram_timing, 2, self._h)

    def strain_clusters(self, acc, core_max=None, acc_max=None, core_max_d=None, acc_ratio=None):
        prm = _cluster_params(self.global_cols, core_max, acc_max, core_max_d, acc_ratio)
        return _cluster_call(self._lib.ps_strain_clusters, prm, self.size, self._h, acc._h)

    def linkage_tree(self, acc, metric="core"):
        return _tree_call(self._lib.ps_linkage_tree, _tree_params(metric), self.size, self._h, acc._h)

    def upgma_tree(self, acc, metric="core"):
        return _upgma_call(self._lib.ps_upgma_tree, _tree_params(metric), self.size, self._h, acc._h)

    def upgma_tree_timing(self):
        return _timing(self._lib.ps_upgma_tree_timing, 3, self._h)

    def neighbour_joining(self, acc, metric="core"):
        from .joining import _nj_call
        return _nj_call(self._lib.ps_neighbour_joining, _tree_params(metric), self.size, self._h, acc._h)

    def neighbour_joining_timing(self):
        return _timing(self._lib.ps_neighbour_joining_timing, 3, self._h)

    def bootstrap_support(self, acc, method="nj", replicates=100, seed=0, draws=None, sites=None):
        from .bootstrap import _boot_call
        return _boot_call(self._lib.ps_bootstrap_support, self.size, method, replicates, seed, draws, sites, self._h, acc._h)

    def bootstrap_support_timing(self):
        return _timing(self._lib.ps_bootstrap_timing, 3, self._h)

    def nearest_neighbours(self, acc, k, metric="core"):
        return _knn_call(self._lib.ps_nearest_neighbours, _knn_params(k, metric), self.size, self._h, acc._h)

    def nearest_neighbours_timing(self):
        return _timing(self._lib.ps_nearest_neighbours_timing, 2, self._h)

    def linkage_tree_timing(self):
        return _timing(self._lib.ps_linkage_tree_timing, 3, self._h)

    def strain_clusters_timing(self):
        return _timing(self._lib.ps_strain_clusters_timing, 3, self._h)

    def group_differentiation(self, labels, acc=None, max_groups=16, min_size=1, per_site=False, counts=False):
        return _diff_call(self._lib.ps_group_differentiation, labels, self.size, self.ncols, acc.ncols if acc is not None else 0,
                          max_groups, min_size, per_site, counts, acc is not None, self._h, acc._h if acc is not None else None)

    def group_differentiation_timing(self):
        return _timing(self._lib.ps_group_differentiation_timing, 3, self._h)

    def tree_parsimony(self, left, right, acc=None, per_site=False, branches=False, genes=False):
        from .parsimony import _pars_call
        if genes and acc is None:
            raise ValueError("genes=True needs the accessory population")
        return _pars_call(self._lib.ps_tree_parsimony, left, right, self.size, self.ncols, acc.ncols if genes else 0, per_site, branches,
                          genes, self._h, acc._h if acc is not None else None)

    def tree_parsimony_timing(self):
        return _timing(self._lib.ps_tree_parsimony_timing, 3, self._h)

    def tree_nni(self, left, right, max_rounds=1000, moves_per_round=0):
        from .search import _nni_call
        return _nni_call(self._lib.ps_tree_nni, left, right, self.size, max_rounds, moves_per_round, self._h)

    def nni_deltas(self, left, right):
        from .search import _deltas_call
        return _deltas_call(self._lib.ps_tree_nni_deltas, left, right, self._h)

    def tree_nni_timing(self):
        return _timing(self._lib.ps_tree_nni_timing, 2, self._h)

    def tree_likelihood(self, left, right, lengths, per_site=False, derivatives=False):
        from .likelihood import _lik_call
        return _lik_call(self._lib.ps_tree_likelihood, left, right, lengths, self.size, self.ncols, per_site, derivatives, self._h)

    def tree_ml_lengths(self, left, right, lengths=None, max_rounds=50, eps_lnl=1e-3):
        from .likelihood import _ml_call, _start_lengths
        if lengths is None:
            lengths = _start_lengths(self, left, right)
        return _ml_call(self._lib.ps_tree_ml_lengths, left, right, lengths, self.size, max_rounds, eps_lnl, self._h)

    def tree_likelihood_timing(self):
        return _timing(self._lib.ps_tree_likelihood_timing, 3, self._h)

    def tree_model_likelihood(self, left, right, lengths, model, per_site=False, derivatives=False):
        from .models import _model_call
        return _model_call(self._lib.ps_tree_model_likelihood, left, right, lengths, model, self.size, self.ncols, per_site, derivatives, self._h)

    def tree_model_ml_lengths(self, left, right, model, lengths=None, max_rounds=50, eps_lnl=1e-3):
        from .models import _model_ml_call, _model_start_lengths
        if lengths is None:
            lengths = _model_start_lengths(self, left, right, model)
        return _model_ml_call(self._lib.ps_tree_model_ml_lengths, left, right, lengths, model, self.size, max_rounds, eps_lnl, self._h)

    def model_nni_deltas(self, left, right, lengths, model):
        from .ml_search import _deltas_call
        return _deltas_call(self._lib.ps_tree_model_nni_deltas, left, right, lengths, model, self.size, self._h)

    def tree_model_nni(self, left, right, model, lengths=None, max_rounds=1000, moves_per_round=0, length_rounds=5, eps_gain=1e-3):
        from .ml_search import _search_call
        from .models import _model_start_lengths
        if lengths is None:
            lengths = _model_start_lengths(self, left, right, model)
        return _search_call(self._lib.ps_tree_model_nni, left, right, lengths, model, self.size, max_rounds, moves_per_round, length_rounds,
                            eps_gain, self._h)

    def tree_model_nni_timing(self):
        return _timing(self._lib.ps_tree_model_nni_timing, 3, self._h)

    def tree_model_timing(self):
        return _timing(self._lib.ps_tree_model_timing, 3, self._h)

    def ancestral_states(self, left, right, lengths, model, min_posterior=0.0, states=True):
        from .ancestral import _device_call
        return _device_call(self._lib.ps_tree_ancestral_states, self, self.ncols, left, right, lengths, model, self.size, min_posterior, states, self._h)

    def ancestral_states_timing(self):
        return _timing(self._lib.ps_ancestral_states_timing, 3, self._h)

    def tree_gene_likelihood(self, left, right, lengths, model, per_gene=False):
        from .gene_model import _lik_call
        return _lik_call(self._lib.ps_tree_gene_likelihood, left, right, lengths, model, self.size, self.ncols, per_gene, self._h)

    def tree_gene_ancestral(self, left, right, lengths, model, states=True):
        from .gene_model import _anc_device_call
        return _anc_device_call(self._lib.ps_tree_gene_ancestral, self, left, right, lengths, model, self.size, states, self._h)

    def tree_gene_fit(self, left, right, lengths, model, fit_rates=True, fit_freq=True, fit_weights=True, max_rounds=50, eps_lnl=1e-3):
        from .gene_model import _fit_call
        return _fit_call(self._lib.ps_tree_gene_fit, left, right, lengths, model, self.size, fit_rates, fit_freq, fit_weights, max_rounds,
                         eps_lnl, self._h)

    def tree_gene_timing(self):
        return _timing(self._lib.ps_tree_gene_timing, 3, self._h)

    def tree_compare(self, a, b, bins=(32, 32), spans=(0, 0), triplets=True, values=None):
        from .tree_compare import _compare_call
# ... 58 lines not shown
```

Baseline: 3220.

## Process two row batches per pass in the two-generation wave sweep

Adds a PAIR variant of the two-generation wave sweep kernel that stages 8 rows (two batches) in LDS per pass. Both batches share one queue push/scan, and homologous-recombination donor values are held in registers instead of a parked queue half. Host code picks pass geometry from LDS room, the HGT list reserve and the expected queue size, and launches the paired kernel when it fits. The aim is to amortise the per-batch scan, sync and event-pass overhead. In exchange it uses more LDS per wave, which can cut occupancy, and it moves the HGT tuning computation after block selection.

```diff
diff --git a/pansim_amd/csrc/core_kernels.h b/pansim_amd/csrc/core_kernels.h
--- a/pansim_amd/csrc/core_kernels.h
+++ b/pansim_amd/csrc/core_kernels.h
@@ -2,6 +2,8 @@
 
 #include "ps_common.h"
 
+#include <algorithm>
+#include <cmath>
 #include <type_traits>
 
 #define PS_SWEEP_MAX_GENS 2
@@ -227,6 +229,12 @@
 {
     const uint32_t c1 = __builtin_amdgcn_bitop3_b32(p1, p2, p3, 0x01) & vm;
     uint32_t lt;
+#ifdef PS_CLASSES_BRANCHFREE
+    {
+        const uint32_t M = nE - 1u, m2 = 0u - ((M >> 2) & 1u), m1 = 0u - ((M >> 1) & 1u), m0 = 0u - (M & 1u);
+        lt = __builtin_amdgcn_bitop3_b32(p0, m2, __builtin_amdgcn_bitop3_b32(p5, m1, __builtin_amdgcn_bitop3_b32(p4, m0, 0xFFFFFFFFu, 0x8E), 0x8E), 0x8E);
+    }
+#else
     switch (nE) {
     case 1: lt = __builtin_amdgcn_bitop3_b32(p0, p5, p4, 0x01); break;
     case 2: lt = __builtin_amdgcn_bitop3_b32(p0, p5, p4, 0x03); break;
@@ -237,6 +245,7 @@
     case 7: lt = __builtin_amdgcn_bitop3_b32(p0, p5, p4, 0x7F); break;
     default: lt = 0xFFFFFFFFu; break;
     }
+#endif
     ps_class_words o;
     o.dec = k ? c1 & __builtin_amdgcn_bitop3_b32(p0, p5, p4, 0x07) : 0u;
     o.res = c1 & lt & ~o.dec;
@@ -295,10 +304,39 @@
     }
     return qn;
 }
-__device__ __forceinline__ uint32_t ps_entry_cell(uint32_t ent)
-{
-    const uint32_t cell = ((ent & 3u) << 2) | ((ent >> 3) & 3u), row = ((ent >> 2) & 1u) | ((ent >> 4) & 2u);
+PS_HD uint32_t ps_entry_cell(uint32_t ent)
+{
+    const uint32_t cell = ((ent & 3u) << 2) | ((ent >> 3) & 3u), row = ((ent >> 2) & 1u) | ((ent >> 4) & 2u) | ((ent >> 10) & 4u);
     return (row << 10) | ((ent >> 2) & 0x3F0u) | cell;
+}
+PS_HD uint32_t ps_entry_make(uint32_t lane, uint32_t second, uint32_t pair, uint32_t p)
+{
+    return p | (pair << 5) | (lane << 6) | (second << 12);
+}
+__device__ __forceinline__ uint32_t ps_push_scan_pass(uint32_t a0, uint32_t a1, uint32_t b0, uint32_t b1,
+                                                      uint16_t *q, uint32_t lane, uint32_t qcap)
+{
+    const uint32_t c1 = (uint32_t)__popc(a0), c2 = c1 + (uint32_t)__popc(a1), c3 = c2 + (uint32_t)__popc(b0), c = c3 + (uint32_t)__popc(b1);
+    const uint32_t incl = ps_wave_scan_incl(c);
+    const uint32_t qn = __builtin_amdgcn_readlane(incl, 63);
+    if (qn <= qcap) {
+        uint16_t *qp0 = q + (incl - c) - 1, *qp1 = qp0 + c1, *qp2 = qp0 + c2, *qp3 = qp0 + c3;
+#ifdef PS_PUSH_ONE_LOOP
+        uint32_t m = a0, n1 = a1, n2 = b0, n3 = b1;
+        uint32_t tg = ps_entry_make(lane, 0u, 0u, 0u), t1 = ps_entry_make(lane, 0u, 1u, 0u), t2 = ps_entry_make(lane, 1u, 0u, 0u), t3 = ps_entry_make(lane, 1u, 1u, 0u);
+        for (uint32_t i = 0; i < c; i++) {
+            while (!m) { m = n1; n1 = n2; n2 = n3; n3 = 0u; tg = t1; t1 = t2; t2 = t3; }
+            *++qp0 = (uint16_t)(tg | (uint32_t)__builtin_ctz(m));
+            m &= m - 1u;
+        }
+        return qn;
+#endif
+        for (uint32_t m = a0; m; m &= m - 1u) *++qp0 = (uint16_t)(ps_entry_make(lane, 0u, 0u, 0u) | (uint32_t)__builtin_ctz(m));
+        for (uint32_t m = a1; m; m &= m - 1u) *++qp1 = (uint16_t)(ps_entry_make(lane, 0u, 1u, 0u) | (uint32_t)__builtin_ctz(m));
+        for (uint32_t m = b0; m; m &= m - 1u) *++qp2 = (uint16_t)(ps_entry_make(lane, 1u, 0u, 0u) | (uint32_t)__builtin_ctz(m));
+        for (uint32_t m = b1; m; m &= m - 1u) *++qp3 = (uint16_t)(ps_entry_make(lane, 1u, 1u, 0u) | (uint32_t)__builtin_ctz(m));
+    }
+    return qn;
 }
 
 PS_HD uint32_t ps_gather_dword(uint32_t lane, uint32_t m) { return lane + 64u * m; }
@@ -325,11 +363,92 @@
 #define PS_WAVE_PREFETCH 0
 #endif
 __host__ __device__ constexpr uint32_t ps_queue_bytes(uint32_t qcap) { return (qcap * 2u + 15u) & ~15u; }
-__host__ __device__ constexpr uint32_t ps_wave_lds(uint32_t qcap) { return PS_BATCH_ROWS * 1024u + ps_queue_bytes(qcap); }
-
-template <bool DO_GATHER, bool DO_MUT, bool DO_HR, bool NT = false, bool WT = false, uint32_t T = 1>
+__host__ __device__ constexpr uint32_t ps_wave_lds(uint32_t qcap, uint32_t rows = PS_BATCH_ROWS) { return rows * 1024u + ps_queue_bytes(qcap); }
+
+#define PS_QREG_TRIPS 5u
+#define PS_QREG_ENTRIES (64u * PS_QREG_TRIPS)
+PS_HD bool ps_batch_partial(uint32_t batch, uint32_t batches, uint32_t off, uint32_t rows)
+{
+    return (batch == 0u && off != 0u) || (batch + 1u == batches && ((rows + off) & (PS_BATCH_ROWS - 1u)) != 0u);
+}
+PS_HD uint32_t ps_pass_batches(uint32_t batch, uint32_t end, uint32_t batches, uint32_t off, uint32_t rows, bool pair)
+{
+    return (pair && batch + 1u < end && !ps_batch_partial(batch, batches, off, rows) && !ps_batch_partial(batch + 1u, batches, off, rows)) ? 2u : 1u;
+}
+inline uint32_t ps_sweep_queue_entries(const ps_core_plan &pl, uint32_t cells, uint32_t rows, bool twice)
+{
+    if (!pl.has_events) return 16u;
+    if (pl.cshift > 1u || pl.k > 1u) return 0u;
+    const double m = (double)rows * (double)cells * (double)pl.R / 64.0;
+    const uint32_t n = ((uint32_t)std::ceil(m + 10.0 * std::sqrt(m) + 16.0) + 15u) & ~15u;
+    return twice ? 2u * n : n;
+}
+struct ps_wave_geom { uint32_t rows, qcap; };
+inline ps_wave_geom ps_wave_geometry(const ps_core_plan &pl, uint32_t cells, bool hr, uint32_t gens, uint32_t lds_limit,
+                                     uint32_t blocks_per_cu, uint32_t reserve, uint32_t force_rows = 0u)
+{
+    ps_wave_geom g = { PS_BATCH_ROWS, ps_sweep_queue_entries(pl, cells, PS_BATCH_ROWS, hr) };
+    if (gens < 2u || !pl.has_events || g.qcap == 0u) return g;
+    const uint32_t n8 = ps_sweep_queue_entries(pl, cells, 2u * PS_BATCH_ROWS, false);
+    if (force_rows != PS_BATCH_ROWS && n8 <= PS_QREG_ENTRIES) {
+        const uint32_t wg4 = 4u * ps_wave_lds(g.qcap), wg8 = 4u * ps_wave_lds(n8, 2u * PS_BATCH_ROWS);
+        const uint32_t want = std::max(1u, std::min(blocks_per_cu, lds_limit / wg4));
+        const uint32_t room = force_rows ? wg8 : want * wg8 + reserve;
+        if (room <= lds_limit) g = { 2u * PS_BATCH_ROWS, n8 };
+    }
+    return g;
+}
+
+template <bool DO_MUT, bool DO_HR, bool WT>
+__device__ __forceinline__ void ps_exact_pass_regs(const core_sweep_args &a, const ps_core_plan &pl, uint8_t *rowbuf, const uint16_t *q,
+                                                   uint32_t qn, uint32_t lane, uint32_t sg, uint32_t gen)
+{
+    static_assert(PS_QREG_TRIPS == 5u, "the switch below names the trips");
+    uint32_t hw[PS_QREG_TRIPS] = {};
+#pragma unroll 1
+    for (uint32_t tr = 0; 64u * tr < qn; tr++) {
+        const uint32_t e = 64u * tr + lane;
+        uint32_t h = 0u;
+        if (e < qn) {
+            const uint32_t ent = ps_entry_cell(q[e]);
+            const uint32_t cellidx = ent & 1023u, site = 4u * sg + (ent >> 10);
+            const ps_u4 l2 = ps_philox(site, cellidx, gen, PS_STREAM_CORE_L2, a.k0, a.k1);
+            const ps_cell cell = ps_classify_site<WT>(l2.x, pl, a, site);
+            if (DO_MUT && cell.mut) rowbuf[ent] = (uint8_t)cell.mut;
+            if (DO_HR && cell.hr) {
+                uint32_t donor = ps_mulhi(l2.y, a.N - 1u);
+                donor += (donor >= cellidx) ? 1u : 0u;
+                h = ent | (donor << 13) | (1u << 23);
+            }
+        }
+        if (DO_HR) {
+            switch (__builtin_amdgcn_readfirstlane(tr)) {
+            case 0: hw[0] = h; break;
+            case 1: hw[1] = h; break;
+            case 2: hw[2] = h; break;
+            case 3: hw[3] = h; break;
+            default: hw[PS_QREG_TRIPS - 1u] = h; break;
+            }
+        }
+    }
+    if (DO_HR) {
+        ps_wave_sync();
+#pragma unroll
+        for (uint32_t tr = 0; tr < PS_QREG_TRIPS; tr++)
+            if (64u * tr < qn && (hw[tr] >> 23))
+                hw[tr] = (hw[tr] & 0x801FFFu) | ((uint32_t)rowbuf[(hw[tr] & 0x1C00u) | ((hw[tr] >> 13) & 1023u)] << 13);
+        ps_wave_sync();
+#pragma unroll
+        for (uint32_t tr = 0; tr < PS_QREG_TRIPS; tr++)
+            if (64u * tr < qn && (hw[tr] >> 23)) rowbuf[hw[tr] & 0x1FFFu] = (uint8_t)((hw[tr] >> 13) & 0xFFu);
+    }
+    ps_wave_sync();
+}
+
+template <bool DO_GATHER, bool DO_MUT, bool DO_HR, bool NT = false, bool WT = false, uint32_t T = 1, bool PAIR = false>
 __global__ void __launch_bounds__(256, T > 1 ? 4 : PS_WAVE_LB) core_sweep_wave_kernel(core_sweep_args a)
 {
+    static_assert(!PAIR || T > 1, "two batches per pass: the two-generation form only");
     static_assert(T >= 1 && T <= PS_SWEEP_MAX_GENS, "generations per pass");
     static_assert(T == 1 || (DO_GATHER && (DO_MUT || DO_HR)), "several generations per pass: the gather + events form only");
 #ifdef PS_STAMP
@@ -343,8 +462,11 @@
     constexpr uint32_t PS_ROWS = PS_BATCH_ROWS;
     extern __shared__ __attribute__((aligned(16))) uint8_t lds[];
     const uint32_t wave = threadIdx.x >> 6, lane = threadIdx.x & 63u;
-    uint8_t *rowbuf = lds + wave * ps_wave_lds(a.qcap);
-    uint16_t *q = (uint16_t *)(rowbuf + PS_ROWS * 1024u);
+    constexpr uint32_t NB = PAIR ? 2u : 1u;
+    constexpr uint32_t prows = NB * PS_ROWS;
+    constexpr bool parked = !PAIR;
+    uint8_t *rowbuf = lds + wave * ps_wave_lds(a.qcap, prows);
+    uint16_t *q = (uint16_t *)(rowbuf + prows * 1024u);
     const ps_core_plan pl = a.plan;
     const uint32_t nE = 3u * pl.k + pl.R;
     constexpr bool events = DO_MUT || DO_HR;
@@ -374,7 +496,7 @@
         }
     }
 
-    constexpr uint32_t PS_CHUNK = 3u;
+    constexpr uint32_t PS_CHUNK = PAIR ? 4u : 3u;
     const uint32_t grp = blockIdx.x & 7u;
     const uint32_t off = a.site_offset & 3u, g0 = a.site_offset >> 2;
     const uint32_t batches = (a.rows + off + PS_ROWS - 1u) / PS_ROWS;
@@ -393,42 +515,53 @@
         const uint32_t chunk = __builtin_amdgcn_readfirstlane(next_chunk);
         if (b_lo + chunk * PS_CHUNK >= b_hi) break;
         if (lane == 0) next_chunk = __hip_atomic_fetch_add(ctr, 1u, __ATOMIC_RELAXED, __HIP_MEMORY_SCOPE_AGENT);
-    for (uint32_t cb = 0; cb < PS_CHUNK; cb++) {
+    for (uint32_t cb = 0; cb < PS_CHUNK;) {
         const uint32_t batch = b_lo + chunk * PS_CHUNK + cb;
         if (batch >= b_hi) break;
+        const uint32_t nb = PAIR ? ps_pass_batches(batch, min(b_lo + (chunk + 1u) * PS_CHUNK, b_hi), batches, off, a.rows, true) : 1u;
+        cb += nb;
         const int lr0 = (int)(batch * PS_ROWS) - (int)off;
         const uint32_t sg = g0 + batch;
         auto lrow = [&](uint32_t rr) -> uint32_t { return (uint32_t)min(max(lr0 + (int)rr, 0), (int)a.rows - 1); };
         uint4 v[PS_ROWS];
 #if PS_WAVE_PREFETCH
-        if (pf_batch == batch) {
+        if (!PAIR && pf_batch == batch) {
 #pragma unroll
             for (uint32_t rr = 0; rr < PS_ROWS; rr++) v[rr] = vn[rr];
         } else
 #endif
 #pragma unroll
-        for (uint32_t rr = 0; rr < PS_ROWS; rr++)
-            v[rr] = ps_load_row16(a.state + (size_t)lrow(rr) * a.pitch + ld_off, NT);
-        if (DO_GATHER) {
-#pragma unroll
-            for (uint32_t rr = 0; rr < PS_ROWS; rr++) *(uint4 *)(rowbuf + rr * 1024u + i0) = v[rr];
-            ps_wave_sync();
-        }
+        for (uint32_t bb = 0; bb < NB; bb++) {
+            if (bb >= nb) break;
+#pragma unroll
+            for (uint32_t rr = 0; rr < PS_ROWS; rr++)
+                v[rr] = ps_load_row16(a.state + (size_t)lrow(bb * PS_ROWS + rr) * a.pitch + ld_off, NT);
+            if (DO_GATHER) {
+#pragma unroll
+                for (uint32_t rr = 0; rr < PS_ROWS; rr++) *(uint4 *)(rowbuf + (bb * PS_ROWS + rr) * 1024u + i0) = v[rr];
+            }
+        }
+        if (DO_GATHER) ps_wave_sync();
         PS_T(0);
 
 #pragma unroll
         for (uint32_t t = 0; t < T; t++) {
         const uint32_t gen = a.gen + t;
-        uint32_t wl[2] = { 0u, 0u };
+        uint32_t wl[2 * NB] = {};
+#pragma unroll
+        for (uint32_t bb = 0; bb < NB; bb++) {
+        if (bb >= nb) break;
+        uint8_t *brows = rowbuf + bb * (PS_ROWS * 1024u);
+        const uint32_t sgb = sg + bb;
         ps_apply_words y[2] = {};
         if (events) {
-            const ps_u4 A0 = ps_philox_l1a(2u * sg, lane, gen, a.k0, a.k1);
-            const ps_u4 A1 = ps_philox_l1a(2u * sg + 1u, lane, gen, a.k0, a.k1);
-            const ps_u4 B = ps_philox_l1b(sg, lane, gen, a.k0, a.k1);
+            const ps_u4 A0 = ps_philox_l1a(2u * sgb, lane, gen, a.k0, a.k1);
+            const ps_u4 A1 = ps_philox_l1a(2u * sgb + 1u, lane, gen, a.k0, a.k1);
+            const ps_u4 B = ps_philox_l1b(sgb, lane, gen, a.k0, a.k1);
             const ps_class_words c0 = ps_classes(A0.x, A0.y, A0.z, A0.w, B.x, B.z, pl.k, nE, vm);
             const ps_class_words c1 = ps_classes(A1.x, A1.y, A1.z, A1.w, B.y, B.w, pl.k, nE, vm);
-            wl[0] = c0.res;
-            wl[1] = c1.res;
+            wl[2u * bb] = c0.res;
+            wl[2u * bb + 1u] = c1.res;
             if (DO_MUT) {
                 y[0] = ps_apply_prepare(c0.dec, B.x & c0.dec, B.z & c0.dec);
                 y[1] = ps_apply_prepare(c1.dec, B.y & c1.dec, B.w & c1.dec);
@@ -439,13 +572,13 @@
         uint32_t g[16] = {};
         auto gather = [&](uint32_t rr) {
 #pragma unroll
-            for (int k = 0; k < 16; k++) g[k] = rowbuf[rr * 1024u + pidx[t][k]];
+            for (int k = 0; k < 16; k++) g[k] = brows[rr * 1024u + pidx[t][k]];
         };
         if (ahead) gather(0u);
 #pragma unroll
         for (uint32_t rr = 0; rr < PS_ROWS; rr++) {
-            uint8_t *row = rowbuf + rr * 1024u;
-            uint4 d = v[rr];
+            uint8_t *row = brows + rr * 1024u;
+            uint4 d = T > 1 ? make_uint4(0u, 0u, 0u, 0u) : v[rr];
             if (DO_GATHER) {
                 if (!ahead) gather(rr);
                 uint32_t w[4];
@@ -471,33 +604,43 @@
             if (events && (DO_MUT || !DO_GATHER)) *(uint4 *)(row + i0) = d;
             __builtin_amdgcn_sched_barrier(0);
         }
+        }
         PS_T(1);
         const uint32_t qcap = a.qcap_limit ? min(a.qcap, a.qcap_limit) : a.qcap;
         uint32_t qn = 0;
-        if (events) qn = ps_push_scan(wl[0], wl[1], q, lane, qcap);
+        if (events) {
+            if (NB > 1) qn = ps_push_scan_pass(wl[0], wl[1], wl[2 * NB - 2], wl[2 * NB - 1], q, lane, qcap);
+            else qn = ps_push_scan(wl[0], wl[1], q, lane, qcap);
+        }
         PS_T(3);
         ps_wave_sync();
 #if PS_WAVE_PREFETCH
-        if (t + 1u == T) {
-            uint32_t nb = batch + 1u;
-            if (cb + 1u >= PS_CHUNK || nb >= b_hi) nb = b_lo + (uint32_t)__builtin_amdgcn_readfirstlane(next_chunk) * PS_CHUNK;
-            pf_batch = nb < b_hi ? nb : 0xFFFFFFFFu;
-            if (nb < b_hi) {
-                const int nlr0 = (int)(nb * PS_ROWS) - (int)off;
+        if (!PAIR && t + 1u == T) {
+            uint32_t nxb = batch + 1u;
+            if (cb >= PS_CHUNK || nxb >= b_hi) nxb = b_lo + (uint32_t)__builtin_amdgcn_readfirstlane(next_chunk) * PS_CHUNK;
+            pf_batch = nxb < b_hi ? nxb : 0xFFFFFFFFu;
+            if (nxb < b_hi) {
+                const int nlr0 = (int)(nxb * PS_ROWS) - (int)off;
 #pragma unroll
                 for (uint32_t rr = 0; rr < PS_ROWS; rr++)
                     vn[rr] = ps_load_row16(a.state + (size_t)(uint32_t)min(max(nlr0 + (int)rr, 0), (int)a.rows - 1) * a.pitch + ld_off, NT);
             }
         }
 #endif
-        const bool redo = events && (qn > qcap || (DO_HR && 2u * qn > qcap));
+#ifdef PS_TRIP_COUNT
+        if (lane == 0) {
+            atomicAdd((unsigned long long *)a.stamps + 4, (unsigned long long)((qn + 63u) >> 6));
+            atomicAdd((unsigned long long *)a.stamps + 7, (unsigned long long)nb);
+        }
+#endif
+        const bool redo = events && (qn > qcap || (DO_HR && parked && 2u * qn > qcap));
         if (redo) {
 #pragma unroll 1
-            for (uint32_t rr = 0; rr < PS_ROWS; rr++) {
+            for (uint32_t rr = 0; rr < nb * PS_ROWS; rr++) {
                 uint8_t *row = rowbuf + rr * 1024u;
                 const uint32_t site = 4u * sg + rr;
                 const ps_u4 Ar = ps_philox_l1a(site >> 1, lane, gen, a.k0, a.k1);
-                const ps_u4 Br = ps_philox_l1b(sg, lane, gen, a.k0, a.k1);
+                const ps_u4 Br = ps_philox_l1b(site >> 2, lane, gen, a.k0, a.k1);
                 uint32_t cmr = ps_cand_word(Ar, site, pl.cshift) & vm;
                 uint32_t hm = 0;
                 while (cmr) {
@@ -528,6 +671,8 @@
                 }
             }
             ps_wave_sync();
+        } else if (events && PAIR) {
+            ps_exact_pass_regs<DO_MUT, DO_HR, WT>(a, pl, rowbuf, q, qn, lane, sg, gen);
         } else if (events) {
             uint16_t *qh = q + qcap - 1u;
             for (uint32_t base = 0; base < qn; base += 64u) {
@@ -555,7 +700,7 @@
                     const uint32_t e = base + lane;
                     if (e < qn) {
                         const uint32_t h = *(qh - e);
-                        if (h >> 15) *(qh - e) = (uint16_t)((uint32_t)rowbuf[(ps_entry_cell(q[e]) & 3072u) | (h & 1023u)] | 0x8000u);
+                        if (h >> 15) *(qh - e) = (uint16_t)((uint32_t)rowbuf[(ps_entry_cell(q[e]) & 0x1C00u) | (h & 1023u)] | 0x8000u);
                     }
                 }
                 ps_wave_sync();
@@ -574,9 +719,9 @@
 
         if (has_chunk) {
 #pragma unroll
-            for (uint32_t rr = 0; rr < PS_ROWS; rr++) {
+            for (uint32_t rr = 0; rr < NB * PS_ROWS; rr++) {
                 const int lr = lr0 + (int)rr;
-                if (lr >= 0 && lr < (int)a.rows) {
+                if (rr < nb * PS_ROWS && lr >= 0 && lr < (int)a.rows) {
                     const uint4 o = (DO_GATHER || events) ? *(const uint4 *)(rowbuf + rr * 1024u + i0) : v[rr];
                     ps_store_row16(a.out + (size_t)lr * a.pitch + i0, o, NT);
                 }
diff --git a/pansim_amd/csrc/pansim_capi.hip b/pansim_amd/csrc/pansim_capi.hip
--- a/pansim_amd/csrc/pansim_capi.hip
+++ b/pansim_amd/csrc/pansim_capi.hip
@@ -256,6 +256,8 @@
     std::vector<uint32_t> h_r1, h_r2;
     uint32_t lds_limit = 160 * 1024;
     uint32_t sweep_blocks_per_cu = 8;
+    uint32_t sweep_pass_rows = 0;
+    uint32_t sweep_lds_reserve = 0;
     uint32_t sweep_rows = 4;
     bool force_block_sweep = false;
     bool force_inline_sweep = false;
@@ -269,6 +271,7 @@
     uint32_t free_cus_per_xcd = 0;
     bool exchange_beside_sweep = false;
     int last_sweep_form = 0;
+    uint32_t last_sweep_pass_rows = 0;
     int window_sweep = -1;
     int (*rows_refresh)(void *ctx) = nullptr;
     void *rows_ctx = nullptr;
@@ -422,6 +425,10 @@
     if (const char *e = getenv("PANSIM_SWEEP_GENERATIONS")) {
         const int v = atoi(e);
         if (v >= 0 && v <= (int)PS_SWEEP_MAX_GENS) p->sweep_generations = (uint32_t)v;
+    }
+    if (const char *e = getenv("PANSIM_SWEEP_PASS_ROWS")) {
+        const int v = atoi(e);
+        if (v == 0 || v == 4 || v == 8) p->sweep_pass_rows = (uint32_t)v;
     }
     if (const char *e = getenv("PANSIM_HGT_MODE")) p->hgt_mode = atoi(e);
     if (const char *e = getenv("PANSIM_SWEEP_OOP")) p->sweep_oop = std::max(-1, std::min(2, atoi(e)));
@@ -637,6 +644,9 @@
     } else if (k == "sweep_generations") {
         if (value < 0 || value > (int64_t)PS_SWEEP_MAX_GENS) return ps_fail(PS_ERR_INVALID, "sweep_generations must be 0 (choose), 1 or 2");
         p->sweep_generations = (uint32_t)value;
+    } else if (k == "sweep_pass_rows") {
+        if (value != 0 && value != 4 && value != 8) return ps_fail(PS_ERR_INVALID, "sweep_pass_rows must be 0 (choose), 4 or 8");
+        p->sweep_pass_rows = (uint32_t)value;
     } else if (k == "sweep_queue_cap") {
         if (value < 0 || value > 65536) return ps_fail(PS_ERR_INVALID, "sweep_queue_cap must be 0 (real size)..65536");
         p->sweep_queue_cap = (uint32_t)value;
@@ -1000,20 +1010,20 @@
 
 static uint32_t sweep_queue_entries(const ps_core_plan &pl, uint32_t cells, bool twice)
 {
-    if (!pl.has_events) return 16u;
-    if (pl.cshift > 1u || pl.k > 1u) return 0u;
-    const double m = (double)PS_BATCH_ROWS * (double)cells * (double)pl.R / 64.0;
-    const uint32_t n = ((uint32_t)std::ceil(m + 10.0 * std::sqrt(m) + 16.0) + 15u) & ~15u;
-    return twice ? 2u * n : n;
+    return ps_sweep_queue_entries(pl, cells, PS_BATCH_ROWS, twice);
 }
 
 template <bool GA, bool MU, bool HR>
 static int launch_core_sweep_wave(ps_population *p, core_sweep_args a, hipStream_t st, uint32_t gens = 1)
 {
     const uint32_t block = 256u, wpb = block / 64u;
-    a.qcap = sweep_queue_entries(a.plan, std::min(1024u, (uint32_t)p->cfg.pop_size), HR);
+    const ps_wave_geom wg = ps_wave_geometry(a.plan, std::min(1024u, (uint32_t)p->cfg.pop_size), HR, gens, p->lds_limit,
+                                             p->sweep_blocks_per_cu, p->sweep_lds_reserve, p->sweep_pass_rows);
+    a.qcap = wg.qcap;
+    p->last_sweep_pass_rows = wg.rows;
+    const bool pair = wg.rows > PS_BATCH_ROWS;
     a.launch_parity = (uint32_t)(p->sweep_launches++ & 1u);
-    const uint32_t lds = wpb * ps_wave_lds(a.qcap);
+    const uint32_t lds = wpb * ps_wave_lds(a.qcap, wg.rows);
     const uint32_t batches = (a.rows + (a.site_offset & 3u) + PS_BATCH_ROWS - 1u) / PS_BATCH_ROWS;
     const uint32_t want = (batches + wpb - 1u) / wpb;
     const uint32_t fit = std::max(1u, std::min(8u, p->lds_limit / lds));
@@ -1023,11 +1033,17 @@
     if (gens > 1) {
         if constexpr (GA && MU) {
             if (gens != 2u) return ps_fail(PS_ERR_INVALID, "the wave sweep applies 1 or 2 generations per launch, not %u", gens);
+#define PS_LAUNCH2(NT_, WT_)                                                                                                       \
+            do {                                                                                                                   \
+                if (pair) hipLaunchKernelGGL((core_sweep_wave_kernel<true, true, HR, NT_, WT_, 2u, true>), dim3(grid), dim3(block), lds, st, a);   \
+                else hipLaunchKernelGGL((core_sweep_wave_kernel<true, true, HR, NT_, WT_, 2u, false>), dim3(grid), dim3(block), lds, st, a);       \
+            } while (0)
             if (a.site_T) {
-                if (a.nt) hipLaunchKernelGGL((core_sweep_wave_kernel<true, true, HR, true, true, 2u>), dim3(grid), dim3(block), lds, st, a);
-                else hipLaunchKernelGGL((core_sweep_wave_kernel<true, true, HR, false, true, 2u>), dim3(grid), dim3(block), lds, st, a);
-            } else if (a.nt) hipLaunchKernelGGL((core_sweep_wave_kernel<true, true, HR, true, false, 2u>), dim3(grid), dim3(block), lds, st, a);
-            else hipLaunchKernelGGL((core_sweep_wave_kernel<true, true, HR, false, false, 2u>), dim3(grid), dim3(block), lds, st, a);
+                if (a.nt) PS_LAUNCH2(true, true);
+                else PS_LAUNCH2(false, true);
+            } else if (a.nt) PS_LAUNCH2(true, false);
+            else PS_LAUNCH2(false, false);
+#undef PS_LAUNCH2
         } else
             return ps_fail(PS_ERR_INVALID, "the wave sweep has no several-generation form of this step");
     } else
@@ -2351,6 +2367,12 @@
     return PS_OK;
 }
 
+extern "C" int ps_last_sweep_pass_rows(ps_population *p)
+{
+    if (!p) return ps_fail(PS_ERR_INVALID, "null handle");
+    return p->last_sweep_form == PS_SWEEP_FORM_WAVE ? (int)p->last_sweep_pass_rows : 0;
+}
+
 extern "C" int ps_last_sweep_form(ps_population *p)
 {
     if (!p) return ps_fail(PS_ERR_INVALID, "null handle");
@@ -3159,6 +3181,8 @@
 
 static int sim_refresh_rows(void *ctx);
 static uint32_t sim_sweep_generations(ps_sim *s);
+static uint32_t sim_sweep_pass_rows(ps_sim *s);
+static void sim_set_sweep_reserve(ps_sim *s);
 
 static int sim_create_impl(const ps_sim_params *p, ps_sim *s)
 {
@@ -3230,25 +3254,13 @@
         if (block_sweep_geometry(s->core, true, true, p->HR_rate > 0.0, &g, &lds, &nw))
             s->acc->hgt_list_in_global = lds + 16384u > s->core->lds_limit;
     }
-    {
-        const double bytes = 2.0 * (double)N * (double)s->core->cfg.ncols;
-        double ept;
-        if (sim_sweep_generations(s) >= 2u) {
-            const double per_gen_ms = bytes / 4.0e12 * 1e3 / 2.0;
-            ept = std::min((per_gen_ms - 0.222) / 0.445e-3, 192.0);
-        } else {
-            const double sweep_ms = bytes / 4.2e12 * 1e3;
-            ept = std::min((sweep_ms - 0.3) / 1.0e-3 * 0.5, 112.0);
-        }
-        s->acc->hgt_events_per_thread = ept >= 16.0 ? (uint32_t)ept : 0u;
-        if (const char *e = getenv("PANSIM_HGT_EVENTS_PER_THREAD")) s->acc->hgt_events_per_thread = (uint32_t)atoi(e);
-    }
     HIPCHK(hipEventCreateWithFlags(&s->ev_hgt, hipEventDisableTiming));
     {
         const uint32_t parts = hgt_partitions(s->acc);
         s->heavy_hgt = (double)N * s->der.n_recombinations_pan_total >= 7.5e6 && parts >= 1 && parts <= 1024;
     }
     if (const char *e = getenv("PANSIM_HEAVY_HGT")) s->heavy_hgt = atoi(e) != 0;
+    sim_set_sweep_reserve(s);
     if (!getenv("PANSIM_SWEEP_BLOCKS_PER_CU")) {
         uint64_t max_comp = 0;
         for (int c = 0; c < d.n_comp; c++) max_comp = std::max<uint64_t>(max_comp, d.comp_end[c] - d.comp_begin[c]);
@@ -3256,6 +3268,20 @@
         if (list_lds > 36 * 1024) s->acc->hgt_list_in_global = true;
         const uint32_t light = 4u;
         s->core->sweep_blocks_per_cu = list_lds <= 16 * 1024 ? light : std::min(light, 6u);
+    }
+    {
+        const double bytes = 2.0 * (double)N * (double)s->core->cfg.ncols;
+        double ept;
+        if (sim_sweep_generations(s) >= 2u) {
+            const bool pair = sim_sweep_pass_rows(s) > PS_BATCH_ROWS;
+            const double per_gen_ms = bytes / (pair ? 4.14e12 : 4.0e12) * 1e3 / 2.0;
+            ept = std::min((per_gen_ms - 0.222) / 0.445e-3, 192.0);
+        } else {
+            const double sweep_ms = bytes / 4.2e12 * 1e3;
+            ept = std::min((sweep_ms - 0.3) / 1.0e-3 * 0.5, 112.0);
+        }
+        s->acc->hgt_events_per_thread = ept >= 16.0 ? (uint32_t)ept : 0u;
+        if (const char *e = getenv("PANSIM_HGT_EVENTS_PER_THREAD")) s->acc->hgt_events_per_thread = (uint32_t)atoi(e);
     }
     HIPCHK(hipHostMalloc(&s->h_num_genes, N * sizeof(int32_t), hipHostMallocMapped));
     HIPCHK(hipHostMalloc(&s->h_logw, N * sizeof(double), hipHostMallocMapped));
@@ -3496,6 +3522,23 @@
     return PS_OK;
 }
 
+static void sim_set_sweep_reserve(ps_sim *s)
+{
+    const ps_derived &d = s->der;
+    uint64_t max_comp = 0;
+    for (int c = 0; c < d.n_comp; c++) max_comp = std::max<uint64_t>(max_comp, d.comp_end[c] - d.comp_begin[c]);
+    if (s->acc->site_weighted) max_comp = std::max<uint64_t>(max_comp, s->acc->d.G);
+    const uint64_t list = (((uint64_t)hgt_list_u16(s->acc, (uint32_t)max_comp) * 2u + 15u) & ~15ull) + 256u;
+    s->core->sweep_lds_reserve = (s->prm.HGT_rate > 0.0 && list <= 36u * 1024u && !s->acc->hgt_list_in_global) ? (uint32_t)list : 0u;
+}
+
+static uint32_t sim_sweep_pass_rows(ps_sim *s)
+{
+    ps_population *core = s->core;
+    return ps_wave_geometry(core->cplan, std::min(1024u, (uint32_t)core->cfg.pop_size), s->prm.HR_rate > 0.0, sim_sweep_generations(s),
+                            core->lds_limit, core->sweep_blocks_per_cu, core->sweep_lds_reserve, core->sweep_pass_rows).rows;
+}
+
 static uint32_t sim_sweep_generations(ps_sim *s)
 {
     ps_population *core = s->core;
@@ -3547,6 +3590,7 @@
         for (int c = 0; c < d.n_comp; c++) lrec[c] = (p.HGT_rate > 0.0) ? d.n_recombinations_pan[c] : 0.0;
         PSCHK(ps_set_site_rates(s->acc, d.n_comp, d.n_pan_mutations, lrec, w_acc_mut, w_acc_rec));
         if (s->acc->site_weighted && (uint64_t)hgt_list_u16(s->acc, (uint32_t)s->acc->d.G) * 2u > 36u * 1024u) s->acc->hgt_list_in_global = true;
+        sim_set_sweep_reserve(s);
     }
     return PS_OK;
 }
diff --git a/pansim_amd/population.py b/pansim_amd/population.py
--- a/pansim_amd/population.py
+++ b/pansim_amd/population.py
@@ -732,6 +732,11 @@
     def last_sweep_form(self):
         return int(self._lib.ps_last_sweep_form(self._h))
 
+    def last_sweep_pass_rows(self):
+        fn = self._lib.ps_last_sweep_pass_rows
+        fn.restype, fn.argtypes = C.c_int, [C.c_void_p]
+        return int(fn(self._h))
+
     def gene_frequencies(self):
         out = np.zeros(self.ncols + self.core_genes, np.float64)
         check(self._lib.ps_gene_frequencies(self._h, out))
```

New measurement: 3256 (median of 6 runs). 1.1% higher.
